# NeurAI-Lab/biHomE

Hardware: AMD Instinct MI355X
Metric: training image-pairs/s (128x128 patch, bs=64 per GPU, full step: fwd+bwd+Adam) (higher is better)
Workload: dtype f32

## Files before the change

### bihome_amd/_lib.py

```python
import ctypes
import os
from ctypes import POINTER, Structure, c_char_p, c_float, c_int, c_int64, c_void_p

_HERE = os.path.dirname(os.path.abspath(__file__))
TUNING = os.environ.get("BIHOME_TUNING") == "1"
_VARIANT = os.environ.get("BIHOME_LIB_VARIANT", "")
LIB_PATH = os.path.join(_HERE, "libbihome_hip_tuning.so" if TUNING else
                        ("libbihome_hip_%s.so" % _VARIANT if _VARIANT.isalnum() else "libbihome_hip.so"))


class BhConvDesc(Structure):
    _fields_ = [(n, c_int) for n in ("N", "Hi", "Wi", "Ci", "Ho", "Wo", "Co", "kh", "kw", "stride", "pad",
                                     "transposed", "in_nchw", "out_nchw", "precision", "w_layout", "route")] + \
               [("a_bound", c_void_p), ("b_bound", c_void_p)]


GEOMETRY_FIELDS = tuple(n for n, _ in BhConvDesc._fields_[:17])
AMAX_FLOATS = 512


class BhPack3x3Job(Structure):
    _fields_ = [("w", c_void_p), ("pf", c_void_p), ("pd", c_void_p), ("Co", c_int), ("Ci", c_int), ("split", c_int),
                ("reserved", c_int)]


ROUTE_GENERIC_CONV, ROUTE_HALO_SMALL, ROUTE_NO_STEM7, ROUTE_WGRAD_GENERIC, ROUTE_WGRAD_3TAP = 1, 2, 4, 8, 16


class BhBnReduce(Structure):
    _fields_ = [("z", c_void_p), ("y", c_void_p), ("stats", c_void_p), ("gamma", c_void_p), ("beta", c_void_p),
                ("eps", c_float), ("relu", c_int)]


class BhBnIn(Structure):
    _fields_ = [("table", c_void_p), ("groups", c_int), ("relu", c_int)]


P = c_void_p
SIGNATURES = {
    "bh_version": [],
    "bh_probe_mfma_bf16": [c_int, P, P, P],
    "bh_probe_mfma_f32": [c_int, P, P, P],
    "bh_device_arch": [c_char_p, c_int],
    "bh_h4pt_fwd": [P, c_int, c_float, c_float, P, P, P],
    "bh_h4pt_bwd": [P, P, P, c_int, c_float, c_float, P, P],
    "bh_dlt_fwd": [P, P, c_int, c_int, c_int, c_int, c_int, P, P, P, P],
    "bh_dlt_bwd": [P, P, P, P, P, c_int, c_int, c_int, c_int, c_int, P, c_int, P],
    "bh_dsac_scores_fwd": [P, c_int, c_int, P, P],
    "bh_scale_samples_fwd": [P, P, c_int, c_int64, c_int, P, P],
    "bh_scale_samples_bwd": [P, P, P, c_int, c_int64, c_int, P, P, c_int, P],
    "bh_dsac_score": [P, P, c_int, c_int, c_int, c_int, c_int, c_float, c_float, P, P, P],
    "bh_dsac_scores_bwd": [P, P, P, P, c_int, c_int, c_int, c_int, c_int, c_float, c_float, P, P, P, c_int, P],
    "bh_ransac_homography": [P, P, c_int, c_int, c_int, c_int, c_float, P, P, P, P, P, P, P, P, P],
    "bh_homography_refine_lm": [P, P, c_int, c_int, c_int, c_int, P, P, P, P],
    "bh_warp_fwd": [P, P, c_int, c_int, c_int, c_int, c_int, P, P, c_int, P],
    "bh_warp_bwd": [P, P, P, P, c_int, c_int, c_int, c_int, c_int, P, c_int, P],
    "bh_triplet_l1_fwd": [P] * 8 + [c_int, c_int, c_int, P, P, P, c_int, P],
    "bh_bihome_loss_fwd": [P, P, P, c_int, c_float, P, P],
    "bh_bihome_loss_bwd": [P] * 14 + [c_int, c_int, c_int, c_float] + [P] * 6 + [P],
    "bh_oneline_loss_fwd": [P, P, P, P, P, c_int, c_int, c_int, c_float, c_int, P, P, P, P, P, c_int, P],
    "bh_oneline_loss_bwd": [P, P, P, P, P, P, P, c_int, c_int, c_int, c_int, P, P, P, P],
    "bh_zhang_triplet_fwd": [P] * 8 + [c_int, c_int, c_float, c_int, P, P, P, P],
    "bh_zhang_triplet_bwd": [P] * 12 + [c_int, c_int, c_int] + [P] * 8 + [P],
    "bh_warp_bwd_img": [P, P, c_int, c_int, c_int, c_int, P, P, c_int, P],
    "bh_photo_warp_fwd": [P, P, P, c_int, c_int, c_int, c_int, c_int, P, c_int, P],
    "bh_photo_warp_bwd": [P, P, P, P, c_int, c_int, c_int, c_int, c_int, P, c_int, P],
    "bh_mask_fwd": [P, P, c_int, c_int, c_float, P, P, P, P, P],
    "bh_mask_bwd": [P] * 7 + [c_int, c_int, c_float, P, P, P],
    "bh_conv3x3_pack": [P, c_int, P],
    "bh_conv3x3_pack_f16": [P, c_int, P],
    "bh_absmax": [P, c_int64, P, P],
    "bh_bn_fwd_coeffs": [P, P, P, P, P, c_int, c_int, c_int, c_float, c_float, P, P, P],
    "bh_bn_fwd": [P] * 8 + [c_int, c_int, c_int, c_float, c_float, c_int, c_int, P, P],
    "bh_bn_bwd": [P] * 11 + [c_int, c_int, c_int, c_float, c_int, c_int, P, P, P, P],
    "bh_conv_variant": [POINTER(BhConvDesc), c_int, c_int, c_int, c_char_p, c_int],
    "bh_conv_fwd": [P, P, P, P, POINTER(BhConvDesc), P],
    "bh_conv_fwd_act": [P, P, P, P, P, POINTER(BhConvDesc), c_int, P],
    "bh_conv_fwd_amax": [P, P, P, P, POINTER(BhConvDesc), P, P],
    "bh_conv_fwd_bnstats": [P, P, P, P, POINTER(BhConvDesc), P, c_int, P],
    "bh_conv_fwd_bnin": [P, P, P, P, POINTER(BhConvDesc), P, c_int, POINTER(BhBnIn), P],
    "bh_conv_wgrad_bnin": [P, P, P, P, POINTER(BhConvDesc), P, c_int64, POINTER(BhBnIn), P],
    "bh_conv_dgrad": [P, P, P, POINTER(BhConvDesc), c_int, P],
    "bh_conv_dgrad_colsum": [P, P, P, POINTER(BhConvDesc), P, P],
    "bh_bias_grad_from_sums": [P, P, c_int, c_int, P],
    "bh_conv_dgrad_s2": [P, P, P, POINTER(BhConvDesc), c_int, P, P],
    "bh_conv_dgrad_bnreduce": [P, P, P, POINTER(BhConvDesc), c_int, POINTER(BhBnReduce), P, c_int, P],
    "bh_col2im_c1": [P, P, POINTER(BhConvDesc), c_int, P],
    "bh_stem7_dgrad_c1": [P, P, P, POINTER(BhConvDesc), P],
    "bh_stem7_dgrad_c1_warp": [P, P, P, POINTER(BhConvDesc), P, P, P, c_int, P, P],
    "bh_stem7_fwd_warp": [P, P, c_int, P, P, P, POINTER(BhConvDesc), P, P, P, c_int, P],
    "bh_stem7_wgrad": [P, P, P, POINTER(BhConvDesc), P, ctypes.c_size_t, P],
    "bh_conv_wgrad": [P, P, P, P, POINTER(BhConvDesc), P],
    "bh_conv_wgrad_det": [P, P, P, P, POINTER(BhConvDesc), P, c_int64, P],
    "bh_conv_bias_grad": [P, P, POINTER(BhConvDesc), P],
    "bh_bn_stats_doubles": [c_int, c_int],
    "bh_bn_scratch_doubles": [c_int, c_int],
    "bh_bn_stats": [P, P, c_int, c_int, c_int, c_int, P],
    "bh_bn_maxpool_fwd": [P] * 8 + [c_int] * 5 + [c_float, c_float, c_int, c_int, P, P],
    "bh_bn_maxpool_bwd": [P] * 10 + [c_int] * 5 + [c_float, c_int, c_int, P, P, P, P],
    "bh_bn_bwd_from_1x1": [P, P, c_int] + [P] * 8 + [c_int, c_int, c_int, c_float, c_int, P, P],
    "bh_bn_join_scratch_doubles": [c_int, c_int],
    "bh_bn_join_fwd": [P] * 13 + [c_int, c_int, c_int, c_float, c_float, c_float, c_float, c_int, P, P],
    "bh_bn_join_bwd": [P] * 15 + [c_int, c_int, c_int, c_float, c_float, c_int, P, P, P],
    "bh_bn_join_bwd_remask": [P] * 16 + [c_int, c_int, c_int, c_float, c_float, c_int, P, P, P],
    "bh_tail_ws_doubles": [c_int, c_int, c_int],
    "bh_tail_scratch_floats": [c_int, c_int, c_int],
    "bh_tail_fwd": [P] * 11 + [c_int] * 6 + [c_float, c_float, c_int, c_int, P],
    "bh_tail_bwd": [P] * 17 + [c_int] * 6 + [c_float, c_int, c_int, P],
    "bh_synth_pairs": [P] * 5 + [c_int] * 5 + [c_float, c_float, P, P, P],
    "bh_synth_image": [P, P, P, c_int, c_int, c_int, c_int, c_float, c_float, P, P],
    "bh_maxpool3s2_fwd": [P, P, P, c_int, c_int, c_int, c_int, P],
    "bh_maxpool3s2_bwd": [P, P, P, c_int, c_int, c_int, c_int, P],
    "bh_gap_fwd": [P, P, c_int, c_int, c_int, P],
    "bh_gap_bwd": [P, P, c_int, c_int, c_int, P],
    "bh_add": [P, P, P, c_int64, P],
}


class BihomeLibError(RuntimeError):
    pass


def _load():
    if not os.path.exists(LIB_PATH):
        raise BihomeLibError(
            "bihome_amd: %s not found - the HIP extension is not built. Run `python __graft_entry__.py build` "
            "(hipcc --offload-arch=gfx950). There is no CPU fallback." % LIB_PATH)
    lib = ctypes.CDLL(LIB_PATH)
    for name, argtypes in SIGNATURES.items():
        try:
            fn = getattr(lib, name)
        except AttributeError as e:
            raise BihomeLibError("bihome_amd: %s does not export %s (stale build?)" % (LIB_PATH, name)) from e
        fn.argtypes = argtypes
        fn.restype = c_int
    lib.bh_conv_wgrad_det_bytes.argtypes = [POINTER(BhConvDesc)]
    lib.bh_conv_wgrad_det_bytes.restype = c_int64
    lib.bh_stem7_wgrad_ws_bytes.argtypes = [POINTER(BhConvDesc)]
    lib.bh_stem7_wgrad_ws_bytes.restype = ctypes.c_size_t
    lib.bh_warp_bwd_img_scratch_doubles.argtypes = [c_int, c_int, c_int, c_int, c_int]
    lib.bh_warp_bwd_img_scratch_doubles.restype = ctypes.c_size_t
    if TUNING:
        lib.bh_debug_force_tile.argtypes = [c_int, c_int]
        lib.bh_debug_force_tile.restype = c_int
    return lib


lib = _load()
ROUTE_DETERMINISTIC, BN_DETERMINISTIC, F_DETERMINISTIC = 128, 32, 1
DSAC_METHODS = {"repr_error": 0, "inliers_ratio": 1, "soft_inliers_ratio": 2}
ROUTE_C3_PC = 512
ROUTE_WX3_PC = 1024
ROUTE_WX3_SHARED = 2048
ROUTE_GEMM_X3 = 4096
ROUTE_C3_TILE_WG = 256


def check(rc, what):
    if rc != 0:
        kind = {-1: "BH_E_BADARG", -2: "BH_E_UNSUPPORTED"}.get(rc, "hipError_t %d" % rc)
        raise BihomeLibError("%s failed: %s" % (what, kind))
```

### bihome_amd/csrc/bn.hip

```cpp
#include "common.h"

#define BN_MAX_CHUNKS 256

struct BnGeom {
    int groups, rows, C, C4, LPR, RPP, nchunks, rows_per_chunk;
    int det;
};

static bool bn_geom(int groups, int rows, int C, BnGeom& g, int det) {
    if (C % 4 || groups < 1 || rows < 1) return false;
    g.groups = groups; g.rows = rows; g.C = C; g.C4 = C / 4; g.det = det;
    if (g.C4 > 256 || (256 % g.C4)) return false;
    g.LPR = g.C4; g.RPP = 256 / g.LPR;
    int n = rows / (g.RPP * 4);
    if (n < 1) n = 1;
    if (n > BN_MAX_CHUNKS) n = BN_MAX_CHUNKS;
    g.rows_per_chunk = (rows + n - 1) / n;
    g.nchunks = (rows + g.rows_per_chunk - 1) / g.rows_per_chunk;
    return true;
}

template <int NV>
__device__ __forceinline__ void reduce_rows(double (&v)[NV], int LPR, int RPP, double* sm ) {
    for (int i = 0; i < NV; ++i) sm[threadIdx.x * NV + i] = v[i];
// ... 582 lines not shown
    for (int i = 0; i < 4; ++i) {
        const int c = cq * 4 + i;
        ra[i] = bn_raw(stats_a, gamma_a, remask ? beta_a : nullptr, nullptr, nullptr, 0, g.groups, grp, g.C, c, g.det);
        rb[i] = bn_raw(stats_b, gamma_b, remask ? beta_b : nullptr, nullptr, nullptr, 0, g.groups, grp, g.C, c, g.det);
        cf[i] = coef[(size_t)grp * g.C + c];
    }
    const size_t gbase = ((size_t)grp * g.rows) * g.C + cq * 4;
    const int stride = gridDim.x * g.RPP;
    int r = blockIdx.x * g.RPP + r0;
    float4 dv[4], yv[4], av[4], bv[4];
    auto issue = [&](int rbase) {
#pragma unroll
        for (int u = 0; u < 4; ++u) {
            const int rr = rbase + u * stride;
            const size_t off = gbase + (size_t)rr * g.C;
            const bool ok = rr < g.rows;
            dv[u] = make_float4(0.f, 0.f, 0.f, 0.f); av[u] = dv[u]; bv[u] = dv[u];
            yv[u] = make_float4(1.f, 1.f, 1.f, 1.f);
            if (ok) {
                dv[u] = *reinterpret_cast<const float4*>(gy + off);
                if (relu && !remask) yv[u] = *reinterpret_cast<const float4*>(y + off);
                av[u] = *reinterpret_cast<const float4*>(xa + off);
                bv[u] = *reinterpret_cast<const float4*>(xb + off);
            }
        }
    };
    issue(r);
    float ma[4], ia[4], sca[4], mb[4], ib[4], scb[4], shm[4];
    const double inv_rows = 1.0 / (double)g.rows;
#pragma unroll
    for (int i = 0; i < 4; ++i) {
        float sha, shb;
        bn_coeffs_from_raw(ra[i], 0, eps_a, inv_rows, ma[i], ia[i], sca[i], sha);
        bn_coeffs_from_raw(rb[i], 0, eps_b, inv_rows, mb[i], ib[i], scb[i], shb);
        shm[i] = sha + shb;
    }
    while (true) {
#pragma unroll
        for (int u = 0; u < 4; ++u) {
            const int rr = r + u * stride;
            if (rr >= g.rows) break;
            const size_t off = gbase + (size_t)rr * g.C;
            const float d0[4] = {dv[u].x, dv[u].y, dv[u].z, dv[u].w};
            const float y0[4] = {yv[u].x, yv[u].y, yv[u].z, yv[u].w};
            const float a[4] = {av[u].x, av[u].y, av[u].z, av[u].w}, b[4] = {bv[u].x, bv[u].y, bv[u].z, bv[u].w};
            float oa[4], ob[4];
#pragma unroll
            for (int i = 0; i < 4; ++i) {
                const float yi = remask ? __builtin_fmaf(a[i], sca[i], __builtin_fmaf(b[i], scb[i], shm[i])) : y0[i];
                const float di = (relu && !(yi > 0.f)) ? 0.f : d0[i];
                const float e = di - cf[i].x;
                oa[i] = sca[i] * (e - (a[i] - ma[i]) * ia[i] * cf[i].y);
                ob[i] = scb[i] * (e - (b[i] - mb[i]) * ib[i] * cf[i].z);
                vmax_a = fmaxf(vmax_a, fabsf(oa[i])); vmax_b = fmaxf(vmax_b, fabsf(ob[i]));
            }
            *reinterpret_cast<float4*>(gxa + off) = make_float4(oa[0], oa[1], oa[2], oa[3]);
            *reinterpret_cast<float4*>(gxb + off) = make_float4(ob[0], ob[1], ob[2], ob[3]);
        }
        r += 4 * stride;
        if (r >= g.rows) break;
        issue(r);
    }
    if (amax_a) bh_amax_commit(amax_a, vmax_a, blockIdx.x + blockIdx.y * 7u, sm_amax);
    if (amax_b) { __syncthreads(); bh_amax_commit(amax_b, vmax_b, blockIdx.x + blockIdx.y * 5u, sm_amax); }
}

BH_KNOB(g_bn_apply_cap, 512);
#ifdef BH_TUNING
void bh_bn_tune(int cap) { g_bn_apply_cap = cap; }
#endif
static int apply_blocks(const BnGeom& g) {
    int nb = (g.rows + g.RPP * 4 - 1) / (g.RPP * 4);
    int cap = g_bn_apply_cap / g.groups;
    if (cap < 1) cap = 1;
    if (nb > cap) nb = cap;
    if (nb < 1) nb = 1;
    return nb;
}

__global__ void __launch_bounds__(256) bn_fwd_coeffs_kernel(const double* __restrict__ stats, const float* __restrict__ gamma,
                                                            const float* __restrict__ beta, BnGeom g, float eps, float momentum,
                                                            float* __restrict__ upd_mean, float* __restrict__ upd_var,
                                                            float2* __restrict__ table, unsigned* __restrict__ amax) {
    __shared__ float sm_amax[4];
    if (upd_mean && blockIdx.x == gridDim.x - 1) { bn_update_running(stats, g, momentum, upd_mean, upd_var); return; }
    const int i = blockIdx.x * 256 + threadIdx.x;
    float bound = 0.f;
    if (i < g.groups * g.C) {
        const int grp = i / g.C, c = i - grp * g.C;
        float mean, invstd, sc, sh;
        bn_coeffs(stats, gamma, beta, nullptr, nullptr, 0, g.groups, grp, g.C, c, eps, (double)g.rows, mean, invstd, sc, sh, g.det);
        table[i] = make_float2(sc, sh);
        bound = 2.0f * (fabsf(gamma ? gamma[c] : 1.f) * sqrtf((float)g.rows) + fabsf(beta ? beta[c] : 0.f));
    }
    if (amax) bh_amax_commit(amax, bound, blockIdx.x, sm_amax);
}

int bn_launch_stats(const float* x, int groups, int rows, int C, double* sums, hipStream_t s, int det) {
    BnGeom g;
    if (!bn_geom(groups, rows, C, g, det ? 1 : 0)) return BH_E_UNSUPPORTED;
    hipLaunchKernelGGL(bn_stats_kernel, dim3(g.nchunks, groups), dim3(256), 0, s, x, g, sums);
    BH_LAUNCH_CHECK();
    return BH_OK;
}

int bn1_fwd(const float* x, const float* gamma, const float* beta, float* running_mean, float* running_var, const float* res, float* y,
            double* stats, int groups, int rows, float eps, float momentum, int flags, int use_running, hipStream_t s);
int bn1_bwd(const float* gy, const float* y, const float* x, const float* gamma, const float* beta, const double* stats, float* gx,
            float* gres, float* ggamma, float* gbeta, double* scratch, int groups, int rows, float eps, int flags, int use_running,
            const float* running_mean, const float* running_var, hipStream_t s);

extern "C" {

int bh_bn_stats_doubles(int groups, int C) { return (int)BH_BN_SUM_DOUBLES(groups, C); }

int bh_bn_fwd(const float* x, const float* gamma, const float* beta, float* running_mean, float* running_var,
              const float* res, float* y, double* stats, int groups, int rows, int C, float eps, float momentum,
              int flags, int use_running, float* amax_y, void* stream) {
    BnGeom g;
    if (!x || !y || !stats) return BH_E_BADARG;
    if (use_running && (!running_mean || !running_var)) return BH_E_BADARG;
    if (C == 1) return amax_y ? BH_E_UNSUPPORTED : bn1_fwd(x, gamma, beta, running_mean, running_var, res, y, stats, groups, rows, eps, momentum, flags, use_running, bh_stream(stream));
    if (!bn_geom(groups, rows, C, g, (flags & BH_BN_DETERMINISTIC) ? 1 : 0)) return BH_E_UNSUPPORTED;
    hipStream_t s = bh_stream(stream);
    if (!use_running && !(flags & 8)) {
        hipLaunchKernelGGL(bn_stats_kernel, dim3(g.nchunks, groups), dim3(256), 0, s, x, g, stats);
        BH_LAUNCH_CHECK();
    }
    const bool upd = !use_running && running_mean && running_var;
    hipLaunchKernelGGL(bn_apply_kernel, dim3(apply_blocks(g), groups), dim3(256), 0, s, x, gamma, beta, running_mean,
                       running_var, res, y, stats, g, eps, flags, use_running, momentum, upd ? running_mean : nullptr,
                       upd ? running_var : nullptr, reinterpret_cast<unsigned*>(amax_y));
    BH_LAUNCH_CHECK();
    return BH_OK;
}

int bh_bn_fwd_coeffs(const double* stats, const float* gamma, const float* beta, float* running_mean, float* running_var, int groups,
                     int rows, int C, float eps, float momentum, float* table, float* amax_y, void* stream) {
    BnGeom g;
    if (!stats || !table) return BH_E_BADARG;
    if (!bn_geom(groups, rows, C, g, -1)) return BH_E_UNSUPPORTED;
    const bool upd = running_mean && running_var;
    hipLaunchKernelGGL(bn_fwd_coeffs_kernel, dim3((groups * C + 255) / 256 + (upd ? 1 : 0)), dim3(256), 0, bh_stream(stream), stats, gamma, beta, g, eps,
                       momentum, upd ? running_mean : nullptr, upd ? running_var : nullptr, reinterpret_cast<float2*>(table),
                       reinterpret_cast<unsigned*>(amax_y));
    BH_LAUNCH_CHECK();
    return BH_OK;
}

int bh_bn_bwd(const float* gy, const float* y, const float* x, const float* gamma, const float* beta, const double* stats, float* gx,
              float* gres, float* ggamma, float* gbeta, double* scratch, int groups, int rows, int C, float eps, int flags,
              int use_running, const float* running_mean, const float* running_var, float* amax_gx, void* stream) {
    BnGeom g;
    if (!gy || !x || !gx || !stats || !scratch || ((flags & 1) && !(flags & 4) && !y)) return BH_E_BADARG;
    if ((flags & 4) && (flags & 2)) return BH_E_BADARG;
    if (C == 1) return amax_gx ? BH_E_UNSUPPORTED : bn1_bwd(gy, y, x, gamma, beta, stats, gx, gres, ggamma, gbeta, scratch, groups, rows, eps, flags, use_running,
                               running_mean, running_var, bh_stream(stream));
    if (!bn_geom(groups, rows, C, g, (flags & BH_BN_DETERMINISTIC) ? 1 : 0)) return BH_E_UNSUPPORTED;
    hipStream_t s = bh_stream(stream);
    if (flags & 16) {
        if (use_running) return BH_E_BADARG;
        hipLaunchKernelGGL(bn_bwd_apply_kernel, dim3(apply_blocks(g), groups), dim3(256), 0, s, gy, y, x, gamma, beta,
                           (const float4*)nullptr, gx, gres, g, flags, stats, (const double*)scratch, eps, ggamma, gbeta,
                           reinterpret_cast<unsigned*>(amax_gx));
        BH_LAUNCH_CHECK();
        return BH_OK;
    }
    float4* coef = reinterpret_cast<float4*>(scratch);
    double* part = scratch + (size_t)groups * C * 2;
    const bool need_sums = !use_running || ggamma || gbeta;
    if (need_sums) {
        hipLaunchKernelGGL(bn_bwd_reduce_kernel, dim3(g.nchunks, groups), dim3(256), 0, s, gy, y, x, gamma, beta, stats,
                           running_mean, running_var, g, eps, flags, use_running, part);
        BH_LAUNCH_CHECK();
    }
    BnGeom gf = g;
    if (!need_sums) gf.nchunks = 0;
    hipLaunchKernelGGL(bn_bwd_finalize_kernel, dim3(C), dim3(64), 0, s, part, gf, stats, running_mean, running_var, eps,
                       use_running, ggamma, gbeta, coef);
    BH_LAUNCH_CHECK();
    hipLaunchKernelGGL(bn_bwd_apply_kernel, dim3(apply_blocks(g), groups), dim3(256), 0, s, gy, y, x, gamma, beta, coef,
                       gx, gres, g, flags, (const double*)nullptr, (const double*)nullptr, eps, (float*)nullptr,
                       (float*)nullptr, reinterpret_cast<unsigned*>(amax_gx));
    BH_LAUNCH_CHECK();
    return BH_OK;
}

int bh_bn_scratch_doubles(int groups, int C) { return groups * C * 2 * (1 + (BN_MAX_CHUNKS > 256 ? BN_MAX_CHUNKS : 256)); }

int bh_bn_stats(const float* x, double* stats, int groups, int rows, int C, int flags, void* stream) {
    if (!x || !stats) return BH_E_BADARG;
    return bn_launch_stats(x, groups, rows, C, stats, bh_stream(stream), (flags & BH_BN_DETERMINISTIC) ? 1 : 0);
}

int bh_bn_maxpool_fwd(const float* x, const float* gamma, const float* beta, float* running_mean, float* running_var, float* y,
                      unsigned char* idx, double* stats, int groups, int N, int Hi, int Wi, int C, float eps, float momentum, int flags,
                      int use_running, float* amax_y, void* stream) {
    BnGeom g;
    if (!x || !y || !stats || N < 1 || groups < 1 || N % groups) return BH_E_BADARG;
    if (use_running && (!running_mean || !running_var)) return BH_E_BADARG;
    const int rows = (N / groups) * Hi * Wi;
    if (!bn_geom(groups, rows, C, g, (flags & BH_BN_DETERMINISTIC) ? 1 : 0) || groups * C * 8 > 32768) return BH_E_UNSUPPORTED;
    hipStream_t s = bh_stream(stream);
    if (!use_running && !(flags & 8)) {
        hipLaunchKernelGGL(bn_stats_kernel, dim3(g.nchunks, groups), dim3(256), 0, s, x, g, stats);
        BH_LAUNCH_CHECK();
    }
    const int Ho = (Hi - 1) / 2 + 1, Wo = (Wi - 1) / 2 + 1;
    const size_t total = (size_t)N * Ho * Wo * (C / 4);
    size_t nb = (total + 255) / 256;
    if (nb > 2048) nb = 2048;
    nb = (nb * 256 / (C / 4)) * (C / 4) / 256;
    if (nb < 1) nb = 1;
    const bool upd = !use_running && running_mean && running_var;
    hipLaunchKernelGGL(bn_maxpool_fwd_kernel, dim3((unsigned)nb), dim3(256), (size_t)groups * C * 8, s, x, gamma, beta, running_mean, running_var,
                       stats, y, idx, g, N, Hi, Wi, Ho, Wo, eps, flags & 1, use_running, momentum, upd ? running_mean : nullptr,
                       upd ? running_var : nullptr, reinterpret_cast<unsigned*>(amax_y));
    BH_LAUNCH_CHECK();
    return BH_OK;
}

struct PoolGeom { int Hi, Wi, Ho, Wo, ipg; };

struct PoolTaps {
    uchar4 w[4];
    float4 g[4];
    unsigned char t[4];
    bool ok[4];
};
__device__ __forceinline__ void pooled_taps_load(PoolTaps& q, const unsigned char* __restrict__ idx, const float* __restrict__ gy, const PoolGeom& pg,
                                                 int n, int iy, int ix, int C4, int c, bool live) {
    const int oyA = iy >> 1, oyB = (iy + 1) >> 1, oxA = ix >> 1, oxB = (ix + 1) >> 1;
    const bool vy = oyB != oyA && oyB < pg.Ho, vx = oxB != oxA && oxB < pg.Wo;
#pragma unroll
    for (int k = 0; k < 4; ++k) {
        const bool by = k >> 1, bx = k & 1;
        q.ok[k] = live && (!by || vy) && (!bx || vx);
        const int oy = (by && vy) ? oyB : oyA, ox = (bx && vx) ? oxB : oxA;
        q.t[k] = (unsigned char)((iy - (oy * 2 - 1)) * 3 + (ix - (ox * 2 - 1)));
        const size_t o = live ? (((size_t)n * pg.Ho + oy) * pg.Wo + ox) * C4 + c : 0;
        q.w[k] = *reinterpret_cast<const uchar4*>(idx + o * 4);
        q.g[k] = *reinterpret_cast<const float4*>(gy + o * 4);
    }
}
__device__ __forceinline__ float4 pooled_taps_sum(const PoolTaps& q) {
    float4 d = make_float4(0.f, 0.f, 0.f, 0.f);
#pragma unroll
    for (int k = 0; k < 4; ++k) {
        if (q.ok[k] && q.w[k].x == q.t[k]) d.x += q.g[k].x;
        if (q.ok[k] && q.w[k].y == q.t[k]) d.y += q.g[k].y;
        if (q.ok[k] && q.w[k].z == q.t[k]) d.z += q.g[k].z;
        if (q.ok[k] && q.w[k].w == q.t[k]) d.w += q.g[k].w;
    }
    return d;
}

__global__ void __launch_bounds__(256) bn_maxpool_bwd_reduce_kernel(const float* __restrict__ gy, const unsigned char* __restrict__ idx,
                                                                    const float* __restrict__ x, const float* __restrict__ gamma,
                                                                    const float* __restrict__ beta, const double* __restrict__ stats,
                                                                    const float* __restrict__ rmean, const float* __restrict__ rvar, BnGeom g,
                                                                    PoolGeom pg, float eps, int relu, int use_running, double* __restrict__ part) {
    __shared__ double sm[256 * 8];
    const int cq = threadIdx.x % g.LPR, r0 = threadIdx.x / g.LPR;
    const int grp = blockIdx.y, chunk = blockIdx.x;
    const int rbeg = chunk * g.rows_per_chunk, rend = min(g.rows, rbeg + g.rows_per_chunk);
    float mean[4], invstd[4], sc[4], sh[4];
#pragma unroll
    for (int i = 0; i < 4; ++i)
        bn_coeffs(stats, gamma, beta, rmean, rvar, use_running, g.groups, grp, g.C, cq * 4 + i, eps, (double)g.rows, mean[i], invstd[i], sc[i], sh[i], g.det);
    const size_t gbase = ((size_t)grp * g.rows) * g.C + cq * 4;
    const int hw = pg.Hi * pg.Wi;
    double v[8] = {0, 0, 0, 0, 0, 0, 0, 0};
    for (int r = rbeg + r0; r < rend; r += 4 * g.RPP) {
        float4 a[4];
        PoolTaps q[4];
#pragma unroll
        for (int u = 0; u < 4; ++u) {
            const int rr = r + u * g.RPP;
            const bool live = rr < rend;
            const int rc = live ? rr : rbeg;
            const int nl = rc / hw, p = rc - nl * hw, iy = p / pg.Wi, ix = p - iy * pg.Wi;
            a[u] = *reinterpret_cast<const float4*>(x + gbase + (size_t)rc * g.C);
            pooled_taps_load(q[u], idx, gy, pg, grp * pg.ipg + nl, iy, ix, g.C4, cq, live);
        }
#pragma unroll
        for (int u = 0; u < 4; ++u) {
            if (r + u * g.RPP >= rend) break;
            float4 d = pooled_taps_sum(q[u]);
            const float4 av = a[u];
            if (relu) {
                if (!(av.x * sc[0] + sh[0] > 0.f)) d.x = 0.f;
                if (!(av.y * sc[1] + sh[1] > 0.f)) d.y = 0.f;
                if (!(av.z * sc[2] + sh[2] > 0.f)) d.z = 0.f;
                if (!(av.w * sc[3] + sh[3] > 0.f)) d.w = 0.f;
            }
            v[0] += d.x; v[1] += d.y; v[2] += d.z; v[3] += d.w;
            v[4] += (double)(d.x * ((av.x - mean[0]) * invstd[0]));
            v[5] += (double)(d.y * ((av.y - mean[1]) * invstd[1]));
            v[6] += (double)(d.z * ((av.z - mean[2]) * invstd[2]));
            v[7] += (double)(d.w * ((av.w - mean[3]) * invstd[3]));
        }
    }
    reduce_rows<8>(v, g.LPR, g.RPP, sm);
    if ((int)threadIdx.x < g.LPR) {
        double* p = part + (((size_t)grp * g.nchunks + chunk) * g.C + cq * 4) * 2;
        for (int i = 0; i < 4; ++i) { p[i * 2] = v[i]; p[i * 2 + 1] = v[4 + i]; }
    }
}

__global__ void __launch_bounds__(256) bn_maxpool_bwd_apply_kernel(const float* __restrict__ gy, const unsigned char* __restrict__ idx,
                                                                   const float* __restrict__ x, const float* __restrict__ gamma,
                                                                   const float* __restrict__ beta, const float4* __restrict__ coef,
                                                                   float* __restrict__ gx, BnGeom g, PoolGeom pg, int relu,
                                                                   unsigned* __restrict__ amax) {
// ... 293 lines not shown
```

### bihome_amd/csrc/capi.hip

```cpp
#include "common.h"
#include <stdarg.h>
#include <stdio.h>
#include <string.h>


thread_local BhQuery* bh_query_ctx = nullptr;


bool bh_query(const char* fmt, ...) {
    BhQuery* q = bh_query_ctx;
    if (!q) return false;
    if (q->len && q->len < (int)sizeof(q->name) - 1) q->name[q->len++] = '+';
    va_list ap;
    va_start(ap, fmt);
    const int room = (int)sizeof(q->name) - q->len;
    const int w = vsnprintf(q->name + q->len, (size_t)room, fmt, ap);
    va_end(ap);
    if (w > 0) q->len += w < room ? w : room - 1;
    return true;
}

extern "C" {

int bh_version(void) { return 2; }


int bh_device_arch(char* buf, int buflen) {
    hipDeviceProp_t prop;
    hipError_t e = hipGetDeviceProperties(&prop, 0);
    if (e != hipSuccess) return (int)e;
    if (buf && buflen > 0) {
        strncpy(buf, prop.gcnArchName, (size_t)buflen - 1);
        buf[buflen - 1] = 0;
    }
    return BH_OK;
}

int bh_conv_variant(const bh_conv_desc* d, int which, int accumulate, int with_bnstats , char* buf, int n) {
    if (!d || !buf || n < 2 || which < 0 || which > 6) return BH_E_BADARG;
    BhQuery q;
    q.name[0] = 0; q.len = 0;
    float* p = reinterpret_cast<float*>(static_cast<uintptr_t>(256));
    double* pd = reinterpret_cast<double*>(static_cast<uintptr_t>(256));
    bh_query_ctx = &q;
    int rc;
    if (which == 0) rc = with_bnstats ? bh_conv_fwd_bnstats(p, p, nullptr, p, d, pd, with_bnstats, nullptr) : bh_conv_fwd(p, p, nullptr, p, d, nullptr);
    else if (which == 1) rc = bh_conv_dgrad(p, p, p, d, accumulate, nullptr);
    else if (which == 2) rc = bh_conv_wgrad(p, p, p, nullptr, d, nullptr);
    else if (which == 3) rc = bh_conv_wgrad_det(p, p, p, nullptr, d, p, 1ll << 40, nullptr);
    else if (which == 6) rc = bh_conv_dgrad_colsum(p, p, p, d, pd, nullptr);
    else {
        bh_bn_reduce bnr = {};
        bnr.z = p; bnr.y = which == 5 ? p : nullptr; bnr.stats = pd; bnr.gamma = p; bnr.beta = p; bnr.eps = 1e-5f; bnr.relu = 1;
        rc = bh_conv_dgrad_bnreduce(p, p, p, d, accumulate, &bnr, pd, with_bnstats > 0 ? with_bnstats : 1, nullptr);
    }
    bh_query_ctx = nullptr;
    if (rc) return rc;
    strncpy(buf, q.name, (size_t)n - 1);
    buf[n - 1] = 0;
    return BH_OK;
}

}
```

### bihome_amd/csrc/conv3x3.hip

```cpp
#include "common.h"
#include "conv3x3_args.h"
#include <type_traits>

#ifndef C3_X3_PIPE
#define C3_X3_PIPE 0
#endif

#ifndef C3_BN32_WAVES
#define C3_BN32_WAVES 2
#endif

#ifdef BH_TUNING
__device__ unsigned long long g_c3_ts[8 * 16384];
#define C3_STAMP(tile, k) do { if (a.dbg_ts && threadIdx.x == 0 && (tile) < 16384) { g_c3_ts[(tile) * 8 + (k)] = wall_clock64();          \
        if ((k) == 1 || (k) == 2) g_c3_ts[(tile) * 8 + 4 + (k)] = __builtin_readcyclecounter(); } } while (0)
#else
#define C3_STAMP(tile, k) do { } while (0)
#endif

constexpr int C3_HALO_BYTES = 8 * 200 * 16;
constexpr int C3_B_BYTES = 8192;
constexpr int C3_LDS_BYTES = 2 * C3_HALO_BYTES + 2 * C3_B_BYTES;

template <int BN, int SUBT, int TM, bool MAP4 = false>
__device__ __forceinline__ void c3_epilogue(const C3Args& a, f32x16 (&acc)[TM], int bx, int n0, int wm, int wn, int wh, int l31, int kh2,
                                            double& s1, double& s2, int& img, int& g) {
    g = bx * SUBT + wm;
    const int n = n0 + wn * 32 + l31;
    const bool valid = g < a.subtiles && n < a.Nn;
    const int gg = g < a.subtiles ? g : 0;
    int ty, tx;
    if constexpr (MAP4) { img = gg * 4; ty = 0; tx = 0; }
    else if (a.tpi_shift >= 0) { img = gg >> a.tpi_shift; const int t = gg & (a.tiles_per_img - 1); ty = t >> a.tx_shift; tx = t & (a.tiles_x - 1); }
    else { img = gg / a.tiles_per_img; const int t = gg - img * a.tiles_per_img; ty = t / a.tiles_x; tx = t - ty * a.tiles_x; }
    const float bv = (a.bias && n < a.Nn) ? a.bias[n] : 0.0f;
    s1 = 0.0; s2 = 0.0;
    float r_mean = 0.f, r_invstd = 0.f, r_sc = 0.f, r_sh = 0.f;
    if (a.bnr_z && valid) {
        const int grp = img / a.imgs_per_group;
        const double rows = (double)a.bnr_rows;
        const double mu = bn_sum_total(a.bnr_stats, a.groups, grp, a.Nn, n, 0, a.det) / rows;
        double var = bn_sum_total(a.bnr_stats, a.groups, grp, a.Nn, n, 1, a.det) / rows - mu * mu;
        if (var < 0) var = 0;
        r_mean = (float)mu;
        r_invstd = 1.0f / sqrtf((float)var + a.bnr_eps);
        r_sc = (a.bnr_gamma ? a.bnr_gamma[n] : 1.f) * r_invstd;
        r_sh = (a.bnr_beta ? a.bnr_beta[n] : 0.f) - r_mean * r_sc;
    }
    if (valid) {
        unsigned rowoff[4];
#pragma unroll
        for (int rq = 0; rq < 4; ++rq) {
            const int sr = c3_strip_row(2 * rq + kh2);
            if constexpr (MAP4)
                rowoff[rq] = ((unsigned)((img + 2 * wh + (sr >> 2)) * 16 + (sr & 3) * 4) * (unsigned)a.Nn + (unsigned)n) * 4u;
            else
                rowoff[rq] = ((unsigned)((img * a.H + ty * 8 + sr) * a.W + tx * 8) * (unsigned)a.Nn + (unsigned)n) * 4u;
        }
        const unsigned colstep = (unsigned)a.Nn * 4u;
        const unsigned col0 = MAP4 ? 0u : (unsigned)(wh * 4) * colstep;
        const __amdgpu_buffer_rsrc_t rsO = __builtin_amdgcn_make_buffer_rsrc(a.Out, 0, a.out_bytes, 0x00020000);
#define C3_SOFF(i, r) (col0 + (unsigned)((i) * 4 + ((r) & 3)) * colstep)
        if (!a.accumulate && !a.res && !a.bnr_z) {
#pragma unroll
            for (int i = 0; i < TM; ++i)
#pragma unroll
                for (int rq = 0; rq < 4; ++rq) {
                    float q1 = 0.f, q2 = 0.f;
#pragma unroll
                    for (int c = 0; c < 4; ++c) {
                        float v = acc[i][rq * 4 + c] + bv;
                        if (a.relu) v = fmaxf(v, 0.0f);
                        __builtin_amdgcn_raw_buffer_store_b32(__builtin_bit_cast(unsigned, v), rsO, rowoff[rq], C3_SOFF(i, c), 0);
                        q1 += v; q2 = __builtin_fmaf(v, v, q2);
                    }
                    s1 += (double)q1; s2 += (double)q2;
                }
        } else {
            const bool rd_old = a.accumulate, rd_res = a.res != nullptr, rd_z = a.bnr_z != nullptr;
            const bool rd_y = rd_z && a.bnr_relu && a.bnr_y != nullptr;
            const float c_x0 = -r_mean * r_invstd;
            auto body = [&](auto EXTRA, auto ZMODE) {
                constexpr bool HAS_EXTRA = decltype(EXTRA)::value;
                constexpr int ZM = decltype(ZMODE)::value;
                float ext[HAS_EXTRA ? TM : 1][16], zin[ZM > 0 ? TM : 1][16], yin[ZM == 2 ? TM : 1][16];
                if constexpr (HAS_EXTRA) {
                    const __amdgpu_buffer_rsrc_t rsR = __builtin_amdgcn_make_buffer_rsrc(const_cast<float*>(rd_res ? a.res : a.Out), 0, a.out_bytes, 0x00020000);
#pragma unroll
                    for (int i = 0; i < TM; ++i)
#pragma unroll
                        for (int r = 0; r < 16; ++r) {
                            float o = 0.f;
                            if (rd_old) o = __builtin_bit_cast(float, __builtin_amdgcn_raw_buffer_load_b32(rsO, rowoff[r >> 2], C3_SOFF(i, r), 0));
                            if (rd_res) o += __builtin_bit_cast(float, __builtin_amdgcn_raw_buffer_load_b32(rsR, rowoff[r >> 2], C3_SOFF(i, r), 0));
                            ext[i][r] = o;
                        }
                }
                if constexpr (ZM > 0) {
                    const __amdgpu_buffer_rsrc_t rsZ = __builtin_amdgcn_make_buffer_rsrc(const_cast<float*>(a.bnr_z), 0, a.out_bytes, 0x00020000);
#pragma unroll
                    for (int i = 0; i < TM; ++i)
#pragma unroll
                        for (int r = 0; r < 16; ++r)
                            zin[i][r] = __builtin_bit_cast(float, __builtin_amdgcn_raw_buffer_load_b32(rsZ, rowoff[r >> 2], C3_SOFF(i, r), 0));
                }
                if constexpr (ZM == 2) {
                    const __amdgpu_buffer_rsrc_t rsY = __builtin_amdgcn_make_buffer_rsrc(const_cast<float*>(a.bnr_y), 0, a.out_bytes, 0x00020000);
#pragma unroll
                    for (int i = 0; i < TM; ++i)
#pragma unroll
                        for (int r = 0; r < 16; ++r)
                            yin[i][r] = __builtin_bit_cast(float, __builtin_amdgcn_raw_buffer_load_b32(rsY, rowoff[r >> 2], C3_SOFF(i, r), 0));
                }
#pragma unroll
                for (int i = 0; i < TM; ++i)
#pragma unroll
                    for (int rq = 0; rq < 4; ++rq) {
                        float q1 = 0.f, q2 = 0.f;
#pragma unroll
                        for (int c = 0; c < 4; ++c) {
                            const int r = rq * 4 + c;
                            float v = acc[i][r] + bv;
                            if constexpr (HAS_EXTRA) v += ext[i][r];
                            if (a.relu) v = fmaxf(v, 0.0f);
                            __builtin_amdgcn_raw_buffer_store_b32(__builtin_bit_cast(unsigned, v), rsO, rowoff[rq], C3_SOFF(i, r), 0);
                            if constexpr (ZM > 0) {
                                const float zv = zin[i][r];
                                if (a.bnr_relu) {
                                    const float yv = ZM == 2 ? yin[i][r] : __builtin_fmaf(zv, r_sc, r_sh);
                                    if (!(yv > 0.f)) v = 0.f;
                                }
                                q1 += v; q2 = __builtin_fmaf(v, __builtin_fmaf(zv, r_invstd, c_x0), q2);
                            } else {
                                q1 += v; q2 = __builtin_fmaf(v, v, q2);
                            }
                        }
                        s1 += (double)q1; s2 += (double)q2;
                    }
            };
            using T_ = std::true_type; using F_ = std::false_type;
            using Z0 = std::integral_constant<int, 0>; using Z1 = std::integral_constant<int, 1>; using Z2 = std::integral_constant<int, 2>;
            if (rd_old || rd_res) {
                if (!rd_z) body(T_{}, Z0{}); else if (!rd_y) body(T_{}, Z1{}); else body(T_{}, Z2{});
            } else {
                if (!rd_z) body(F_{}, Z0{}); else if (!rd_y) body(F_{}, Z1{}); else body(F_{}, Z2{});
            }
        }
#undef C3_SOFF
    }
}

template <int BN, int PHASE>
__device__ __forceinline__ void c3_stats_merge(const C3Args& a, char* redb, double s1, double s2, int img, int g, int bx, int n0, int wave,
                                               int lane, int tid) {
    const int l31 = lane & 31, kh2 = lane >> 5;
    double* red = reinterpret_cast<double*>(redb);
    int* grp_of = reinterpret_cast<int*>(redb + 4 * 32 * 2 * 8);
    if constexpr (PHASE != 2) {
        s1 += __shfl_xor(s1, 32, 64);
        s2 += __shfl_xor(s2, 32, 64);
        const int grp = img / a.imgs_per_group;
        if (kh2 == 0) { red[(wave * 32 + l31) * 2] = s1; red[(wave * 32 + l31) * 2 + 1] = s2; }
        if (lane == 0) grp_of[wave] = g < a.subtiles ? grp : -1;
    }
    if constexpr (PHASE == 0) __syncthreads();
    if constexpr (PHASE != 1) {
        constexpr int SHARE = BN == 64 ? 2 : 4;
        if (tid < (4 / SHARE) * 64) {
            const int cr = tid >> 6, col = (tid >> 1) & 31, mom = tid & 1;
            const int nn = n0 + cr * 32 + col;
            if (nn < a.Nn) {
                int done = 0;
#pragma unroll
                for (int w0 = 0; w0 < SHARE; ++w0) {
                    const int wv0 = BN == 64 ? (w0 + 2 * cr) : w0;
                    const int g0 = grp_of[wv0];
                    if (g0 < 0 || (done >> w0) & 1) continue;
                    double tot = red[(wv0 * 32 + col) * 2 + mom];
#pragma unroll
                    for (int w1 = w0 + 1; w1 < SHARE; ++w1) {
                        const int wv1 = BN == 64 ? (w1 + 2 * cr) : w1;
                        if (grp_of[wv1] == g0) { tot += red[(wv1 * 32 + col) * 2 + mom]; done |= 1 << w1; }
                    }
                    bh_acc_add(&a.bn_sums[bn_sum_index(bx % BH_BN_SUM_SLOTS, a.groups, g0, a.Nn, nn, mom)], tot, a.det);
                }
            }
        }
    }
}

template <bool FLIP, int BN, bool BF16 = false, int SUBT = 2, bool PACKED = false, bool X3 = false, bool BNI = false, int NP = 3, bool MAP4 = false, bool F16 = false>
__global__ void __launch_bounds__(256, X3 ? ((BN == 32 && NP == 2 && !BNI) ? C3_BN32_WAVES : 2) : 1) conv3x3_halo_kernel(C3Args a) {
    static_assert(NP == 3 || (NP == 2 && X3), "two pieces: split form only");
    static_assert(!F16 || (X3 && NP == 2), "fp16 pieces: the two-piece split form");
    static_assert(!MAP4 || (X3 && SUBT == 1 && BN == 64 && !BNI), "the 4 x 4 map form: split operands, one sub-tile, 64-channel tile");
    constexpr int SLOTS = MAP4 ? 144 : 100;
    constexpr int ROWP = MAP4 ? 6 : 10;
    static_assert(SUBT == 2 || BN == 64, "one sub-tile per workgroup is built for the 64-channel tile only");
    static_assert(!X3 || (PACKED && !BF16), "the split form exists for packed weights only");
    static_assert(!BNI || (X3 && !FLIP), "the BatchNorm-on-load form is a forward f32x3 kernel");
    constexpr int TM = (BN == 64 && SUBT == 2) ? 2 : 1;
    constexpr int HPL = SLOTS * SUBT;
    constexpr int HALO_B = (X3 ? 4 * NP : 8) * HPL * 16;
    constexpr int XJ = (4 * HPL + 255) / 256;
    constexpr int HINS = (8 * HPL + 63) / 64;
    constexpr int HJ = (HINS + 3) / 4;
    constexpr int BINS = BN == 64 ? 2 : 1;
    extern __shared__ __attribute__((aligned(16))) char smem[];
    const int tid = threadIdx.x, lane = tid & 63, wave = __builtin_amdgcn_readfirstlane(tid >> 6);
    const int l31 = lane & 31, kh2 = lane >> 5;
    const int wm = SUBT == 1 ? 0 : (BN == 64 ? (wave & 1) : (wave >> 1));
    const int wn = BN == 64 ? (wave >> 1) : 0;
    const int wh = (BN == 64 && SUBT == 2) ? 0 : (wave & 1);
    const int n0 = blockIdx.y * BN;
    constexpr unsigned OOB = 0xFFFFFFF0u;
    __amdgpu_buffer_rsrc_t rsA = __builtin_amdgcn_make_buffer_rsrc(const_cast<float*>(a.Src), 0, a.src_bytes, 0x00020000);
    __amdgpu_buffer_rsrc_t rsB = __builtin_amdgcn_make_buffer_rsrc(const_cast<float*>(a.Wt), 0, a.w_bytes, 0x00020000);
    float f16_s = 1.0f;
    int f16_kout = 0;
    if constexpr (F16) {
        const unsigned* const wrec = reinterpret_cast<const unsigned*>(a.Wt) + (a.w_bytes >> 2);
        unsigned wv = lane < 16 ? wrec[lane] : 0u;
#pragma unroll
        for (int off = 8; off > 0; off >>= 1) { const unsigned o = (unsigned)__shfl_xor((int)wv, off, 64); wv = o > wv ? o : wv; }
        const int kw = bh_f16_scale_exp((unsigned)__builtin_amdgcn_readfirstlane((int)wv));
        const int ka = bh_f16_scale_exp(bh_amax_read(a.amax_src, lane));
        f16_s = __builtin_bit_cast(float, (unsigned)(127 + ka) << 23);
        f16_kout = -(ka + kw);
    }

    unsigned boff[2] = {0u, 0u};
#pragma unroll
    for (int i = 0; i < BINS; ++i) {
        const int idx = i * 4 + wave;
        if (!FLIP) {
            const int plane = BN == 64 ? idx : idx * 2 + (lane >> 5), n = n0 + (BN == 64 ? lane : (lane & 31));
            boff[i] = n < a.Nn ? ((unsigned)(n * 9) * (unsigned)a.Cw + (unsigned)(plane * 4)) * 4u : OOB;
        } else {
            constexpr int LPR = BN / 4;
            const int k = idx * (64 / LPR) + lane / LPR, n = n0 + (lane % LPR) * 4;
            boff[i] = n < a.Nn ? ((unsigned)(k * 9) * (unsigned)a.Cw + (unsigned)n) * 4u : OOB;
        }
    }
#ifdef BH_TUNING
    const int nch = a.dbg_nch >= 0 ? a.dbg_nch : a.Kc / 32;
    const int dbg_noload = a.dbg_noload;
#else
    const int nch = a.Kc / 32;
    constexpr int dbg_noload = 0;
#endif
    const int wnG = blockIdx.y * (BN / 32) + (BN == 64 ? (wave >> 1) : 0);
    const unsigned pb_voff = (unsigned)lane * 16u;
#define C3_LOAD_B(dst, c, tap)                                                                                          \
    do {                                                                                                                \
        const unsigned so_ = (unsigned)(((c) * 9 + (tap)) * a.NW + wnG) * 4096u;                                        \
        _Pragma("unroll") for (int q_ = 0; q_ < 4; ++q_) {                                                              \
            const auto v_ = __builtin_amdgcn_raw_buffer_load_b128(rsB, pb_voff + (unsigned)q_ * 1024u, so_, 0);         \
            dst[q_] = __builtin_bit_cast(float4, v_);                                                                   \
        }                                                                                                               \
    } while (0)
#define C3_LOAD_BX(dst, c, tap)                                                                                         \
    do {                                                                                                                \
        const unsigned so_ = (unsigned)(((c) * 9 + (tap)) * a.NW + wnG) * (unsigned)(NP * 2048);                        \
        _Pragma("unroll") for (int q_ = 0; q_ < 2 * NP; ++q_) {                                                              \
            const auto v_ = __builtin_amdgcn_raw_buffer_load_b128(rsB, pb_voff + (unsigned)q_ * 1024u, so_, 0);         \
            dst[q_] = __builtin_bit_cast(uint4, v_);                                                                    \
        }                                                                                                               \
    } while (0)
    const int slab0 = (a.Kc / 32 > 1 ? 2 : 1) * HALO_B;
#define issue_B(c, tap, bs)                                                                                             \
    do {                                                                                                                \
        const unsigned soff_ = FLIP ? (unsigned)(((c) * 32 * 9 + (8 - (tap))) * a.Cw) * 4u                             \
                                    : (unsigned)((tap) * a.Cw + (c) * 32) * 4u;                                        \
        char* base_ = smem + slab0 + (bs) * C3_B_BYTES + wave * 1024;                                              \
        __builtin_amdgcn_raw_ptr_buffer_load_lds(rsB, (lds_void_ptr)(base_), 16, boff[0], soff_, 0, 0);                 \
        if (BINS == 2)                                                                                                  \
            __builtin_amdgcn_raw_ptr_buffer_load_lds(rsB, (lds_void_ptr)(base_ + 4096), 16, boff[1], soff_, 0, 0); \
    } while (0)
#define C3_ISSUE_HALO(j, c, hs)                                                                                         \
    do {                                                                                                                \
        if ((j) < HJ && (j) * 4 + wave < HINS && (((j) * 4 + wave) * 64 + lane) < 8 * HPL)                              \
            __builtin_amdgcn_raw_ptr_buffer_load_lds(rsA, (lds_void_ptr)(smem + (hs) * HALO_B + ((j) * 4 + wave) * 1024), \
                                                     16, hoff[(j) < HJ ? (j) : 0], (unsigned)((c) * 32) * 4u, 0, 0);    \
    } while (0)

    if constexpr (BNI) {
        const int n4 = a.bni_groups * a.Kc / 2;
        for (int i = tid; i < n4; i += 256)
            reinterpret_cast<float4*>(smem + a.bni_lds)[i] = reinterpret_cast<const float4*>(a.bni)[i];
        __syncthreads();
    }
    double S1 = 0.0, S2 = 0.0;
    int Simg = 0, Sg = 0x7fffffff, Sbx = 0;
    if (a.desync > 0 && (((blockIdx.x + gridDim.x * blockIdx.y) >> 8) & 1)) {
        for (int i = 0; i < a.desync; ++i) __builtin_amdgcn_s_sleep(127);
    }
    for (int it = 0; it < a.tpb; ++it) {
    const int bx = blockIdx.x * a.tpb + it;
// ... 278 lines not shown
                        for (int i = 0; i < TM; ++i) acc[i] = __builtin_amdgcn_mfma_f32_32x32x2f32(af[i][q].z, bcur[q].z, acc[i], 0, 0, 0);
#pragma unroll
                        for (int i = 0; i < TM; ++i) acc[i] = __builtin_amdgcn_mfma_f32_32x32x2f32(af[i][q].w, bcur[q].w, acc[i], 0, 0, 0);
                    }
                }
                if (tap == 8) {
                    __builtin_amdgcn_sched_barrier(0);
                    asm volatile("s_waitcnt vmcnt(0)" ::: "memory");
                    __syncthreads();
                }
#pragma unroll
                for (int q = 0; q < 4; ++q) bcur[q] = bnext[q];
            }
        }
    } else {
    for (int c = 0; c < nch; ++c) {
        const int hs = c & 1;
        const char* hbase = smem + hs * HALO_B + a_lane;
        const bool more = c + 1 < nch;
#pragma unroll
        for (int tap = 0; tap < 9; ++tap) {
            const int dy = tap / 3, dx = tap - dy * 3;
            const char* ap = hbase + (dy * 10 + dx) * 16;
            const char* bp = smem + slab0 + bs * C3_B_BYTES + b_lane;
            float4 af[TM][4], b[4];
#pragma unroll
            for (int q = 0; q < 4; ++q) {
#pragma unroll
                for (int i = 0; i < TM; ++i) af[i][q] = *reinterpret_cast<const float4*>(ap + q * (2 * HPL * 16) + i * 64);
                if (!FLIP) b[q] = *reinterpret_cast<const float4*>(bp + q * (2 * BN * 16));
                else {
                    b[q].x = *reinterpret_cast<const float*>(bp + (q * 8 + 0) * (BN * 4));
                    b[q].y = *reinterpret_cast<const float*>(bp + (q * 8 + 1) * (BN * 4));
                    b[q].z = *reinterpret_cast<const float*>(bp + (q * 8 + 2) * (BN * 4));
                    b[q].w = *reinterpret_cast<const float*>(bp + (q * 8 + 3) * (BN * 4));
                }
            }
            if (!(dbg_noload & 1)) {
                if (tap < 8) issue_B(c, tap + 1, bs ^ 1);
                else if (more) issue_B(c + 1, 0, bs ^ 1);
            }
            if (tap < HJ && more && !(dbg_noload & 2)) C3_ISSUE_HALO(tap, c + 1, hs ^ 1);
            if constexpr (BF16) {
#pragma unroll
                for (int s2 = 0; s2 < 2; ++s2) {
                    const bf16x8 bb = c3_pack_bf16(b[2 * s2], b[2 * s2 + 1]);
#pragma unroll
                    for (int i = 0; i < TM; ++i)
                        acc[i] = __builtin_amdgcn_mfma_f32_32x32x16_bf16(c3_pack_bf16(af[i][2 * s2], af[i][2 * s2 + 1]), bb, acc[i], 0, 0, 0);
                }
            } else {
#pragma unroll
            for (int q = 0; q < 4; ++q) {
#pragma unroll
                for (int i = 0; i < TM; ++i) acc[i] = __builtin_amdgcn_mfma_f32_32x32x2f32(af[i][q].x, b[q].x, acc[i], 0, 0, 0);
#pragma unroll
                for (int i = 0; i < TM; ++i) acc[i] = __builtin_amdgcn_mfma_f32_32x32x2f32(af[i][q].y, b[q].y, acc[i], 0, 0, 0);
#pragma unroll
                for (int i = 0; i < TM; ++i) acc[i] = __builtin_amdgcn_mfma_f32_32x32x2f32(af[i][q].z, b[q].z, acc[i], 0, 0, 0);
#pragma unroll
                for (int i = 0; i < TM; ++i) acc[i] = __builtin_amdgcn_mfma_f32_32x32x2f32(af[i][q].w, b[q].w, acc[i], 0, 0, 0);
            }
            }
            __builtin_amdgcn_sched_barrier(0);
            asm volatile("s_waitcnt vmcnt(0)" ::: "memory");
            __syncthreads();
            bs ^= 1;
        }
    }
    }
    }
#undef C3_ISSUE_HALO
#undef issue_B
#undef C3_LOAD_B
#undef C3_LOAD_BX

    C3_STAMP(bx * gridDim.y + blockIdx.y, 2);
    if constexpr (F16) {
#pragma unroll
        for (int i = 0; i < TM; ++i)
#pragma unroll
            for (int r = 0; r < 16; ++r) acc[i][r] = __builtin_ldexpf(acc[i][r], f16_kout);
    }
    double s1, s2;
    int img, g;
    c3_epilogue<BN, SUBT, TM, MAP4>(a, acc, bx, n0, wm, wn, wh, l31, kh2, s1, s2, img, g);
    if (a.bn_sums) {
        if (a.stat_acc) { S1 += s1; S2 += s2; Sbx = bx; if (g < Sg) { Sg = g; Simg = img; } }
        else c3_stats_merge<BN, 0>(a, smem, s1, s2, img, g, bx, n0, wave, lane, tid);
    }
#ifdef BH_TUNING
    if (a.dbg_ts) asm volatile("s_waitcnt vmcnt(0)" ::: "memory");
#endif
    __syncthreads();
    C3_STAMP(bx * gridDim.y + blockIdx.y, 3);
    }
    if (a.bn_sums && a.stat_acc) c3_stats_merge<BN, 0>(a, smem, S1, S2, Simg, Sg, Sbx, n0, wave, lane, tid);
}

constexpr int C3_MIN_BLOCKS = 256;
BH_KNOB(g_c3_noload, 0); BH_KNOB(g_c3_dbg_nch, -1); BH_KNOB(g_c3_subt, 2); BH_KNOB(g_c3_tpb, 2); BH_KNOB(g_c3_stamp, 0); BH_KNOB(g_c3_desync, 0); BH_KNOB(g_c3_walk32, 1); BH_KNOB(g_c3_pc, 1); BH_KNOB(g_c3_wt64, 512); BH_KNOB(g_c3_wt32, 512);
#ifdef BH_TUNING
extern "C" int bh_debug_read_c3_stamps(unsigned long long* out, int n) {
    if (n > 16384) n = 16384;
    return (int)hipMemcpyFromSymbol(out, HIP_SYMBOL(g_c3_ts), (size_t)n * 8 * sizeof(unsigned long long), 0, hipMemcpyDeviceToHost);
}
void bh_conv3x3_tune(int disable, int min_blocks) {
    (void)min_blocks;
    if (disable >= 500 && disable < 1000) { g_c3_stamp = disable - 500; return; }
    if (disable >= 200 && disable < 264) { g_c3_desync = disable - 200; return; }
    if (disable == 300 || disable == 301) { g_c3_walk32 = disable - 300; return; }
    if (disable >= 2000 && disable < 6000) { g_c3_wt64 = disable - 2000; return; }
    if (disable >= 6000 && disable < 10000) { g_c3_wt32 = disable - 6000; return; }
    if (disable == 310 || disable == 311) { g_c3_pc = disable - 310; return; }
    if (disable <= -100) { g_c3_dbg_nch = -100 - disable - 1; return; }
    if (disable >= 400 && disable < 464) { g_c3_noload = disable - 400; return; }
    if (disable >= 20 && disable < 24) { g_c3_tpb = disable - 20; return; }
    if (disable >= 11 && disable <= 13) { g_c3_subt = disable - 10; return; }
}
#endif

int bh_conv3x3_try(const float* src, const float* w, const float* bias, float* out, const bh_conv_desc* d, int dgrad,
                   int accumulate, hipStream_t stream, int* taken, double* bn_sums, int groups, const float* res, int relu,
                   const bh_bn_reduce* bnr, const bh_bn_in* bni) {
    *taken = 0;
    if ((d->route & BH_ROUTE_GENERIC_CONV) || d->transposed || d->kh != 3 || d->kw != 3 || d->stride != 1 || d->pad != 1 || d->in_nchw ||
        d->out_nchw || d->precision < 0 || d->precision > 4)
        return d->w_layout ? BH_E_UNSUPPORTED : 0;
    if (d->w_layout != 0 && ((d->w_layout == 2) != (d->precision == 2) || (d->w_layout == 3) != (d->precision == 3) ||
                             (d->w_layout == 4) != (d->precision == 4))) return BH_E_BADARG;
    if (d->w_layout == 4 && !d->a_bound) return BH_E_BADARG;
    const bool map4 = d->Hi == 4 && d->Wi == 4 && d->Ho == 4 && d->Wo == 4 && d->N % 4 == 0 && (d->w_layout >= 2 && d->w_layout <= 4) &&
                      d->Co % 64 == 0 && d->Ci % 64 == 0 && !bni && (!bn_sums || (groups >= 1 && d->N % groups == 0 && (d->N / groups) % 4 == 0));
    if (!map4 && (d->Hi % 8 || d->Wi % 8 || d->Ho != d->Hi || d->Wo != d->Wi)) return d->w_layout ? BH_E_UNSUPPORTED : 0;
    const int Kc = dgrad ? d->Co : d->Ci, Nn = dgrad ? d->Ci : d->Co;
    if (Kc % 32 || Nn % 32) return d->w_layout ? BH_E_UNSUPPORTED : 0;
    const int bn_tile = (Nn % 64) ? 32 : 64;
    const bool packed = d->w_layout != 0;
    const bool x3 = d->w_layout >= 2 && d->w_layout <= 4;
    const int np = d->w_layout >= 3 ? 2 : 3;
    const bool f16 = d->w_layout == 4;
    const bool bf16 = d->precision == 1;
    const long long src_bytes = (long long)d->N * d->Hi * d->Wi * Kc * 4, w_bytes = (long long)d->Co * 9 * d->Ci * (x3 ? 2 * np : 4);
    const long long out_bytes = (long long)d->N * d->Hi * d->Wi * Nn * 4;
    if (src_bytes >= (1ll << 31) || w_bytes >= (1ll << 31) || out_bytes >= (1ll << 31)) return 0;
    C3Args a = {};
    a.Src = src; a.Wt = w; a.bias = bias; a.Out = out;
    a.N = d->N; a.H = d->Hi; a.W = d->Wi; a.Kc = Kc; a.Nn = Nn; a.Cw = d->Ci; a.accumulate = accumulate;
    a.amax_src = reinterpret_cast<const unsigned*>(d->a_bound);
    a.src_bytes = (unsigned)src_bytes; a.w_bytes = (unsigned)w_bytes; a.out_bytes = (unsigned)out_bytes;
    if (bn_sums && (groups < 1 || d->N % groups || (!dgrad && bnr) || (dgrad && !bnr && accumulate))) return BH_E_BADARG;
    if (bnr) {
        if (!bnr->z || !bnr->stats) return BH_E_BADARG;
        a.bnr_z = bnr->z; a.bnr_y = bnr->y; a.bnr_stats = bnr->stats; a.bnr_gamma = bnr->gamma; a.bnr_beta = bnr->beta;
        a.bnr_eps = bnr->eps; a.bnr_relu = bnr->relu; a.bnr_rows = (d->N / groups) * d->Hi * d->Wi;
    }
    a.res = res; a.relu = relu; a.dbg_nch = g_c3_dbg_nch;
    a.bn_sums = bn_sums; a.imgs_per_group = bn_sums ? d->N / groups : 1; a.groups = groups;
    a.tiles_x = d->Wi / 8; a.tiles_per_img = (d->Hi / 8) * a.tiles_x; a.subtiles = d->N * a.tiles_per_img;
    if (map4) { a.tiles_x = 1; a.tiles_per_img = 1; a.subtiles = d->N / 4; }
    a.tx_shift = a.tpi_shift = -1;
    for (int b = 0; b < 24; ++b) {
        if (a.tiles_x == (1 << b)) a.tx_shift = b;
        if (a.tiles_per_img == (1 << b)) a.tpi_shift = b;
    }
    if (a.tx_shift < 0 || a.tpi_shift < 0) a.tx_shift = a.tpi_shift = -1;
    const bool few = (long long)((a.subtiles + 1) / 2) * (Nn / bn_tile) <= 256;
    const int subt = map4 ? 1 : (bn_tile == 64 && (g_c3_subt == 1 || (d->route & BH_ROUTE_C3_ONE_SUBTILE) || (g_c3_subt == 2 && few))) ? 1 : 2;
    dim3 grid((a.subtiles + subt - 1) / subt, Nn / bn_tile);
    a.gx_total = (int)grid.x; a.tpb = 1;
    {
        const long long wgs = (long long)grid.x * grid.y;
        if (g_c3_tpb >= 2 && !(d->route & BH_ROUTE_C3_ONE_POSITION) && subt == 2 && Kc / 32 > 1 && wgs > 512 && wgs <= 1024) {
            a.tpb = 2; grid.x = (grid.x + 1) / 2;
        }
    }
    if (bn_sums && !map4 && !(d->route & BH_ROUTE_C3_ONE_POSITION) && groups >= 1 && a.subtiles % (subt * groups) == 0) {
        const int ppg = a.subtiles / (subt * groups);
        int t = a.tpb;
        const long long wtarget = (x3 && bn_tile == 64) ? g_c3_wt64 : (x3 ? g_c3_wt32 : 2048);
        while (ppg % (t * 2) == 0 && (ppg / t > 1024 || (long long)(ppg / t) * groups * grid.y > wtarget) && t < 64) t *= 2;
        if (ppg % t == 0 && (t > 1 || a.tpb == 1)) {
            if (t != a.tpb) { a.tpb = t; grid.x = (a.gx_total + t - 1) / t; }
            a.stat_acc = 1;
        }
    }
    if (x3 && !map4 && a.tpb == 1 && !bn_sums && g_c3_walk32 && !(d->route & BH_ROUTE_C3_ONE_POSITION)) {
        const long long target = bn_tile == 32 ? 1024 : 512;
        int t = 1;
        while (a.gx_total % (t * 2) == 0 && (long long)(a.gx_total / (t * 2)) * grid.y >= target && t < 64) t *= 2;
        if (t > 1) { a.tpb = t; grid.x = a.gx_total / t; }
    }
    if (!(d->route & BH_ROUTE_HALO_SMALL) && (int)((map4 ? a.subtiles : (a.subtiles + 1) / 2) * grid.y) < (map4 ? C3_MIN_BLOCKS / 2 : C3_MIN_BLOCKS))
        return d->w_layout ? BH_E_UNSUPPORTED : 0;
    a.NW = Nn / 32;
    if (bni) {
        if (!x3 || dgrad || !bni->table || bni->groups < 1 || d->N % bni->groups || (long long)bni->groups * Kc * 8 > 4096) return BH_E_UNSUPPORTED;
        a.bni = bni->table; a.bni_relu = bni->relu; a.bni_groups = bni->groups; a.bni_ipg = d->N / bni->groups;
    }
    if (f16 && !map4 && bn_tile == 64 && !(d->route & (BH_ROUTE_C3_TILE_WG | BH_ROUTE_C3_ONE_SUBTILE | BH_ROUTE_C3_ONE_POSITION)) && g_c3_pc) {
        C3Args b = a;
        b.det = (d->route & BH_ROUTE_DETERMINISTIC) ? 1 : 0; b.dbg_noload = g_c3_noload; b.dbg_ts = g_c3_stamp;
        const int st = bh_conv3x3_pc_launch(b, dgrad, bni ? bni->table : nullptr, bni ? bni->groups : 0, bni ? bni->relu : 0, (d->route & BH_ROUTE_C3_PC) != 0, stream);
        if (st != BH_E_UNSUPPORTED) { if (st == BH_OK) *taken = 1; return st; }
    }
    if (bh_query("conv3x3_halo_kernel<%s,%d,%s,%d,%s,%s,%s,%d,%s,%s>", dgrad ? "true" : "false", bn_tile, bf16 ? "true" : "false", subt,
                 packed ? "true" : "false", x3 ? "true" : "false", bni ? "true" : "false", np, map4 ? "true" : "false", f16 ? "true" : "false")) {
        *taken = 1;
        return BH_OK;
    }
    static unsigned long long attr_devs = 0;
    typedef void (*kern_t)(C3Args);
#define C3_ROW(P) conv3x3_halo_kernel<false, 64, false, 2, P>, conv3x3_halo_kernel<true, 64, false, 2, P>,   \
                  conv3x3_halo_kernel<false, 32, false, 2, P>, conv3x3_halo_kernel<true, 32, false, 2, P>,   \
                  conv3x3_halo_kernel<false, 64, true, 2, P>,  conv3x3_halo_kernel<true, 64, true, 2, P>,    \
                  conv3x3_halo_kernel<false, 32, true, 2, P>,  conv3x3_halo_kernel<true, 32, true, 2, P>,    \
                  conv3x3_halo_kernel<false, 64, false, 1, P>, conv3x3_halo_kernel<true, 64, false, 1, P>,   \
                  conv3x3_halo_kernel<false, 64, true, 1, P>,  conv3x3_halo_kernel<true, 64, true, 1, P>
#define C3_XROW(NP_, F_) conv3x3_halo_kernel<false, 64, false, 2, true, true, false, NP_, false, F_>, conv3x3_halo_kernel<true, 64, false, 2, true, true, false, NP_, false, F_>,  \
                     conv3x3_halo_kernel<false, 32, false, 2, true, true, false, NP_, false, F_>, conv3x3_halo_kernel<true, 32, false, 2, true, true, false, NP_, false, F_>,  \
                     conv3x3_halo_kernel<false, 64, false, 1, true, true, false, NP_, false, F_>, conv3x3_halo_kernel<true, 64, false, 1, true, true, false, NP_, false, F_>,  \
                     conv3x3_halo_kernel<false, 64, false, 2, true, true, true, NP_, false, F_>, conv3x3_halo_kernel<false, 32, false, 2, true, true, true, NP_, false, F_>,   \
                     conv3x3_halo_kernel<false, 64, false, 1, true, true, true, NP_, false, F_>
    static const kern_t fns[57] = {C3_ROW(false), C3_ROW(true), C3_XROW(3, false), C3_XROW(2, false),
                                   conv3x3_halo_kernel<false, 64, false, 1, true, true, false, 3, true>, conv3x3_halo_kernel<true, 64, false, 1, true, true, false, 3, true>,
                                   conv3x3_halo_kernel<false, 64, false, 1, true, true, false, 2, true>, conv3x3_halo_kernel<true, 64, false, 1, true, true, false, 2, true>,
                                   C3_XROW(2, true),
                                   conv3x3_halo_kernel<false, 64, false, 1, true, true, false, 2, true, true>, conv3x3_halo_kernel<true, 64, false, 1, true, true, false, 2, true, true>};
#undef C3_XROW
#undef C3_ROW
    constexpr int HALO2 = 8 * 200 * 16, HALO1 = 8 * 100 * 16;
    constexpr int LDS1 = 2 * HALO1 + 2 * C3_B_BYTES;
    const int XHALO2 = 4 * np * 200 * 16, XHALO1 = 4 * np * 100 * 16;
    if (bh_device_once(attr_devs)) {
        for (int i = 42; i < 57; ++i) {
            if (i >= 46 && i < 55) continue;
            hipError_t e = hipFuncSetAttribute(reinterpret_cast<const void*>(fns[i]), hipFuncAttributeMaxDynamicSharedMemorySize, 2 * (i < 44 ? 12 : 8) * 144 * 16);
            if (e != hipSuccess) return (int)e;
        }
        for (int i0 = 0; i0 < 51; ++i0) {
            const int i = i0 < 42 ? i0 : 33 + (i0 - 42);
            const int fi = i0 < 42 ? i0 : 46 + (i0 - 42);
            const int j = i % 12;
            const int xi = i >= 24 ? (i - 24) % 9 : 0, xh2 = (i >= 33 ? 8 : 12) * 200 * 16, xh1 = xh2 / 2;
            const int full = i >= 24 ? 2 * ((xi == 4 || xi == 5 || xi == 8) ? xh1 : xh2) + (xi >= 6 ? 4096 : 0)
                                     : i < 12 ? (j < 8 ? C3_LDS_BYTES : LDS1) : 2 * (j < 8 ? HALO2 : HALO1);
            hipError_t e = hipFuncSetAttribute(reinterpret_cast<const void*>(fns[fi]), hipFuncAttributeMaxDynamicSharedMemorySize, full);
            if (e != hipSuccess) return (int)e;
        }
    }
    const int xrow = f16 ? 46 : 24 + (np == 2 ? 9 : 0);
    const kern_t fn = map4 ? fns[(f16 ? 55 : 42 + (np == 2 ? 2 : 0)) + (dgrad ? 1 : 0)] : bni ? fns[xrow + 6 + (subt == 1 ? 2 : bn_tile == 64 ? 0 : 1)] : x3 ? fns[xrow + (subt == 1 ? 4 : bn_tile == 64 ? 0 : 2) + (dgrad ? 1 : 0)]
                         : fns[(packed ? 12 : 0) + (subt == 1 ? 8 + (bf16 ? 2 : 0) + (dgrad ? 1 : 0)
                                                              : (bf16 ? 4 : 0) + (bn_tile == 64 ? 0 : 2) + (dgrad ? 1 : 0))];
    a.dbg_noload = g_c3_noload; a.dbg_ts = g_c3_stamp; a.desync = g_c3_desync; a.det = (d->route & BH_ROUTE_DETERMINISTIC) ? 1 : 0;
    const int stage = map4 ? 4 * np * 144 * 16 : x3 ? (subt == 1 ? XHALO1 : XHALO2) : subt == 1 ? HALO1 : HALO2;
    const int lds = packed ? (Kc / 32 > 1 ? 2 : 1) * stage
                           : (subt == 1 ? LDS1 : C3_LDS_BYTES) - (Kc / 32 > 1 ? 0 : stage);
    if (bni) a.bni_lds = lds;
    hipLaunchKernelGGL(fn, grid, dim3(256), lds + (bni ? bni->groups * Kc * 8 : 0), stream, a);
    BH_LAUNCH_CHECK();
    *taken = 1;
    return BH_OK;
}

__global__ void __launch_bounds__(256) pack_conv3x3_weights_kernel(const bh_pack3x3_job* __restrict__ jobs) {
    const bh_pack3x3_job j = jobs[blockIdx.y];
    const int Co = j.Co, Ci = j.Ci;
    const long long n4 = (long long)Co * 9 * Ci / 4;
    const float4* __restrict__ w4 = reinterpret_cast<const float4*>(j.w);
    if (j.split) {
        const int np = j.split == 1 ? 3 : 2;
        float wscale = 1.0f;
        if (j.split == 3) {
            const unsigned* rec = reinterpret_cast<const unsigned*>(j.pf ? j.pf : j.pd) + (long long)Co * 9 * Ci;
            unsigned m = 0;
            for (int i = 0; i < 16; ++i) m = rec[i] > m ? rec[i] : m;
            wscale = __builtin_bit_cast(float, (unsigned)(127 + bh_f16_scale_exp(m)) << 23);
        }
        const long long n8 = (long long)Co * 9 * Ci / 8;
        for (long long i = (long long)blockIdx.x * 256 + threadIdx.x; i < n8; i += (long long)gridDim.x * 256) {
            const int lane = (int)(i & 63), s2 = (int)((i >> 6) & 1);
            const int l31 = lane & 31, kh2 = lane >> 5;
            const long long r = i >> 7;
            for (int dir = 0; dir < 2; ++dir) {
                float* const dst = dir ? j.pd : j.pf;
                if (!dst) continue;
                const int NW = (dir ? Ci : Co) / 32;
                const int nt = (int)(r % NW); const long long r2 = r / NW;
                const int tap = (int)(r2 % 9), c = (int)(r2 / 9);
                const int n = nt * 32 + l31, k0 = c * 32 + (2 * s2 + kh2) * 8;
                float4 u, v;
                if (!dir) {
                    const float4* src = reinterpret_cast<const float4*>(j.w + ((long long)(n * 9 + tap) * Ci + k0));
                    u = src[0]; v = src[1];
                } else {
                    const float* src = j.w + ((long long)k0 * 9 + (8 - tap)) * Ci + n;
                    const long long ks = 9ll * Ci;
                    u = make_float4(src[0], src[ks], src[2 * ks], src[3 * ks]);
                    v = make_float4(src[4 * ks], src[5 * ks], src[6 * ks], src[7 * ks]);
                }
                uint4 p0, p1, p2;
                uint4* const o = reinterpret_cast<uint4*>(dst) + (r * 2 * np + s2) * 64 + lane;
                if (np == 3) { bh_split8(u, v, p0, p1, p2); o[4 * 64] = p2; }
                else if (j.split == 3) bh_split8_f16(u, v, wscale, p0, p1);
                else bh_split8_2(u, v, p0, p1);
// ... 65 lines not shown
```

### bihome_amd/csrc/conv3x3_pc.hip

```cpp
#include "conv3x3_args.h"
#include <type_traits>

namespace {
constexpr int PC_HPL = 200;
constexpr int PC_PS = PC_HPL * 16 + 32;
constexpr int PC_PIECE = 4 * PC_PS;
constexpr int PC_STAGE = 2 * PC_PIECE;
constexpr int PC_BTAP = 8192;
constexpr int PC_BROW = 3 * PC_BTAP;
constexpr int PC_OFF_B = 2 * PC_STAGE;
constexpr int PC_OFF_EPI = PC_OFF_B + 3 * PC_BROW;
constexpr int PC_EPI_BYTES = 128 * 64 * 4;
constexpr int PC_OFF_RED = PC_OFF_EPI + PC_EPI_BYTES;
constexpr int PC_RED_BYTES = 4 * 128 * 8;
constexpr int PC_LDS = PC_OFF_RED + PC_RED_BYTES;
constexpr unsigned PC_XOOB = 0x80000000u;

#ifdef BH_TUNING
__device__ unsigned long long g_pc_ts[12 * 160 * 2];
#define PC_BARRIER()                                                                                                    \
    do {                                                                                                                \
        const bool st_ = a.dbg_ts && blockIdx.x == (unsigned)(a.dbg_ts - 1) && (tid & 63) == 0;                        \
        if (st_ && pc_nb < 160) g_pc_ts[(wave * 160 + pc_nb) * 2] = __builtin_readcyclecounter();                       \
        asm volatile("s_waitcnt lgkmcnt(0)\n\ts_barrier" ::: "memory");                                                \
// ... 206 lines not shown
            pc_decode(a, bx * 2 < a.subtiles ? bx * 2 : 0, img, ty, tx);
            const unsigned vo = k < K ? (unsigned)((img / a.bni_ipg) * a.Kc + plane * 8) * 8u : PC_XOOB, so = (unsigned)(c_ * 256);
#pragma unroll
            for (int q = 0; q < 4; ++q)
                tb[q] = __builtin_bit_cast(pc_f4, __builtin_amdgcn_raw_buffer_load_b128(rsT, vo + (unsigned)q * 16u, so, 0));
            nis += 4; seq_tb = nis;
        };
        auto h_issue = [&](auto J, pc_f4 (&h)[NR][2], unsigned& okm, int (&seq)[NR], bool en) {
            constexpr int j = decltype(J)::value;
            if (j == 0 && en && li_c == 0) h_tile(wt0 + li_t);
            const unsigned vo = en ? xoff[j] : PC_XOOB, so = en ? (unsigned)(li_c * 128) : 0u;
            h[j][0] = __builtin_bit_cast(pc_f4, __builtin_amdgcn_raw_buffer_load_b128(rsA, vo, so, 0));
            h[j][1] = __builtin_bit_cast(pc_f4, __builtin_amdgcn_raw_buffer_load_b128(rsA, vo + 16u, so, 0));
            nis += 2; seq[j] = nis;
            okm = (okm & ~(1u << j)) | ((vo != PC_XOOB ? 1u : 0u) << j);
            if (j == NR - 1 && en) { if (++li_c == nch) { li_c = 0; ++li_t; } }
        };
        float f16_s = 1.0f;
        const float bni_lo = a.bni_relu ? 0.0f : -__builtin_inff();
        auto h_cut = [&](auto J, int stage, pc_f4 (&h)[NR][2], unsigned okm, const int (&seq)[NR], bool en) {
            constexpr int j = decltype(J)::value;
            if constexpr (BNI) {
                if (j == 0 && PC_H_ASM) {
                    wait_vm(nis - seq_tb);
                    asm volatile("" : "+v"(tb[0]), "+v"(tb[1]), "+v"(tb[2]), "+v"(tb[3]));
                }
            }
            if (PC_H_ASM) {
                wait_vm(nis - seq[j]);
                asm volatile("" : "+v"(h[j][0]), "+v"(h[j][1]));
            }
            if (en && j * 48 + (ht >> 2) < PC_HPL) {
                char* const st = smem + stage * PC_STAGE;
                float4 u = make_float4(h[j][0][0], h[j][0][1], h[j][0][2], h[j][0][3]), v = make_float4(h[j][1][0], h[j][1][1], h[j][1][2], h[j][1][3]);
                if constexpr (BNI) {
                    const bool ok = (okm >> j) & 1u;
                    u.x = ok ? __builtin_elementwise_maximum(__builtin_fmaf(u.x, tb[0][0], tb[0][1]), bni_lo) : 0.f;
                    u.y = ok ? __builtin_elementwise_maximum(__builtin_fmaf(u.y, tb[0][2], tb[0][3]), bni_lo) : 0.f;
                    u.z = ok ? __builtin_elementwise_maximum(__builtin_fmaf(u.z, tb[1][0], tb[1][1]), bni_lo) : 0.f;
                    u.w = ok ? __builtin_elementwise_maximum(__builtin_fmaf(u.w, tb[1][2], tb[1][3]), bni_lo) : 0.f;
                    v.x = ok ? __builtin_elementwise_maximum(__builtin_fmaf(v.x, tb[2][0], tb[2][1]), bni_lo) : 0.f;
                    v.y = ok ? __builtin_elementwise_maximum(__builtin_fmaf(v.y, tb[2][2], tb[2][3]), bni_lo) : 0.f;
                    v.z = ok ? __builtin_elementwise_maximum(__builtin_fmaf(v.z, tb[3][0], tb[3][1]), bni_lo) : 0.f;
                    v.w = ok ? __builtin_elementwise_maximum(__builtin_fmaf(v.w, tb[3][2], tb[3][3]), bni_lo) : 0.f;
                }
                uint4 p0, p1;
                bh_split8_f16(u, v, f16_s, p0, p1);
                *reinterpret_cast<uint4*>(st + lo0 + j * 768) = p0;
                *reinterpret_cast<uint4*>(st + PC_PIECE + lo0 + j * 768) = p1;
            }
        };
#ifdef BH_TUNING
        const bool hon = !(a.dbg_noload & 4);
#else
        constexpr bool hon = true;
#endif
        using J0 = std::integral_constant<int, 0>; using J1 = std::integral_constant<int, 1>; using J2 = std::integral_constant<int, 2>;
        using J3 = std::integral_constant<int, 3>; using J4 = std::integral_constant<int, 4>;
#define PC_H_CHUNK(kap_, h, okm, seq, SET, AHEAD)                                                                       \
    do {                                                                                                                \
        const bool cut_ = (kap_) + 1 < K && hon, iss_ = (kap_) + (AHEAD) < K && hon;                                    \
        h_cut(J0{}, SET, h, okm, seq, cut_); h_issue(J0{}, h, okm, seq, iss_);                                          \
        h_cut(J1{}, SET, h, okm, seq, cut_); h_issue(J1{}, h, okm, seq, iss_);                                          \
        PC_BARRIER();                                                                                        \
        h_cut(J2{}, SET, h, okm, seq, cut_); h_issue(J2{}, h, okm, seq, iss_);                                          \
        h_cut(J3{}, SET, h, okm, seq, cut_); h_issue(J3{}, h, okm, seq, iss_);                                          \
        PC_BARRIER();                                                                                        \
        h_cut(J4{}, SET, h, okm, seq, cut_); h_issue(J4{}, h, okm, seq, iss_);                                          \
        if constexpr (BNI) tb_issue(hon ? (kap_) + 2 : K);                                                              \
        PC_BARRIER();                                                                                        \
    } while (0)
#define PC_H_ISSUE_ALL(h, okm, seq, en)                                                                                 \
    do { h_issue(J0{}, h, okm, seq, en); h_issue(J1{}, h, okm, seq, en); h_issue(J2{}, h, okm, seq, en);                \
         h_issue(J3{}, h, okm, seq, en); h_issue(J4{}, h, okm, seq, en); } while (0)
        if constexpr (!BNI) {
            const unsigned rec_ = lane < BH_AMAX_SLOTS ? a.amax_src[lane * BH_AMAX_STRIDE] : 0u;
            PC_H_ISSUE_ALL(hA, okA, seqA, hon);
            PC_H_ISSUE_ALL(hB, okB, seqB, 1 < K && hon);
            f16_s = __builtin_bit_cast(float, (unsigned)(127 + bh_f16_scale_exp(pc_amax_reduce(rec_))) << 23);
            h_cut(J0{}, 0, hA, okA, seqA, hon); h_cut(J1{}, 0, hA, okA, seqA, hon); h_cut(J2{}, 0, hA, okA, seqA, hon);
            h_cut(J3{}, 0, hA, okA, seqA, hon); h_cut(J4{}, 0, hA, okA, seqA, hon);
            PC_H_ISSUE_ALL(hA, okA, seqA, 2 < K && hon);
            PC_BARRIER();
            for (int kap = 0; kap < K; kap += 2) {
                PC_H_CHUNK(kap, hB, okB, seqB, 1, 3);
                if (kap + 1 < K) PC_H_CHUNK(kap + 1, hA, okA, seqA, 0, 3);
            }
        } else {
            (void)hB; (void)okB; (void)seqB;
            const unsigned rec_ = lane < BH_AMAX_SLOTS ? a.amax_src[lane * BH_AMAX_STRIDE] : 0u;
            tb_issue(hon ? 0 : K);
            PC_H_ISSUE_ALL(hA, okA, seqA, hon);
            f16_s = __builtin_bit_cast(float, (unsigned)(127 + bh_f16_scale_exp(pc_amax_reduce(rec_))) << 23);
            h_cut(J0{}, 0, hA, okA, seqA, hon); h_cut(J1{}, 0, hA, okA, seqA, hon); h_cut(J2{}, 0, hA, okA, seqA, hon);
            h_cut(J3{}, 0, hA, okA, seqA, hon); h_cut(J4{}, 0, hA, okA, seqA, hon);
            tb_issue(hon ? 1 : K);
            PC_H_ISSUE_ALL(hA, okA, seqA, 1 < K && hon);
            PC_BARRIER();
            for (int kap = 0; kap < K; ++kap) PC_H_CHUNK(kap, hA, okA, seqA, (kap + 1) & 1, 2);
        }
        PC_BARRIER();
        PC_BARRIER();
        PC_BARRIER();
        PC_BARRIER();
#undef PC_H_ISSUE_ALL
#undef PC_H_CHUNK
        return;
    }

    if (wave < 8) {
        const __amdgpu_buffer_rsrc_t rsB = __builtin_amdgcn_make_buffer_rsrc(const_cast<float*>(a.Wt), 0, a.w_bytes, 0x00020000);
#ifdef BH_TUNING
        const bool doff = a.dbg_noload & 8;
#else
        constexpr bool doff = false;
#endif
        auto dma_num = [&](int r) {
            const int kp = r / 3, row = r - kp * 3, ti_ = kp / nch, c_ = kp - ti_ * nch;
            const int ny = (wt0 + ti_) / a.gx_total;
#pragma unroll
            for (int t = 0; t < 3; ++t)
#pragma unroll
                for (int piece = 0; piece < 8; ++piece) {
                    const unsigned so = (unsigned)(((c_ * 9 + row * 3 + t) * a.NW + ny * 2) * 4096 + piece * 1024);
                    __builtin_amdgcn_raw_ptr_buffer_load_lds(rsB, (lds_void_ptr)(smem + PC_OFF_B + row * PC_BROW + t * PC_BTAP + piece * 1024), 16,
                                                             (unsigned)lane * 16u, so, 0, 0);
                }
        };
        int pro = 0;
        if (!doff) { dma_num(0); if (R > 1) { dma_num(1); ++pro; } if (R > 2) { dma_num(2); ++pro; } }
        wait_vm(24 * pro);
        PC_BARRIER();
        for (int rho = 0; rho < R; ++rho) {
            int nd = 0;
            if (rho >= 1 && rho + 2 < R && !doff) { dma_num(rho + 2); nd = 24; }
            wait_vm(rho == 0 ? ((R > 2 && !doff) ? 24 : 0) : nd);
            PC_BARRIER();
        }
        PC_BARRIER();
        PC_BARRIER();
        PC_BARRIER();
        PC_BARRIER();
        return;
    }

    {
        __builtin_amdgcn_s_setprio(1);
        const int ew = wave - 8;
        const int cq = lane & 15, pl = lane >> 4;
        const __amdgpu_buffer_rsrc_t rsO = __builtin_amdgcn_make_buffer_rsrc(a.Out, 0, a.out_bytes, 0x00020000);
        const __amdgpu_buffer_rsrc_t rsR = __builtin_amdgcn_make_buffer_rsrc(const_cast<float*>(a.res ? a.res : a.Out), 0, a.out_bytes, 0x00020000);
        const __amdgpu_buffer_rsrc_t rsZ = __builtin_amdgcn_make_buffer_rsrc(const_cast<float*>(a.bnr_z ? a.bnr_z : a.Out), 0, a.out_bytes, 0x00020000);
        const __amdgpu_buffer_rsrc_t rsY = __builtin_amdgcn_make_buffer_rsrc(const_cast<float*>(a.bnr_y ? a.bnr_y : a.Out), 0, a.out_bytes, 0x00020000);
        constexpr bool stats = EM & 1, use_ext = EM & 2, rd_z = EM & 4, rd_y = EM & 8;
        const bool rd_res = a.res != nullptr;
        const unsigned nn4 = (unsigned)a.Nn * 4u;
#ifdef BH_TUNING
        const bool eoff_ = a.dbg_noload & 16;
#else
        constexpr bool eoff_ = false;
#endif

        unsigned tbase[2] = {0u, 0u}, fbase[2] = {0u, 0u};
        bool tvalid[2] = {false, false}, fvalid[2] = {false, false};
        float4 bv = make_float4(0.f, 0.f, 0.f, 0.f);
        float4 r_invstd = bv, r_cx0 = bv, r_sc = bv, r_sh = bv;
        int cur_grp = -1, cur_n0 = 0;
        double S1[4] = {0.0, 0.0, 0.0, 0.0}, S2[4] = {0.0, 0.0, 0.0, 0.0};
        bool have = false;
        int pend_grp = 0, pend_n0 = 0;
        bool pending = false;
        auto stash = [&]() {
            double* const red = reinterpret_cast<double*>(smem + PC_OFF_RED);
#pragma unroll
            for (int e = 0; e < 4; ++e) {
                double s1 = S1[e], s2 = S2[e];
                s1 += __shfl_xor(s1, 16, 64); s1 += __shfl_xor(s1, 32, 64);
                s2 += __shfl_xor(s2, 16, 64); s2 += __shfl_xor(s2, 32, 64);
                if (pl == 0) { red[(ew * 64 + cq * 4 + e) * 2] = s1; red[(ew * 64 + cq * 4 + e) * 2 + 1] = s2; }
                S1[e] = 0.0; S2[e] = 0.0;
            }
            pend_grp = cur_grp; pend_n0 = cur_n0; pending = true; have = false;
        };
        auto commit = [&]() {
            if (!pending) return;
            if (ew == 0) {
                const double* const red = reinterpret_cast<const double*>(smem + PC_OFF_RED);
#pragma unroll
                for (int q = 0; q < 2; ++q) {
                    const int idx = q * 64 + lane;
                    const double tot = ((red[idx] + red[128 + idx]) + red[256 + idx]) + red[384 + idx];
                    bh_acc_add(&a.bn_sums[bn_sum_index(0, a.groups, pend_grp, a.Nn, pend_n0 + (idx >> 1), idx & 1)], tot, a.det);
                }
            }
            pending = false;
        };
        auto tile_geom = [&](int wt, unsigned (&base)[2], bool (&valid)[2], int& grp, int& n0) {
            const int ny_ = wt / a.gx_total, bx = wt - ny_ * a.gx_total;
            n0 = ny_ * 64; grp = 0;
#pragma unroll
            for (int s_ = 0; s_ < 2; ++s_) {
                const int g = bx * 2 + s_;
                int img, ty, tx;
                pc_decode(a, g < a.subtiles ? g : 0, img, ty, tx);
                valid[s_] = g < a.subtiles;
                base[s_] = ((unsigned)((img * a.H + ty * 8) * a.W + tx * 8) * (unsigned)a.Nn + (unsigned)n0) * 4u;
                if (s_ == 0) grp = img / a.imgs_per_group;
            }
        };
        auto f_tile = [&](int wt) { int g_, n_; tile_geom(wt, fbase, fvalid, g_, n_); };
        auto e_tile = [&](int wt) {
            int grp, n0;
            tile_geom(wt, tbase, tvalid, grp, n0);
            if (stats && have && (grp != cur_grp || n0 != cur_n0)) stash();
            if (grp != cur_grp || n0 != cur_n0) {
                cur_grp = grp; cur_n0 = n0;
                const int n = n0 + cq * 4;
                bv = a.bias ? *reinterpret_cast<const float4*>(a.bias + n) : make_float4(0.f, 0.f, 0.f, 0.f);
                if (rd_z) {
                    float isd[4], cx[4], sc[4], sh[4];
                    const double rows = (double)a.bnr_rows;
#pragma unroll
                    for (int e = 0; e < 4; ++e) {
                        const double mu = bn_sum_total(a.bnr_stats, a.groups, grp, a.Nn, n + e, 0, a.det) / rows;
                        double var = bn_sum_total(a.bnr_stats, a.groups, grp, a.Nn, n + e, 1, a.det) / rows - mu * mu;
                        if (var < 0) var = 0;
                        const float mean = (float)mu;
                        isd[e] = 1.0f / sqrtf((float)var + a.bnr_eps);
                        sc[e] = (a.bnr_gamma ? a.bnr_gamma[n + e] : 1.f) * isd[e];
                        sh[e] = (a.bnr_beta ? a.bnr_beta[n + e] : 0.f) - mean * sc[e];
                        cx[e] = -mean * isd[e];
                    }
                    r_invstd = make_float4(isd[0], isd[1], isd[2], isd[3]); r_cx0 = make_float4(cx[0], cx[1], cx[2], cx[3]);
                    r_sc = make_float4(sc[0], sc[1], sc[2], sc[3]); r_sh = make_float4(sh[0], sh[1], sh[2], sh[3]);
                }
            }
        };
        float4 pf_a[4], pf_z[4], pf_y[4];
        constexpr int nld = (use_ext ? 1 : 0) + (rd_z ? 1 : 0) + (rd_y ? 1 : 0);
        const unsigned voff = (unsigned)((ew >> 1) * a.W + ((ew & 1) << 2) + pl) * nn4 + (unsigned)cq * 16u;
        const unsigned rowstep2 = 2u * (unsigned)a.W * nn4;
        const char* const epi_l = smem + PC_OFF_EPI + ew * 1024 + lane * 16;
        const __amdgpu_buffer_rsrc_t rsA_ = rd_res ? rsR : rsO;
        auto epi_fetch = [&](auto Q, int idx) {
            constexpr int q = decltype(Q)::value;
            if (nld == 0 || !((idx >> 2) ? fvalid[1] : fvalid[0])) return;
            const unsigned so = ((idx >> 2) ? fbase[1] : fbase[0]) + (unsigned)(idx & 3) * rowstep2;
            if constexpr (use_ext) pf_a[q] = __builtin_bit_cast(float4, __builtin_amdgcn_raw_buffer_load_b128(rsA_, voff, so, 0));
            if constexpr (rd_z) pf_z[q] = __builtin_bit_cast(float4, __builtin_amdgcn_raw_buffer_load_b128(rsZ, voff, so, 0));
            if constexpr (rd_y) pf_y[q] = __builtin_bit_cast(float4, __builtin_amdgcn_raw_buffer_load_b128(rsY, voff, so, 0));
        };
        int kout = 0;
        auto epi_run = [&](auto Q, int idx) {
            constexpr int q = decltype(Q)::value;
            if (!((idx >> 2) ? tvalid[1] : tvalid[0])) return;
            const unsigned so = ((idx >> 2) ? tbase[1] : tbase[0]) + (unsigned)(idx & 3) * rowstep2;
            const float4 av = *reinterpret_cast<const float4*>(epi_l + idx * 4096);
            const float4 z0 = make_float4(0.f, 0.f, 0.f, 0.f);
            const float4 o = use_ext ? pf_a[q] : z0, zz = rd_z ? pf_z[q] : z0, yy = rd_y ? pf_y[q] : z0;
            const float accv[4] = {av.x, av.y, av.z, av.w}, bb[4] = {bv.x, bv.y, bv.z, bv.w};
            const float oo[4] = {o.x, o.y, o.z, o.w};
            const float z4[4] = {zz.x, zz.y, zz.z, zz.w}, y4[4] = {yy.x, yy.y, yy.z, yy.w};
            const float isd[4] = {r_invstd.x, r_invstd.y, r_invstd.z, r_invstd.w}, cx[4] = {r_cx0.x, r_cx0.y, r_cx0.z, r_cx0.w};
            const float sc[4] = {r_sc.x, r_sc.y, r_sc.z, r_sc.w}, sh[4] = {r_sh.x, r_sh.y, r_sh.z, r_sh.w};
            float out[4];
            const bool do_relu = a.relu != 0, mask_on = rd_z && a.bnr_relu;
#pragma unroll
            for (int e = 0; e < 4; ++e) {
                float v = __builtin_ldexpf(accv[e], kout) + bb[e];
                if constexpr (use_ext) v += oo[e];
                v = do_relu ? fmaxf(v, 0.0f) : v;
                out[e] = v;
                if constexpr (stats) {
                    float vm = v, t = v;
                    if constexpr (rd_z) {
                        const float yv = rd_y ? y4[e] : __builtin_fmaf(z4[e], sc[e], sh[e]);
                        vm = (mask_on && !(yv > 0.f)) ? 0.f : v;
                        t = __builtin_fmaf(z4[e], isd[e], cx[e]);
                    }
                    S1[e] += (double)vm;
                    S2[e] = __builtin_fma((double)vm, (double)t, S2[e]);
                }
            }
            const __attribute__((ext_vector_type(4))) unsigned ov =
                __builtin_bit_cast(__attribute__((ext_vector_type(4))) unsigned, make_float4(out[0], out[1], out[2], out[3]));
            __builtin_amdgcn_raw_buffer_store_b128(ov, rsO, voff, so, 0);
            asm volatile("s_nop 3" :: "v"(ov));
            have = true;
        };
        using Q0 = std::integral_constant<int, 0>; using Q1 = std::integral_constant<int, 1>; using Q2 = std::integral_constant<int, 2>;
        using Q3 = std::integral_constant<int, 3>;
        const int nph = 3 * nch;
        const int grp = ew >> 1;
        const int nA = grp ? (nph - 1) / 2 : nph / 2;
        constexpr int UB = 4, NB = 2;
        const int BPP = (NB + nA - 1) / nA;
        auto run_batch = [&](int b) {
            const int i0 = b * UB;
            epi_run(Q0{}, i0 + 0); epi_run(Q1{}, i0 + 1); epi_run(Q2{}, i0 + 2); epi_run(Q3{}, i0 + 3);
        };
        auto fetch_batch = [&](int b) {
            const int i0 = b * UB;
            epi_fetch(Q0{}, i0 + 0); epi_fetch(Q1{}, i0 + 1); epi_fetch(Q2{}, i0 + 2); epi_fetch(Q3{}, i0 + 3);
        };
        auto step_batch = [&](int b, int nxt) {
            run_batch(b);
            if (nld == 0) return;
            if (b + 1 < NB) fetch_batch(b + 1);
            else if (nxt >= 0) { f_tile(nxt); fetch_batch(0); }
        };

        if (!eoff_) {
            const unsigned* const wrec = reinterpret_cast<const unsigned*>(a.Wt) + (a.w_bytes >> 2);
            const unsigned wv = lane < 16 ? wrec[lane] : 0u;
            const unsigned rec_ = lane < BH_AMAX_SLOTS ? a.amax_src[lane * BH_AMAX_STRIDE] : 0u;
            kout = -(bh_f16_scale_exp(pc_amax_reduce(wv)) + bh_f16_scale_exp(pc_amax_reduce(rec_)));
            asm volatile("" :: "s"(kout) : "memory");
            f_tile(wt0);
            fetch_batch(0);
        }
        PC_BARRIER();
        for (int ti = 0; ti < Tw; ++ti) {
            for (int k = 0; k < nph; ++k) {
                if (ti > 0 && !eoff_) {
                    if (k == 0) e_tile(wt0 + ti - 1);
                    else {
                        if (k == 1) commit();
                        if ((k & 1) != grp) {
                            const int a_ = grp ? (k >> 1) - 1 : (k >> 1);
                            for (int bb = 0; bb < BPP; ++bb) { const int b = a_ * BPP + bb; if (b < NB) step_batch(b, wt0 + ti); }
                        }
                    }
                }
                PC_BARRIER();
            }
        }
        PC_BARRIER();
        if (!eoff_) e_tile(wt0 + Tw - 1);
        PC_BARRIER();
        commit();
        PC_BARRIER();
        if (!eoff_) {
            for (int b = 0; b < NB; ++b) step_batch(b, -1);
            if (stats) stash();
        }
        PC_BARRIER();
        commit();
    }
}
}

#ifdef BH_TUNING
extern "C" int bh_debug_read_pc_stamps(unsigned long long* out) {
    return (int)hipMemcpyFromSymbol(out, HIP_SYMBOL(g_pc_ts), sizeof(unsigned long long) * 12 * 160 * 2, 0, hipMemcpyDeviceToHost);
}
#endif

int bh_conv3x3_pc_launch(C3Args& a, int dgrad, const float* bni_table, int bni_groups, int bni_relu, bool force, hipStream_t stream) {
    if (a.Kc % 32 || a.Nn % 64 || a.subtiles < 1) return BH_E_UNSUPPORTED;
    const long long sub_per_group = (long long)a.imgs_per_group * a.tiles_per_img;
    if ((a.bn_sums || a.bnr_z) && (sub_per_group % 2)) return BH_E_UNSUPPORTED;
    if (a.accumulate && a.res) return BH_E_UNSUPPORTED;
    if (a.bnr_z && !a.bn_sums) return BH_E_UNSUPPORTED;
    if (bni_table) {
        if (dgrad || bni_groups < 1 || a.N % bni_groups || ((long long)(a.N / bni_groups) * a.tiles_per_img) % 2) return BH_E_UNSUPPORTED;
        a.bni = bni_table; a.bni_groups = bni_groups; a.bni_relu = bni_relu; a.bni_ipg = a.N / bni_groups;
    }
    const int em = (a.bn_sums ? 1 : 0) | ((a.accumulate || a.res) ? 2 : 0) | (a.bnr_z ? 4 : 0) | ((a.bnr_z && a.bnr_relu && a.bnr_y) ? 8 : 0);
    typedef void (*kern_t)(C3Args);
    struct Row { int dgrad, bni, em; kern_t fn; };
#define PC_ROW(D, B, E) {D, B, E, conv3x3_pc_kernel<(D) != 0, (B) != 0, E>}
    static const Row rows[] = {PC_ROW(0, 0, 0), PC_ROW(0, 0, 1), PC_ROW(0, 0, 2), PC_ROW(0, 1, 0), PC_ROW(0, 1, 1),
                               PC_ROW(1, 0, 0), PC_ROW(1, 0, 1), PC_ROW(1, 0, 2), PC_ROW(1, 0, 5), PC_ROW(1, 0, 7), PC_ROW(1, 0, 13), PC_ROW(1, 0, 15)};
#undef PC_ROW
    constexpr int NROWS = sizeof(rows) / sizeof(rows[0]);
    kern_t fn = nullptr;
    for (int i = 0; i < NROWS; ++i)
        if (rows[i].dgrad == (dgrad ? 1 : 0) && rows[i].bni == (bni_table ? 1 : 0) && rows[i].em == em) fn = rows[i].fn;
    if (!fn) return BH_E_UNSUPPORTED;
    a.gx_total = (a.subtiles + 1) / 2;
    const long long total = (long long)a.gx_total * (a.Nn / 64);
    const int cus = 256;
    const int T = (int)((total + cus - 1) / cus);
    if (!force && (em & 14) && dgrad && T > 1) return BH_E_UNSUPPORTED;
    const int grid = (int)((total + T - 1) / T);
    a.tpb = T;
    a.NW = a.Nn / 32;
    if (bh_query("conv3x3_pc_kernel<%s,%s,%d>", dgrad ? "true" : "false", bni_table ? "true" : "false", em)) return BH_OK;
    static unsigned long long attr_devs = 0;
    if (bh_device_once(attr_devs)) {
        for (int i = 0; i < NROWS; ++i) {
            hipError_t e = hipFuncSetAttribute(reinterpret_cast<const void*>(rows[i].fn), hipFuncAttributeMaxDynamicSharedMemorySize, PC_LDS);
            if (e != hipSuccess) return (int)e;
        }
    }
    hipLaunchKernelGGL(fn, dim3(grid), dim3(768), PC_LDS, stream, a);
    BH_LAUNCH_CHECK();
    return BH_OK;
}
```

### bihome_amd/kernels.py

```python
import ctypes
import os

import torch

from ._lib import (AMAX_FLOATS, BN_DETERMINISTIC, DSAC_METHODS, F_DETERMINISTIC, GEOMETRY_FIELDS, ROUTE_DETERMINISTIC, ROUTE_WX3_PC, ROUTE_WX3_SHARED, BhBnIn, BhBnReduce, BhConvDesc,
                   BhPack3x3Job, check, lib)


def _p(t):
    return None if t is None else ctypes.c_void_p(t.data_ptr())


_DET_DEFAULT = os.environ.get("BIHOME_DETERMINISTIC", "0") == "1"
_DET_SCOPE = []


def set_deterministic(on=True):
    global _DET_DEFAULT
    prev, _DET_DEFAULT = _DET_DEFAULT, bool(on)
    return prev


def deterministic():
    return _DET_SCOPE[-1] if _DET_SCOPE else _DET_DEFAULT


class det_scope:

    def __init__(self, on):
        self.on = bool(on)

    def __enter__(self):
        _DET_SCOPE.append(self.on)
        return self

    def __exit__(self, *exc):
        _DET_SCOPE.pop()


def scoped_function(cls):
    fwd, bwd = cls.forward, cls.backward

    def forward(ctx, *a, **k):
        ctx.det = deterministic()
        return fwd(ctx, *a, **k)

    def backward(ctx, *g):
        with det_scope(ctx.det):
            return bwd(ctx, *g)
    cls.forward, cls.backward = staticmethod(forward), staticmethod(backward)
    return cls


def scoped_module(cls):
    init = cls.__init__

    def __init__(self, *a, **k):
        init(self, *a, **k)
        if not hasattr(self, "det"):
            self.det = deterministic()
    cls.__init__ = __init__
    for name in ("forward", "predict_homography"):
        fn = cls.__dict__.get(name)
        if fn is None:
            continue

        def wrap(fn):
            def method(self, *a, **k):
                with det_scope(self.det):
                    return fn(self, *a, **k)
            method.__name__, method.__doc__ = fn.__name__, fn.__doc__
            return method
        setattr(cls, name, wrap(fn))
    return cls


def _mark(d):
    _route_det(d)
    dp = getattr(d, "bh_packed", None)
    if dp is not None:
        _route_det(dp)
    return d


def _fdet():
    return F_DETERMINISTIC if deterministic() else 0


def _route_det(d):
    d.route = (d.route | ROUTE_DETERMINISTIC) if deterministic() else (d.route & ~ROUTE_DETERMINISTIC)
    return d


_raw_stream, _cur_device = torch._C._cuda_getCurrentRawStream, torch._C._cuda_getDevice


def _stream():
    return ctypes.c_void_p(_raw_stream(_cur_device()))


TIMING_DETAIL = False
TIMING = None


class _Timed:
    __slots__ = ("name", "flops", "bytes", "ev")

    def __init__(self, name, flops=0.0, nbytes=0.0):
        self.name, self.flops, self.bytes = name, flops, nbytes

    def __enter__(self):
        if TIMING is not None:
            self.ev = (torch.cuda.Event(enable_timing=True), torch.cuda.Event(enable_timing=True))
            self.ev[0].record()
        return self

    def __exit__(self, *exc):
        if TIMING is not None:
            self.ev[1].record()
            r = TIMING.setdefault(self.name, {"events": [], "flops": 0.0, "bytes": 0.0, "n": 0})
            r["events"].append(self.ev)
            r["flops"] += self.flops
            r["bytes"] += self.bytes
            r["n"] += 1


_VARIANT_CACHE = {}


def conv_variant(d, which, accumulate=False, bn_groups=0):
    key = (tuple(getattr(d, f) for f in GEOMETRY_FIELDS), which, bool(accumulate), int(bn_groups))
    v = _VARIANT_CACHE.get(key)
    if v is None:
        buf = ctypes.create_string_buffer(256)
        if d.precision == 4 and not d.a_bound:
            d = _with_layout(d, d.w_layout)
            d.a_bound = d.b_bound = 256
        check(lib.bh_conv_variant(ctypes.byref(d), {"fwd": 0, "dgrad": 1, "wgrad": 2, "wgrad_det": 3, "dgrad_bnr_z": 4, "dgrad_bnr_y": 5, "dgrad_colsum": 6}[which], int(bool(accumulate)), int(bn_groups),
                                  buf, 256), "bh_conv_variant")
        v = _VARIANT_CACHE[key] = buf.value.decode()
    return v


def _conv_variant(d, which, accumulate=False, bn_groups=0):
    if TIMING is None:
        return ""
    v = conv_variant(d, which, accumulate, bn_groups)
    if TIMING_DETAIL:
        v += " %s N%d %dx%d C%d->%d k%d s%d%s" % (which.split("_")[0], d.N, d.Hi, d.Wi, d.Ci, d.Co, d.kh, d.stride, " T" if d.transposed else "")
    return v


def _bni_name(v):
    import re
    if v.startswith("conv3x3_pc_kernel<"):
        return re.sub(r"<(false|true),false,", r"<\1,true,", v, count=1)
    return re.sub(r",false,(\d)((?:,(?:false|true))*)>", r",true,\1\2>", v, count=1)


def conv_flops(d):
    if d.transposed:
        return 2.0 * d.N * d.Hi * d.Wi * d.Ci * d.Co * d.kh * d.kw
    return 2.0 * d.N * d.Ho * d.Wo * d.Co * d.Ci * d.kh * d.kw


def _chk(t, dtype=torch.float32):
    if t is None:
        return
    if not t.is_cuda:
        raise RuntimeError("bihome_amd kernels need device tensors (got %s); there is no CPU path" % t.device)
    if t.dtype != dtype:
        raise TypeError("expected %s, got %s" % (dtype, t.dtype))
    if not t.is_contiguous():
        raise ValueError("tensor must be contiguous")


def h4pt_fwd(delta, size):
    _chk(delta)
    B = delta.shape[0]
    H64 = torch.empty(B, 9, dtype=torch.float64, device=delta.device)
    H32 = torch.empty(B, 3, 3, dtype=torch.float32, device=delta.device)
    check(lib.bh_h4pt_fwd(_p(delta), B, float(size), float(size), _p(H64), _p(H32), _stream()), "bh_h4pt_fwd")
    return H64, H32


def h4pt_bwd(delta, H64, gH, size):
    _chk(delta); _chk(H64, torch.float64); _chk(gH, torch.float64)
    B = delta.shape[0]
    gd = torch.empty(B, 4, 2, dtype=torch.float32, device=delta.device)
    check(lib.bh_h4pt_bwd(_p(delta), _p(H64), _p(gH), B, float(size), float(size), _p(gd), _stream()), "bh_h4pt_bwd")
    return gd


def dlt_fwd(pf, choice, n, P):
    _chk(pf); _chk(choice, torch.int64)
    B, _, h, w = pf.shape
    assert choice.shape == (B, n * P), (choice.shape, B, n, P)
    Hd = torch.empty(B * n, 3, 3, dtype=torch.float32, device=pf.device)
    dh = torch.empty(B * n, 4, 2, dtype=torch.float32, device=pf.device)
    eig = torch.empty(B * n, 96, dtype=torch.float64, device=pf.device)
    check(lib.bh_dlt_fwd(_p(pf), _p(choice), B, n, P, h, w, _p(Hd), _p(dh), _p(eig), _stream()), "bh_dlt_fwd")
    return Hd, dh, eig


def dlt_bwd(pf, choice, eig, g_delta, n, P, g_H=None):
    _chk(pf); _chk(choice, torch.int64); _chk(eig, torch.float64); _chk(g_delta); _chk(g_H, torch.float64)
    B, _, h, w = pf.shape
    g_pf = torch.zeros_like(pf)
    check(lib.bh_dlt_bwd(_p(pf), _p(choice), _p(eig), _p(g_delta), _p(g_H), B, n, P, h, w, _p(g_pf), _fdet(), _stream()), "bh_dlt_bwd")
    return g_pf


def _dsac_method(method, thr, beta):
    if method not in DSAC_METHODS:
        raise ValueError("unknown DSAC scoring method %r (built: %s)" % (method, ", ".join(DSAC_METHODS)))
    return DSAC_METHODS[method], float(thr), float(beta)


def dsac_scores_fwd(pf, Hd, n, method="repr_error", thr=0.0, beta=0.0):
    _chk(pf); _chk(Hd)
    B, _, h, w = pf.shape
    err = torch.empty(B, n, dtype=torch.float32, device=pf.device)
    scores = torch.empty_like(err)
    m, thr, beta = _dsac_method(method, thr, beta)
    check(lib.bh_dsac_score(_p(pf), _p(Hd), B, n, h, w, m, thr, beta, _p(err), None, _stream()), "bh_dsac_score")
    check(lib.bh_dsac_scores_fwd(_p(err), B, n, _p(scores), _stream()), "bh_dsac_scores_fwd")
    return scores, err


def dsac_scores_bwd(pf, Hd, scores, g_scores, n, method="repr_error", thr=0.0, beta=0.0):
    _chk(pf); _chk(Hd); _chk(scores); _chk(g_scores)
    B, _, h, w = pf.shape
    g_err = torch.empty_like(scores)
    g_Hd = torch.empty(B * n, 9, dtype=torch.float64, device=pf.device)
    g_pf = torch.zeros_like(pf)
    m, thr, beta = _dsac_method(method, thr, beta)
    check(lib.bh_dsac_scores_bwd(_p(pf), _p(Hd), _p(scores), _p(g_scores), B, n, h, w, m, thr, beta, _p(g_err), _p(g_Hd), _p(g_pf),
                                 _fdet(), _stream()), "bh_dsac_scores_bwd")
    return g_pf, g_Hd


def scale_samples_fwd(x, s, rep):
    _chk(x); _chk(s)
    Bn = s.numel()
    L = x.numel() // x.shape[0]
    y = torch.empty((Bn,) + tuple(x.shape[1:]), dtype=torch.float32, device=x.device)
    check(lib.bh_scale_samples_fwd(_p(x), _p(s), Bn, L, rep, _p(y), _stream()), "bh_scale_samples_fwd")
    return y


def scale_samples_bwd(g_y, x, s, rep, want_gx):
    _chk(g_y); _chk(x); _chk(s)
    Bn = s.numel()
    L = x.numel() // x.shape[0]
    g_x = torch.empty_like(g_y) if want_gx else None
    g_s = torch.empty(Bn, dtype=torch.float32, device=x.device)
    check(lib.bh_scale_samples_bwd(_p(g_y), _p(x), _p(s), Bn, L, rep, _p(g_x), _p(g_s), _fdet(), _stream()), "bh_scale_samples_bwd")
    return g_x, g_s


def dsac_score(pf, Hd, n, method="repr_error", thr=0.0, beta=0.0):
    _chk(pf); _chk(Hd)
    B, _, h, w = pf.shape
    err = torch.empty(B, n, dtype=torch.float32, device=pf.device)
    best = torch.empty(B, dtype=torch.int64, device=pf.device)
    m, thr, beta = _dsac_method(method, thr, beta)
    check(lib.bh_dsac_score(_p(pf), _p(Hd), B, n, h, w, m, thr, beta, _p(err), _p(best), _stream()), "bh_dsac_score")
    return err, best


def ransac_homography(pf, choice, thr=10.0, want_mask=False, check_range=True):
    _chk(pf); _chk(choice, torch.int64)
    if pf.requires_grad:
        raise RuntimeError("ransac_homography is an evaluation path without a gradient: call it under torch.no_grad() on a detached field")
    if pf.dim() != 4 or pf.shape[1] != 2:
        raise ValueError("pf must be [B,2,h,w], got %s" % (tuple(pf.shape),))
    B, _, h, w = pf.shape
    if choice.dim() != 3 or choice.shape[0] != B or choice.shape[2] != 4 or choice.shape[1] < 1:
        raise ValueError("choice must be [B,K,4] with K >= 1, got %s for B = %d" % (tuple(choice.shape), B))
    K = choice.shape[1]
    if check_range and choice.numel() and not torch.cuda.is_current_stream_capturing() and not bool(((choice >= 0) & (choice < h * w)).all()):
        raise ValueError("bihome_amd: ransac_homography choice holds indices outside [0, %d)" % (h * w))
    dev = pf.device
    hyp = torch.empty(B, K, 9, dtype=torch.float32, device=dev)
    count = torch.empty(B, K, dtype=torch.int32, device=dev)
    best = torch.empty(B, dtype=torch.int64, device=dev)
    n_inl = torch.empty(B, dtype=torch.int32, device=dev)
    mask = torch.empty(B, h, w, dtype=torch.uint8, device=dev) if want_mask else None
    work = torch.empty(B, 32, dtype=torch.float64, device=dev)
    Hd = torch.empty(B, 3, 3, dtype=torch.float32, device=dev)
    dh = torch.empty(B, 4, 2, dtype=torch.float32, device=dev)
# ... 349 lines not shown
    @property
    def shape(self):
        return self.z.shape

    def struct(self):
        b = BhBnIn()
        b.table, b.groups, b.relu = self.table.data_ptr(), int(self.groups), int(bool(self.relu))
        return b


def bn_fwd_coeffs(stats, gamma, beta, rmean, rvar, groups, rows, C, eps, momentum, amax=None):
    table = torch.empty((groups, C, 2), dtype=torch.float32, device=stats.device)
    check(lib.bh_bn_fwd_coeffs(_p(stats), _p(gamma), _p(beta), _p(rmean), _p(rvar), groups, rows, C, float(eps), float(momentum),
                               _p(table), _p(amax), _stream()), "bh_bn_fwd_coeffs")
    return table


def conv_fwd(x, w, bias, d, bn_sums=None, groups=1, res=None, relu=False, wpacked=None, amax=None, warp_src=None):
    _mark(d)
    if warp_src is not None:
        ws_ = warp_src
        _chk(ws_["src"]); _chk(ws_["H64"], torch.float64); _chk(ws_["cov"]); _chk(x); _chk(w); _chk(bias); _chk(bn_sums, torch.float64)
        B_, h_, w_ = ws_["src"].shape[0], ws_["src"].shape[-2], ws_["src"].shape[-1]
        if (res is None and not relu and wpacked is None and amax is None and d.Ci == 1 and d.precision == F16X2 and ws_["pool"] == 4
                and not d.transposed and d.kh == 7 and d.kw == 7 and d.stride == 2 and d.pad == 3 and d.Co == 64 and not d.out_nchw
                and d.Ho % 8 == 0 and d.Wo % 8 == 0 and d.Ho * 2 == d.Hi and d.Wo * 2 == d.Wi and d.N * (d.Ho // 8) * (d.Wo // 8) >= 256
                and w.is_contiguous() and os.environ.get("BIHOME_WARP_IN_STEM_FWD", "1") != "0"):
            y = torch.empty(conv_out_shape(d), dtype=torch.float32, device=x.device)
            with _Timed("stem7_fwd_f16_kernel<1,true>", conv_flops(d), 4.0 * (2 * x.numel() + y.numel() + w.numel())):
                rc = lib.bh_stem7_fwd_warp(_p(ws_["src"]), _p(ws_["H64"]), 4, _p(w), _p(bias), _p(y), ctypes.byref(d),
                                           _p(x) if ws_.get("want_image", True) else None, _p(ws_["cov"]), _p(bn_sums), groups, _stream())
            if rc != -2:
                check(rc, "bh_stem7_fwd_warp")
                ws_["done"] = ws_["filled"] = True
                return y
        with _Timed("warp_fwd_kernel", 0.0, 4.0 * (2 * x.numel() + (ws_["cov"].numel() if ws_["cov"] is not None else 0))):
            check(lib.bh_warp_fwd(_p(ws_["src"]), _p(ws_["H64"]), B_, 1, h_, w_, int(ws_["pool"]), _p(x), _p(ws_["cov"]), _fdet(), _stream()),
                  "bh_warp_fwd")
        ws_["filled"] = True
    if isinstance(x, BnOnLoad):
        bol, x = x, x.z
        _chk(x); _chk(bias); _chk(bn_sums, torch.float64)
        if d.kh == 1 and wpacked is None and res is None and not relu:
            _chk(w)
            y = torch.empty(conv_out_shape(d), dtype=torch.float32, device=x.device)
            bs = bol.struct()
            with _Timed((conv_variant(d, "fwd") + " bnin" + (" fwd N%d %dx%d C%d->%d k1" % (d.N, d.Hi, d.Wi, d.Ci, d.Co) if TIMING_DETAIL else "")) if TIMING is not None else "",
                        conv_flops(d), 4.0 * (x.numel() + y.numel() + w.numel())):
                check(lib.bh_conv_fwd_bnin(_p(x), _p(w), _p(bias), _p(y), ctypes.byref(d), _p(bn_sums), groups, ctypes.byref(bs), _stream()),
                      "bh_conv_fwd_bnin(1x1)")
            return y
        if wpacked is None or res is not None or relu:
            raise RuntimeError("BatchNorm-on-load needs the packed f32x3 3x3 forward")
        y = torch.empty(conv_out_shape(d), dtype=torch.float32, device=x.device)
        dp = getattr(d, "bh_packed", None) or _with_layout(d, packed_layout(d.precision))
        _route_det(dp)
        if dp.precision == F16X2:
            dp.a_bound = amax_of(bol).data_ptr()
        bs = bol.struct()
        with _Timed(_bni_name(_conv_variant(dp, "fwd", bn_groups=groups if bn_sums is not None else 0)) if TIMING is not None else "",
                    conv_flops(d), 4.0 * (x.numel() + y.numel() + w.numel())):
            check(lib.bh_conv_fwd_bnin(_p(x), _p(wpacked), _p(bias), _p(y), ctypes.byref(dp), _p(bn_sums), groups, ctypes.byref(bs),
                                       _stream()), "bh_conv_fwd_bnin")
        return y
    _chk(x); _chk(w); _chk(bias); _chk(res)
    y = torch.empty(conv_out_shape(d), dtype=torch.float32, device=x.device)
    if wpacked is not None:
        d, w = _route_det(getattr(d, "bh_packed", None) or _with_layout(d, packed_layout(d.precision))), wpacked
        if d.precision == F16X2:
            d.a_bound = amax_of(x).data_ptr()
    with _Timed(_conv_variant(d, "fwd", bn_groups=groups if bn_sums is not None else 0), conv_flops(d),
                4.0 * (x.numel() + y.numel() + w.numel())):
        if res is not None or relu:
            check(lib.bh_conv_fwd_act(_p(x), _p(w), _p(bias), _p(res), _p(y), ctypes.byref(d), int(bool(relu)), _stream()),
                  "bh_conv_fwd_act")
        elif amax is not None and bn_sums is None and wpacked is None:
            check(lib.bh_conv_fwd_amax(_p(x), _p(w), _p(bias), _p(y), ctypes.byref(d), _p(amax), _stream()), "bh_conv_fwd_amax")
            y._bh_amax = amax
        elif bn_sums is None:
            check(lib.bh_conv_fwd(_p(x), _p(w), _p(bias), _p(y), ctypes.byref(d), _stream()), "bh_conv_fwd")
        else:
            _chk(bn_sums, torch.float64)
            check(lib.bh_conv_fwd_bnstats(_p(x), _p(w), _p(bias), _p(y), ctypes.byref(d), _p(bn_sums), groups, _stream()),
                  "bh_conv_fwd_bnstats")
    return y


_STEM_WT = {}
_STEM_WT_DIRTY = set()


def invalidate_stem_tables():
    _STEM_WT_DIRTY.update(_STEM_WT.keys())


def _stem_dgrad_two_step(gy, w, d, wkey=None):
    cols = 49 * d.Ci
    ld = (cols + 3) // 4 * 4
    import weakref
    key = None if wkey is None else (id(wkey[0]), str(w.device), d.Ci)
    ent = _STEM_WT.get(key) if key is not None else None
    if ent is not None and (ent[2]() is not wkey[0] or ent[1].shape != (ld, 1, 1, d.Co)):
        ent = None
    if ent is None:
        wt = torch.zeros(ld, 1, 1, d.Co, dtype=torch.float32, device=w.device)
        wt[:cols, 0, 0, :] = w.reshape(d.Co, cols).t()
        if key is not None:
            _STEM_WT[key] = [wkey[1], wt, weakref.ref(wkey[0])]
            _STEM_WT_DIRTY.discard(key)
    else:
        wt = ent[1]
        if ent[0] != wkey[1] or key in _STEM_WT_DIRTY:
            wt[:cols, 0, 0, :] = w.reshape(d.Co, cols).t()
            ent[0] = wkey[1]
            _STEM_WT_DIRTY.discard(key)
    d1 = conv_desc(d.N, d.Ho, d.Wo, d.Co, ld, 1, 1, 0, precision=d.precision)
    tm = conv_fwd(gy, wt, None, d1)
    shape = (d.N, d.Hi, d.Wi, 1) if d.Ci == 1 else (d.N, d.Ci, d.Hi, d.Wi)
    gx = torch.empty(shape, dtype=torch.float32, device=gy.device)
    with _Timed("col2im_c1_kernel", 0.0, 4.0 * (tm.numel() + gx.numel())):
        check(lib.bh_col2im_c1(_p(tm), _p(gx), ctypes.byref(d), ld, _stream()), "bh_col2im_c1")
    return gx


def dgrad_bn_reduce_ok(d):
    return conv_variant(d, "dgrad").startswith(_C3_KERNELS)


def bias_grad_from_sums(sums, gbias, groups, C):
    _chk(sums, torch.float64); _chk(gbias)
    check(lib.bh_bias_grad_from_sums(_p(sums), _p(gbias), groups, C, _stream()), "bh_bias_grad_from_sums")


def conv_dgrad(gy, w, d, out=None, bn_reduce=None, wkey=None, wpacked=None, colsum=None, warp_sink=None):
    _chk(gy); _chk(w)
    _mark(d)
    if wpacked is not None:
        d, w = _route_det(getattr(d, "bh_packed", None) or _with_layout(d, packed_layout(d.precision))), wpacked
        if d.precision == F16X2:
            d.a_bound = amax_of(gy).data_ptr()
    if colsum is not None:
        assert out is None and bn_reduce is None
        _chk(colsum, torch.float64)
        out = torch.empty((d.N, d.Hi, d.Wi, d.Ci), dtype=torch.float32, device=gy.device)
        with _Timed(_conv_variant(d, "dgrad_colsum"), conv_flops(d), 4.0 * (gy.numel() + out.numel() + w.numel())):
            check(lib.bh_conv_dgrad_colsum(_p(gy), _p(w), _p(out), ctypes.byref(d), _p(colsum), _stream()), "bh_conv_dgrad_colsum")
        return out
    if bn_reduce is not None:
        acc = out is not None
        if out is None:
            out = torch.empty((d.N, d.Hi, d.Wi, d.Ci), dtype=torch.float32, device=gy.device)
        b = bn_reduce
        _chk(b["z"]); _chk(b["y"]); _chk(b["stats"], torch.float64); _chk(b["sums"], torch.float64)
        st = BhBnReduce(_p(b["z"]), _p(b["y"]), _p(b["stats"]), _p(b["gamma"]), _p(b["beta"]), float(b["eps"]), int(bool(b["relu"])))
        with _Timed(_conv_variant(d, "dgrad_bnr_y" if b["y"] is not None else "dgrad_bnr_z", acc, int(b["groups"])), conv_flops(d),
                    4.0 * (gy.numel() + out.numel() * ((3 if acc else 2) + (1 if b["y"] is not None else 0)) + w.numel())):
            check(lib.bh_conv_dgrad_bnreduce(_p(gy), _p(w), _p(out), ctypes.byref(d), int(acc), ctypes.byref(st), _p(b["sums"]),
                                             int(b["groups"]), _stream()), "bh_conv_dgrad_bnreduce")
        if acc:
            out._bh_amax = None
        return out
    if (out is None and not d.transposed and d.kh == 7 and d.stride == 2 and not d.out_nchw
            and (d.Ci == 1 or (d.Ci == 3 and d.in_nchw)) and d.Co % 4 == 0 and d.N * d.Ho * d.Wo >= 4096):
        if (d.Ci == 1 and d.Co == 64 and d.pad == 3 and d.Ho % 8 == 0 and d.Wo % 8 == 0 and d.Ho * 2 == d.Hi and d.Wo * 2 == d.Wi
                and w.is_contiguous() and os.environ.get("BIHOME_STEM_DGRAD_FUSED", "1") != "0"):
            if warp_sink is not None and not deterministic() and os.environ.get("BIHOME_WARP_IN_STEM_DGRAD", "1") != "0":
                ws_ = warp_sink
                _chk(ws_["src"]); _chk(ws_["H64"], torch.float64); _chk(ws_["gH"], torch.float64); _chk(ws_["g_cov"])
                with _Timed("stem7_dgrad_c1_kernel<true>", conv_flops(d), 4.0 * (gy.numel() + ws_["src"].numel())):
                    check(lib.bh_stem7_dgrad_c1_warp(_p(gy), _p(w), None, ctypes.byref(d), _p(ws_["src"]), _p(ws_["H64"]), _p(ws_["g_cov"]),
                                                     int(ws_["pool"]), _p(ws_["gH"]), _stream()), "bh_stem7_dgrad_c1_warp")
                ws_["done"] = True
                return None
            gx = torch.empty((d.N, d.Hi, d.Wi, 1), dtype=torch.float32, device=gy.device)
            with _Timed("stem7_dgrad_c1_kernel", conv_flops(d), 4.0 * (gy.numel() + gx.numel())):
                check(lib.bh_stem7_dgrad_c1(_p(gy), _p(w), _p(gx), ctypes.byref(d), _stream()), "bh_stem7_dgrad_c1")
            return gx
        return _stem_dgrad_two_step(gy, w, d, wkey)
    acc = out is not None
    if (not d.transposed and d.stride == 2 and not d.in_nchw and not d.out_nchw and d.Co % 4 == 0 and d.Ci % 4 == 0
            and d.Hi % 2 == 0 and d.Wi % 2 == 0 and d.Ho * 2 == d.Hi and d.Wo * 2 == d.Wi
            and ((d.kh == 3 and d.kw == 3 and d.pad == 1) or (d.kh == 1 and d.kw == 1 and d.pad == 0))):
        if out is None:
            out = torch.empty((d.N, d.Hi, d.Wi, d.Ci), dtype=torch.float32, device=gy.device)
        wpack = torch.empty(w.numel(), dtype=torch.float32, device=gy.device)
        nlaunch = 2 if d.kh == 3 else (2 + (0 if acc else 1))
        with _Timed("conv_dgrad_s2(%d kernels)" % nlaunch + (" N%d %dx%d C%d->%d k%d" % (d.N, d.Hi, d.Wi, d.Ci, d.Co, d.kh) if TIMING_DETAIL else ""),
                    conv_flops(d) / 4.0 * (1.0 if d.kh == 1 else 1.0), 4.0 * (gy.numel() + out.numel() * (2 if acc else 1) + 2 * w.numel())):
            check(lib.bh_conv_dgrad_s2(_p(gy), _p(w), _p(out), ctypes.byref(d), int(acc), _p(wpack), _stream()), "bh_conv_dgrad_s2")
        if acc:
            out._bh_amax = None
        return out
    if out is None:
        shape = (d.N, d.Ci, d.Hi, d.Wi) if d.in_nchw else (d.N, d.Hi, d.Wi, d.Ci)
        out = torch.empty(shape, dtype=torch.float32, device=gy.device)
    with _Timed(_conv_variant(d, "dgrad", acc), conv_flops(d), 4.0 * (gy.numel() + out.numel() * (2 if acc else 1) + w.numel())):
        check(lib.bh_conv_dgrad(_p(gy), _p(w), _p(out), ctypes.byref(d), int(acc), _stream()), "bh_conv_dgrad")
    if acc:
        out._bh_amax = None
    return out


def wgrad_det_bytes(d):
    _route_det(d)
    if d.precision == 4 and not d.a_bound:
        d = _with_layout(d, d.w_layout)
        d.a_bound = d.b_bound = 256
    return int(lib.bh_conv_wgrad_det_bytes(ctypes.byref(d)))


_STEM_WGRAD_WS = {}


def conv_wgrad(x, gy, gw, gbias, d, det_ws=None):
    _route_det(d)
    if d.precision == F16X2 and getattr(d, "bh_wx3", True):
        d.a_bound, d.b_bound = amax_of(x).data_ptr(), amax_of(gy).data_ptr()
    if isinstance(x, BnOnLoad):
        bol, x = x, x.z
        _chk(x); _chk(gy); _chk(gw); _chk(gbias)
        if d.kh == 1:
            bs = bol.struct()
            ws_ = det_ws if deterministic() else None
            with _Timed((conv_variant(d, "wgrad") + " bnin") if TIMING is not None else "", conv_flops(d), 4.0 * (x.numel() + gy.numel() + gw.numel())):
                check(lib.bh_conv_wgrad_bnin(_p(x), _p(gy), _p(gw), _p(gbias), ctypes.byref(d), _p(ws_), ws_.numel() * 4 if ws_ is not None else 0,
                                             ctypes.byref(bs), _stream()), "bh_conv_wgrad_bnin(1x1)")
            return
        need = wgrad_det_bytes(d)
        if det_ws is None or not (0 < need <= det_ws.numel() * 4):
            raise RuntimeError("BatchNorm-on-load needs the f32x3 weight gradient and its workspace")
        bs = bol.struct()
        with _Timed((_bni_name(conv_variant(d, "wgrad_det")) if TIMING is not None else ""), conv_flops(d),
                    4.0 * (x.numel() + gy.numel() + gw.numel())):
            check(lib.bh_conv_wgrad_bnin(_p(x), _p(gy), _p(gw), _p(gbias), ctypes.byref(d), _p(det_ws), det_ws.numel() * 4,
                                         ctypes.byref(bs), _stream()), "bh_conv_wgrad_bnin")
        return
    _chk(x); _chk(gy); _chk(gw); _chk(gbias)
    if d.kh == 7 and d.stride == 2 and d.Ci == 2 and d.in_nchw and gbias is None and gw.is_contiguous():
        need = lib.bh_stem7_wgrad_ws_bytes(ctypes.byref(d))
        if need:
            if torch.cuda.is_current_stream_capturing():
                ws = torch.empty(need // 4, dtype=torch.float32, device=x.device)
            else:
                key = (str(x.device), int(need), int(torch.cuda.current_stream(x.device).cuda_stream))
                ws = _STEM_WGRAD_WS.get(key)
                if ws is None:
                    if len(_STEM_WGRAD_WS) >= 8:
                        _STEM_WGRAD_WS.clear()
                    ws = _STEM_WGRAD_WS[key] = torch.empty(need // 4, dtype=torch.float32, device=x.device)
            with _Timed("stem7_wgrad_kernel<2>+stem7_wgrad_reduce_kernel<2>", conv_flops(d), 4.0 * (x.numel() + gy.numel() + gw.numel())):
                check(lib.bh_stem7_wgrad(_p(x), _p(gy), _p(gw), ctypes.byref(d), _p(ws), need, _stream()), "bh_stem7_wgrad")
            return
    det = deterministic()
    if det and det_ws is None:
        raise RuntimeError("deterministic mode: conv_wgrad needs a workspace (det_ws) - bh_conv_wgrad has only the atomic form")
    if det_ws is not None:
        need = wgrad_det_bytes(d)
        if det and not (0 < need <= det_ws.numel() * 4):
            raise RuntimeError("deterministic mode: workspace of %d bytes, %d needed" % (det_ws.numel() * 4, need))
        if 0 < need <= det_ws.numel() * 4:
            with _Timed((conv_variant(d, "wgrad_det") if TIMING is not None else ""), conv_flops(d), 4.0 * (x.numel() + gy.numel() + gw.numel())):
                check(lib.bh_conv_wgrad_det(_p(x), _p(gy), _p(gw), _p(gbias) if det else None, ctypes.byref(d), _p(det_ws),
                                            det_ws.numel() * 4, _stream()), "bh_conv_wgrad_det")
            if gbias is not None and not det:
                check(lib.bh_conv_bias_grad(_p(gy), _p(gbias), ctypes.byref(d), _stream()), "bh_conv_bias_grad")
            return
    with _Timed((conv_variant(d, "wgrad") if TIMING is not None else "") + (" N%d %dx%d C%d->%d k%d s%d%s" % (d.N, d.Hi, d.Wi, d.Ci, d.Co, d.kh, d.stride, " T" if d.transposed else "") if TIMING_DETAIL else ""), conv_flops(d), 4.0 * (x.numel() + gy.numel() + gw.numel())):
        check(lib.bh_conv_wgrad(_p(x), _p(gy), _p(gw), None, ctypes.byref(d), _stream()), "bh_conv_wgrad")
    if gbias is not None:
        with _Timed("bias_grad(colsum)", 0.0, 4.0 * gy.numel()):
            check(lib.bh_conv_bias_grad(_p(gy), _p(gbias), ctypes.byref(d), _stream()), "bh_conv_bias_grad")


BN_SUM_STRIDE = 16
BN_SUM_SLOTS = 1


def bn_stats_doubles(groups, C):
    return BN_SUM_SLOTS * groups * C * 2 * BN_SUM_STRIDE


def bn_stats_buffer(groups, C, device):
    return torch.zeros(lib.bh_bn_stats_doubles(groups, C), dtype=torch.float64, device=device)


def bn_fwd(x, gamma, beta, rmean, rvar, res, groups, eps, momentum, relu, training, stats=None, stats_ready=False, amax=None):
    _chk(x); _chk(res)
    C = gamma.numel() if gamma is not None else x.shape[-1]
    rows = x.numel() // C // groups
    y = torch.empty_like(x)
    if stats is None:
        stats = bn_stats_buffer(groups, C, x.device)
        stats_ready = False
    flags = (1 if relu else 0) | (2 if res is not None else 0) | (8 if stats_ready else 0) | (BN_DETERMINISTIC if deterministic() else 0)
    nb = 4.0 * x.numel() * ((2 if (training and not stats_ready) else 1) + 1 + (1 if res is not None else 0))
    with _Timed("bn_fwd(%d kernels)" % (2 if (training and not stats_ready) else 1) + (" g%d rows%d C%d" % (groups, rows, C) if TIMING_DETAIL else ""), 0.0, nb):
        check(lib.bh_bn_fwd(_p(x), _p(gamma), _p(beta), _p(rmean), _p(rvar), _p(res), _p(y), _p(stats), groups, rows, C,
                            float(eps), float(momentum), flags, 0 if training else 1, _p(amax), _stream()), "bh_bn_fwd")
    if amax is not None:
        y._bh_amax = amax
    return y, stats


def bn_bwd(gy, y, x, gamma, stats, rmean, rvar, groups, eps, relu, training, want_gres, ggamma=None, gbeta=None, beta=None,
           had_res=None, scratch=None, sums_ready=None, amax=None):
    _chk(gy); _chk(x)
    C = gamma.numel() if gamma is not None else x.shape[-1]
    rows = x.numel() // C // groups
    gx = torch.empty_like(x)
    gres = torch.empty_like(x) if want_gres else None
    if sums_ready is not None:
        scratch = sums_ready
    elif scratch is None:
        scratch = torch.empty(lib.bh_bn_scratch_doubles(groups, C), dtype=torch.float64, device=x.device)
    had_res = want_gres if had_res is None else had_res
    mask_from_x = relu and not had_res
    flags = ((1 if relu else 0) | (2 if want_gres else 0) | (4 if mask_from_x else 0) | (16 if sums_ready is not None else 0)
             | (BN_DETERMINISTIC if deterministic() else 0))
    passes = 1 if sums_ready is not None else 2
    nb = 4.0 * x.numel() * (passes * (2 + (1 if (relu and not mask_from_x) else 0)) + 1 + (1 if want_gres else 0))
    with _Timed("bn_bwd(%d kernels)" % (1 if sums_ready is not None else 3) + (" g%d rows%d C%d" % (groups, rows, C) if TIMING_DETAIL else ""), 0.0, nb):
        check(lib.bh_bn_bwd(_p(gy), _p(y), _p(x), _p(gamma), _p(beta), _p(stats), _p(gx), _p(gres), _p(ggamma), _p(gbeta),
                            _p(scratch), groups, rows, C, float(eps), flags, 0 if training else 1, _p(rmean), _p(rvar),
                            _p(amax), _stream()), "bh_bn_bwd")
    if amax is not None:
        gx._bh_amax = amax
    return gx, gres


def bn_stats(x, stats, groups, C):
    _chk(x); _chk(stats, torch.float64)
    rows = x.numel() // C // groups
    with _Timed("bn_stats_kernel", 0.0, 4.0 * x.numel()):
        check(lib.bh_bn_stats(_p(x), _p(stats), groups, rows, C, BN_DETERMINISTIC if deterministic() else 0, _stream()), "bh_bn_stats")
    return stats


class BnPooled:
    __slots__ = ("pooled", "idx", "shape")

    def __init__(self, pooled, idx, shape):
        self.pooled, self.idx, self.shape = pooled, idx, tuple(shape)


def bn_maxpool_fwd(x, gamma, beta, rmean, rvar, groups, eps, momentum, relu, training, stats, stats_ready, want_index=True, amax=None):
    _chk(x)
    N, Hi, Wi, C = x.shape
    y = torch.empty((N, (Hi - 1) // 2 + 1, (Wi - 1) // 2 + 1, C), dtype=torch.float32, device=x.device)
    idx = torch.empty(y.shape, dtype=torch.uint8, device=x.device) if want_index else None
    flags = (1 if relu else 0) | (8 if stats_ready else 0) | (BN_DETERMINISTIC if deterministic() else 0)
    with _Timed("bn_maxpool_fwd" + (" N%d %dx%d C%d" % (N, Hi, Wi, C) if TIMING_DETAIL else ""), 0.0, 4.0 * (x.numel() + y.numel()) + y.numel()):
        check(lib.bh_bn_maxpool_fwd(_p(x), _p(gamma), _p(beta), _p(rmean), _p(rvar), _p(y), _p(idx), _p(stats), groups, N, Hi, Wi, C,
                                    float(eps), float(momentum), flags, 0 if training else 1, _p(amax), _stream()), "bh_bn_maxpool_fwd")
    if amax is not None:
        y._bh_amax = amax
    return BnPooled(y, idx, x.shape)


class BnJoinPending:
    __slots__ = ("x", "stats", "mod")

    def __init__(self, x, stats, mod):
        self.x, self.stats, self.mod = x, stats, mod

    @property
    def shape(self):
        return self.x.shape


def bn_join_fwd(xa, xb, ma, mb, stats_a, stats_b, groups, relu, mom_a, mom_b, amax=None):
    _chk(xa); _chk(xb); _chk(stats_a, torch.float64); _chk(stats_b, torch.float64)
    C = ma.num_features
    rows = xa.numel() // C // groups
    y = torch.empty_like(xa)
    flags = (1 if relu else 0) | (BN_DETERMINISTIC if deterministic() else 0)
    with _Timed("bn_join_fwd" + (" g%d rows%d C%d" % (groups, rows, C) if TIMING_DETAIL else ""), 0.0, 12.0 * xa.numel()):
        check(lib.bh_bn_join_fwd(_p(xa), _p(xb), _p(ma.weight), _p(ma.bias), _p(ma.running_mean), _p(ma.running_var), _p(mb.weight), _p(mb.bias),
                                 _p(mb.running_mean), _p(mb.running_var), _p(stats_a), _p(stats_b), _p(y), groups, rows, C, float(ma.eps),
                                 float(mb.eps), float(mom_a), float(mom_b), flags, _p(amax), _stream()), "bh_bn_join_fwd")
    if amax is not None:
        y._bh_amax = amax
    return y


def bn_join_bwd(gy, y, xa, xb, ma, mb, stats_a, stats_b, groups, relu, train_a, train_b, amax_a=None, amax_b=None):
    _chk(gy); _chk(xa); _chk(xb)
    C = ma.num_features
    rows = xa.numel() // C // groups
    gxa, gxb = torch.empty_like(xa), torch.empty_like(xb)
    scratch = torch.empty(lib.bh_bn_join_scratch_doubles(groups, C), dtype=torch.float64, device=xa.device)
    flags = (1 if relu else 0) | (BN_DETERMINISTIC if deterministic() else 0)
    if os.environ.get("BIHOME_JOIN_REMASK", "1") != "0":
        with _Timed("bn_join_bwd(3 kernels)" + (" g%d rows%d C%d" % (groups, rows, C) if TIMING_DETAIL else ""), 0.0, 32.0 * xa.numel()):
            check(lib.bh_bn_join_bwd_remask(_p(gy), _p(xa), _p(xb), _p(ma.weight), _p(ma.bias), _p(mb.weight), _p(mb.bias), _p(stats_a),
                                            _p(stats_b), _p(gxa), _p(gxb),
                                            _p(ma.weight.grad) if train_a else None, _p(ma.bias.grad) if train_a else None,
                                            _p(mb.weight.grad) if train_b else None, _p(mb.bias.grad) if train_b else None, _p(scratch), groups,
                                            rows, C, float(ma.eps), float(mb.eps), flags, _p(amax_a), _p(amax_b), _stream()),
                  "bh_bn_join_bwd_remask")
    else:
      with _Timed("bn_join_bwd(3 kernels)" + (" g%d rows%d C%d" % (groups, rows, C) if TIMING_DETAIL else ""), 0.0, 40.0 * xa.numel()):
        check(lib.bh_bn_join_bwd(_p(gy), _p(y), _p(xa), _p(xb), _p(ma.weight), _p(mb.weight), _p(stats_a), _p(stats_b), _p(gxa), _p(gxb),
                                 _p(ma.weight.grad) if train_a else None, _p(ma.bias.grad) if train_a else None,
                                 _p(mb.weight.grad) if train_b else None, _p(mb.bias.grad) if train_b else None, _p(scratch), groups, rows, C,
                                 float(ma.eps), float(mb.eps), flags, _p(amax_a), _p(amax_b), _stream()), "bh_bn_join_bwd")
    if amax_a is not None:
        gxa._bh_amax = amax_a
    if amax_b is not None:
        gxb._bh_amax = amax_b
    return gxa, gxb


TAIL_ROUTE_VALU_FWD = 1
TAIL_ROUTE_LDS_MOMENTS = 2


def tail_fwd(x, w1, b1, gamma, beta, rmean, rvar, w2, b2, groups, hw, eps, momentum, training, route=0):
    _chk(x)
    N, h, w, Ci = x.shape
    Cm, Co = w1.shape[0], w2.shape[0]
    rows = N * h * w // groups
    out = torch.empty((N, Co, h, w), dtype=torch.float32, device=x.device)
    ws = torch.empty(lib.bh_tail_ws_doubles(groups, Ci, Cm), dtype=torch.float64, device=x.device)
    fl = 2.0 * N * h * w * Cm * (Ci + Co)
    with _Timed("tail_fwd(4 kernels)", fl, 4.0 * (x.numel() * (2 if training else 1) + out.numel())):
        check(lib.bh_tail_fwd(_p(x), _p(w1), _p(b1), _p(gamma), _p(beta), _p(rmean), _p(rvar), _p(w2), _p(b2), _p(out),
                              _p(ws), groups, rows, hw, Ci, Cm, Co, float(eps), float(momentum), 0 if training else 1,
                              int(route), _stream()), "bh_tail_fwd")
    return out, ws


def tail_bwd(gout, x, w1, b1, gamma, beta, w2, ws, rmean, rvar, groups, hw, eps, training, want_gx, gw1, ggamma, gbeta,
             gw2, gb2):
    _chk(gout); _chk(x)
    N, h, w, Ci = x.shape
    Cm, Co = w1.shape[0], w2.shape[0]
    rows = N * h * w // groups
    gx = torch.empty_like(x) if want_gx else None
    scratch = torch.empty(lib.bh_tail_scratch_floats(groups, Ci, Cm), dtype=torch.float32, device=x.device)
    fl = 2.0 * N * h * w * Cm * (3 * Ci + 2 * Co + Ci)
    with _Timed("tail_bwd(5 kernels)", fl, 4.0 * (x.numel() * 3 + gout.numel() * 3)):
        check(lib.bh_tail_bwd(_p(gout), _p(x), _p(w1), _p(b1), _p(gamma), _p(beta), _p(w2), _p(ws), _p(rmean), _p(rvar),
                              _p(gx), _p(gw1), _p(ggamma), _p(gbeta), _p(gw2), _p(gb2), _p(scratch), groups, rows, hw, Ci,
                              Cm, Co, float(eps), 0 if training else 1, _fdet(), _stream()), "bh_tail_bwd")
    return gx


def maxpool_fwd(x, want_index=True):
    _chk(x)
    N, Hi, Wi, C = x.shape
    y = torch.empty((N, (Hi - 1) // 2 + 1, (Wi - 1) // 2 + 1, C), dtype=torch.float32, device=x.device)
    idx = torch.empty(y.shape, dtype=torch.uint8, device=x.device) if want_index else None
    check(lib.bh_maxpool3s2_fwd(_p(x), _p(y), _p(idx), N, Hi, Wi, C, _stream()), "bh_maxpool3s2_fwd")
    rec = getattr(x, "_bh_amax", None)
    if rec is not None:
        y._bh_amax = rec
    return y, idx


class GradFrom1x1:
    __slots__ = ("gs", "w")
# ... 78 lines not shown
```

### bihome_amd/net.py

```python
import os
import weakref

import torch
import torch.nn as nn

from . import kernels as K
from . import plan as P


def to_kernel_layout_(module):
    for m in module.modules():
        if isinstance(m, (nn.Conv2d, nn.ConvTranspose2d)):
            if not m.weight.data.is_contiguous(memory_format=torch.channels_last):
                m.weight.data = m.weight.data.contiguous(memory_format=torch.channels_last)
    return module


def kview(w):
    if w.dim() == 2:
        return w
    v = w.permute(0, 2, 3, 1)
    if not v.is_contiguous():
        raise RuntimeError("conv weight is not in kernel (channels_last) layout; call net.to_kernel_layout_(module)")
    return v
# ... 275 lines not shown
            pf = ent[3]
    return K.conv_fwd(csrc, kview(wf), bf, d, res=slots[op.res] if op.res is not None else None, relu=op.relu, wpacked=pf,
                      warp_src=s.input_source if cop.src == 0 else None)


def _fw_conv(s, i, op, src):
    e, packer, groups, amax_next = op.extra, s.packer, s.groups, s.amax_next
    d = _conv_geometry(op.mod, src.shape, e["in_nchw"], e["out_nchw"], s.precision)
    w = e["weight_fn"](op.mod.weight) if e["weight_fn"] else op.mod.weight
    wk = kview(w)
    pk = None
    if packer is not None and e["weight_fn"] is None and d.bh_packs and id(op.mod.weight) in packer.entries:
        pk = packer.entries[id(op.mod.weight)]
    wsrc = s.input_source if op.src == 0 else None
    fused_stats = s.plan.fused_stats
    if i in fused_stats and d.N % groups == 0:
        b = fused_stats[i]
        out = K.conv_fwd(src, wk, op.mod.bias, d, bn_sums=_bn_stats_slice(s, b, d.Co), groups=groups,
                         wpacked=pk[1] if pk else None, warp_src=wsrc)
        s.ready.add(b)
    elif amax_next and pk is None and isinstance(op.mod, nn.ConvTranspose2d) and not e["out_nchw"]:
        out = K.conv_fwd(src, wk, op.mod.bias, d, amax=amax_next(), warp_src=wsrc)
    else:
        out = K.conv_fwd(src, wk, op.mod.bias, d, wpacked=pk[1] if pk else None, warp_src=wsrc)
    if s.save:
        ctx = s.ctx
        ctx.descs[i], ctx.weights[i] = d, wk
        ctx.wpacked[i] = pk[2] if pk else None
        ctx.wkeys[i] = (op.mod.weight, op.mod.weight._version)
    return out


def _bn_on_load_ok(s, i, op, src):
    m, groups, plan = op.mod, s.groups, s.plan
    if i in plan.bn_on_load_1x1 and i in s.ready and src.shape[0] % groups == 0 and (src.numel() // (m.num_features * groups)) % 128 == 0:
        return True
    if i in plan.bn_on_load and i in s.ready and src.shape[0] % groups == 0:
        cop = s.prog.ops[plan.consumer[op.dst]]
        cd = _conv_geometry(cop.mod, src.shape, False, cop.extra["out_nchw"], s.precision)
        return bool(cd.bh_packs and cd.bh_wx3 and 0 < cd.bh_wx3_bytes <= (DET_WS_BYTES if K.deterministic() else X3_WS_BYTES))
    return False


def _fw_bn(s, i, op, src):
    m, plan, groups, training, amax_next = op.mod, s.plan, s.groups, s.training, s.amax_next
    res = s.slots[op.res] if op.res is not None else None
    if i in plan.join_lower and src.shape[0] % groups == 0:
        st = _bn_stats_slice(s, i, m.num_features)
        if i not in s.ready:
            K.bn_stats(src, st, groups, m.num_features)
        out = K.BnJoinPending(src, st, m)
    elif i in plan.joins and isinstance(res, K.BnJoinPending) and src.shape[0] % groups == 0:
        st = _bn_stats_slice(s, i, m.num_features)
        if i not in s.ready:
            K.bn_stats(src, st, groups, m.num_features)
        out = K.bn_join_fwd(src, res.x, m, res.mod, st, res.stats, groups, op.relu, _momentum(m), _momentum(res.mod),
                            amax=amax_next() if amax_next else None)
        if s.save:
            s.ctx.joined[i] = plan.joins[i]
    else:
        if isinstance(res, K.BnJoinPending):
            lo, _ = K.bn_fwd(res.x, res.mod.weight, res.mod.bias, res.mod.running_mean, res.mod.running_var, None, groups, res.mod.eps,
                             _momentum(res.mod), False, training, stats=res.stats, stats_ready=True)
            res = s.slots[op.res] = lo
        st = _bn_stats_slice(s, i, m.num_features)
        if i in plan.bn_pool and src.dim() == 4 and src.shape[0] % groups == 0:
            out = K.bn_maxpool_fwd(src, m.weight, m.bias, m.running_mean, m.running_var, groups, m.eps, _momentum(m), op.relu,
                                   training, st, i in s.ready, want_index=s.save, amax=amax_next() if amax_next else None)
        elif _bn_on_load_ok(s, i, op, src):
            rec = amax_next() if amax_next else None
            table = K.bn_fwd_coeffs(st, m.weight, m.bias, m.running_mean, m.running_var, groups,
                                    src.numel() // (m.num_features * groups), m.num_features, m.eps, _momentum(m), amax=rec)
            out = K.BnOnLoad(src, table, groups, op.relu, amax=rec)
        else:
            out, st = K.bn_fwd(src, m.weight, m.bias, m.running_mean, m.running_var, res, groups, m.eps, _momentum(m), op.relu, training,
                               stats=st, stats_ready=i in s.ready, amax=amax_next() if (amax_next and m.num_features > 1) else None)
    if training:
        _count_batch(m, groups)
    if s.save:
        s.ctx.stats[i] = st
    return out


def _fw_tail(s, i, op, src):
    c1, bn, c2 = op.mod
    N, h, w, _ = src.shape
    out, ws = K.tail_fwd(src, kview(c1.weight), c1.bias, bn.weight, bn.bias, bn.running_mean, bn.running_var,
                         kview(c2.weight), c2.bias, s.groups, h * w, bn.eps, _momentum(bn), s.training)
    if s.training:
        _count_batch(bn, s.groups)
    if s.save:
        s.ctx.stats[i] = ws
    return out


def _fw_maxpool(s, i, op, src):
    if isinstance(src, K.BnPooled):
        out, idx = src.pooled, src.idx
    else:
        out, idx = K.maxpool_fwd(src, want_index=s.save)
    if s.save:
        s.ctx.stats[i] = idx
    return out


def _fw_gap(s, i, op, src):
    return K.gap_fwd(src)


_FW_ARMS = {"conv": _fw_conv, "bn": _fw_bn, "tail": _fw_tail, "maxpool": _fw_maxpool, "gap": _fw_gap}


def run_forward(prog, x, groups, training, save, precision=0, fold_cache=None, packer=None, input_source=None):
    precision = int(precision)
    if precision == K.F16X2 and (packer is None or not packer.f16):
        precision = 2
    if packer is not None:
        packer.refresh(training or save)
    plan = P.forward_plan(prog, training, groups, precision, packer, fold_cache is not None and not training and not save)
    s = _FwPass()
    s.prog, s.plan, s.groups, s.training, s.save, s.precision = prog, plan, groups, training, save, precision
    s.packer, s.fold_cache, s.input_source = packer, fold_cache, input_source
    s.slots = slots = {0: x}
    s.ready = set()
    s.ctx = ctx = Ctx() if save else None
    if save:
        ctx.groups, ctx.training, ctx.precision = groups, training, precision
    s.arena, amax_arena = _zero_arenas(plan.total, plan.nrec * K.AMAX_FLOATS, x.device)
    s.amax_next = iter(amax_arena.split(K.AMAX_FLOATS)).__next__ if plan.nrec else None
    folded, deferred, arms = plan.folded, plan.deferred, _FW_ARMS
    for i, op in enumerate(prog.ops):
        if i in deferred:
            continue
        if i in folded:
            slots[op.dst] = _fw_folded_conv(s, i, op)
        else:
            slots[op.dst] = arms[op.kind](s, i, op, slots.get(op.src))
    if save:
        ctx.slots = slots
    return slots[prog.ops[-1].dst], ctx


_SIDE_STREAMS = {}


def side_stream(device):
    key = torch.device(device).index if torch.device(device).index is not None else torch.cuda.current_device()
    if key not in _SIDE_STREAMS:
        _SIDE_STREAMS[key] = torch.cuda.Stream(device=key)
    return _SIDE_STREAMS[key]


class _BwPass:
    __slots__ = ("prog", "plan", "ctx", "slots", "grads", "bn_reduced", "red_arena", "amax_next", "want_wgrad", "want_input_grad",
                 "on_param_grad", "wgrad_stream", "main", "det_ws", "x3_ws", "input_sink")


def _contribute(grads, slot, g):
    if slot in grads:
        K.add_(grads[slot], g)
    else:
        grads[slot] = g


def _params_ready(s, *params):
    if s.on_param_grad is not None:
        for p in params:
            if p is not None:
                s.on_param_grad(p)


def _enqueue_wgrad(s, i, op, g, x, d):
    m, wgrad_stream, red_arena, bias_off = op.mod, s.wgrad_stream, s.red_arena, s.plan.bias_off
    gw = m.weight.grad if m.weight.dim() == 2 else kview(m.weight.grad)
    gb = m.bias.grad if (m.bias is not None and m.bias.requires_grad) else None
    has_gb = gb is not None
    if i in bias_off and has_gb:
        K.bias_grad_from_sums(red_arena[bias_off[i]:bias_off[i] + K.bn_stats_doubles(1, d.Co)], gb, 1, d.Co)
        gb = None
    ws = s.det_ws if s.det_ws is not None else (s.x3_ws if d.bh_wx3 else None)
    if wgrad_stream is None:
        d.route = (d.route | K.ROUTE_WX3_PC) & ~K.ROUTE_WX3_SHARED
    else:
        d.route = (d.route & ~K.ROUTE_WX3_PC) | K.ROUTE_WX3_SHARED
    if wgrad_stream is None:
        K.conv_wgrad(x, g, gw, gb, d, det_ws=ws)
    else:
        if s.ctx.precision == K.F16X2 and d.bh_wx3:
            K.amax_of(g)
            K.amax_of(x)
        ev = torch.cuda.Event()
        ev.record(s.main)
        g.record_stream(wgrad_stream)
        with torch.cuda.stream(wgrad_stream):
            wgrad_stream.wait_event(ev)
            K.conv_wgrad(x, g, gw, gb, d, det_ws=ws if d.bh_wx3 else None)
    _params_ready(s, m.weight, m.bias if has_gb else None)


def _bw_conv(s, i, op, g, x, need_src_grad):
    ctx, plan, grads = s.ctx, s.plan, s.grads
    d, wk = ctx.descs[i], ctx.weights[i]
    if s.want_wgrad and op.mod.weight.requires_grad and op.extra["weight_fn"] is None:
        _enqueue_wgrad(s, i, op, g, x, d)
    if not need_src_grad:
        return
    if i in plan.from_1x1 and op.src not in grads:
        grads[op.src] = K.GradFrom1x1(g, wk)
        return
    red = None
    if i in plan.fuse_bn:
        b = plan.fuse_bn[i]
        bop, bm = s.prog.ops[b], s.prog.ops[b].mod
        sums = s.red_arena[plan.red_off[b]:plan.red_off[b] + K.bn_stats_doubles(ctx.groups, bm.num_features)]
        red = dict(z=s.slots[bop.src], y=s.slots[bop.dst] if (bop.relu and bop.res is not None) else None,
                   stats=ctx.stats[b], gamma=bm.weight, beta=bm.bias, eps=bm.eps, relu=bop.relu, sums=sums,
                   groups=ctx.groups)
        s.bn_reduced[b] = sums
    if i in plan.fuse_bias and op.src not in grads and red is None:
        p = plan.fuse_bias[i]
        grads[op.src] = K.conv_dgrad(g, wk, d, wpacked=ctx.wpacked.get(i),
                                     colsum=s.red_arena[plan.bias_off[p]:plan.bias_off[p] + K.bn_stats_doubles(1, d.Ci)])
    elif op.src in grads:
        K.conv_dgrad(g, wk, d, out=grads[op.src], bn_reduce=red, wkey=ctx.wkeys[i], wpacked=ctx.wpacked.get(i))
    else:
        gsrc = K.conv_dgrad(g, wk, d, bn_reduce=red, wkey=ctx.wkeys[i], wpacked=ctx.wpacked.get(i),
                            warp_sink=s.input_sink if (op.src == 0 and red is None) else None)
        if gsrc is not None:
            grads[op.src] = gsrc


def _bw_bn_join(s, i, op, g, x, need_src_grad):
    ctx, slots, amax_next = s.ctx, s.slots, s.amax_next
    j = ctx.joined[i]
    lop, m, lm = s.prog.ops[j], op.mod, s.prog.ops[j].mod
    train_a = s.want_wgrad and m.weight.requires_grad
    train_b = s.want_wgrad and lm.weight.requires_grad
    xb = slots[lop.src]
    gxa, gxb = K.bn_join_bwd(g, slots[op.dst], x, xb, m, lm, ctx.stats[i], ctx.stats[j], ctx.groups, op.relu, train_a, train_b,
                             amax_a=amax_next() if amax_next else None, amax_b=amax_next() if amax_next else None)
    if train_a:
        _params_ready(s, m.weight, m.bias)
    if train_b:
        _params_ready(s, lm.weight, lm.bias)
    if need_src_grad:
        _contribute(s.grads, op.src, gxa)
    if (lop.src != 0) or s.want_input_grad:
        _contribute(s.grads, lop.src, gxb)


def _bw_bn(s, i, op, g, x, need_src_grad):
    m, ctx, amax_next = op.mod, s.ctx, s.amax_next
    train_w = s.want_wgrad and m.weight is not None and m.weight.requires_grad
    ggamma, gbeta = (m.weight.grad, m.bias.grad) if train_w else (None, None)
    amax = amax_next() if (amax_next and m.num_features > 1) else None
    gres = None
    if isinstance(g, K.GradFrom1x1):
        gx = K.bn_bwd_from_1x1(g, x, m.weight, m.bias, ctx.stats[i], ctx.groups, m.eps, op.relu, ggamma, gbeta, amax=amax)
    elif isinstance(g, K.PooledGrad):
        gx = K.bn_maxpool_bwd(g, x, m.weight, m.bias, ctx.stats[i], m.running_mean, m.running_var, ctx.groups, m.eps, op.relu,
                              ctx.training, ggamma, gbeta, amax=amax)
    else:
        yb = s.slots[op.dst]
        if isinstance(yb, (K.BnOnLoad, K.BnPooled)):
            yb = None
        gx, gres = K.bn_bwd(g, yb, x, m.weight, ctx.stats[i], m.running_mean, m.running_var, ctx.groups,
                            m.eps, op.relu, ctx.training, op.res is not None and ((op.res != 0) or s.want_input_grad),
                            ggamma, gbeta, beta=m.bias, had_res=op.res is not None, sums_ready=s.bn_reduced.get(i), amax=amax)
    if train_w and s.on_param_grad is not None:
        s.on_param_grad(m.weight)
        s.on_param_grad(m.bias)
    if need_src_grad:
        _contribute(s.grads, op.src, gx)
    if gres is not None:
        _contribute(s.grads, op.res, gres)


def _bw_tail(s, i, op, g, x, need_src_grad):
    ctx = s.ctx
    c1, bn, c2 = op.mod
    tr = s.want_wgrad and c1.weight.requires_grad
    N, h, w, _ = x.shape
    eval_b1 = tr and not ctx.training and c1.bias is not None and c1.bias.requires_grad
    gbeta0 = bn.bias.grad.clone() if eval_b1 else None
    gx = K.tail_bwd(g, x, kview(c1.weight), c1.bias, bn.weight, bn.bias, kview(c2.weight), ctx.stats[i],
                    bn.running_mean, bn.running_var, ctx.groups, h * w, bn.eps, ctx.training, need_src_grad,
                    kview(c1.weight.grad) if tr else None, bn.weight.grad if tr else None,
                    bn.bias.grad if tr else None, kview(c2.weight.grad) if tr else None,
                    c2.bias.grad if (tr and c2.bias is not None) else None)
    if eval_b1:
        with torch.no_grad():
            c1.bias.grad.add_((bn.bias.grad - gbeta0) * bn.weight * torch.rsqrt(bn.running_var + bn.eps))
    if tr:
        _params_ready(s, c2.weight, c2.bias, bn.weight, bn.bias, c1.weight, c1.bias)
    if need_src_grad:
        _contribute(s.grads, op.src, gx)


def _bw_maxpool(s, i, op, g, x, need_src_grad):
    if need_src_grad:
        if isinstance(x, K.BnPooled) and op.src not in s.grads:
            s.grads[op.src] = K.PooledGrad(g, s.ctx.stats[i])
        else:
            _contribute(s.grads, op.src, K.maxpool_bwd(s.ctx.stats[i], g, tuple(x.shape)))


def _bw_gap(s, i, op, g, x, need_src_grad):
    if need_src_grad:
        _contribute(s.grads, op.src, K.gap_bwd(g, tuple(x.shape)))


_BW_ARMS = {"conv": _bw_conv, "bn": _bw_bn, "tail": _bw_tail, "maxpool": _bw_maxpool, "gap": _bw_gap}


def run_backward(prog, ctx, gout, want_wgrad, want_input_grad, on_param_grad=None, wgrad_stream=None, det_ws=None, x3_ws=None, input_sink=None):
    main = torch.cuda.current_stream() if wgrad_stream is not None else None
    if wgrad_stream is not None:
        wgrad_stream.wait_stream(main)
    plan = P.backward_plan(prog, ctx, gout.shape, want_wgrad)
    s = _BwPass()
    s.prog, s.plan, s.ctx, s.slots, s.main, s.wgrad_stream = prog, plan, ctx, ctx.slots, main, wgrad_stream
    s.want_wgrad, s.want_input_grad, s.on_param_grad = want_wgrad, want_input_grad, on_param_grad
    s.det_ws, s.x3_ws, s.input_sink = det_ws, x3_ws, input_sink
    s.grads = grads = {prog.ops[-1].dst: gout}
    s.bn_reduced = {}
    s.red_arena, amax_arena = _zero_arenas(plan.total, plan.nrec * K.AMAX_FLOATS, gout.device)
    s.amax_next = iter(amax_arena.split(K.AMAX_FLOATS)).__next__ if plan.nrec else None
    ops, slots, joined, arms = prog.ops, ctx.slots, ctx.joined, _BW_ARMS
    for i in range(len(ops) - 1, -1, -1):
        op = ops[i]
        g = grads.pop(op.dst, None)
        if g is None:
            continue
        arm = _bw_bn_join if (op.kind == "bn" and i in joined) else arms[op.kind]
        arm(s, i, op, g, slots[op.src], (op.src != 0) or want_input_grad)
    if wgrad_stream is not None:
        main.wait_stream(wgrad_stream)
    return grads.get(0)


def _drop_pending_counters(module, *unused):
    for m in module.modules():
        if getattr(m, "_bh_pending_batches", 0):
            m._bh_pending_batches = 0


def install_counter_hooks(module):
    module.register_load_state_dict_pre_hook(lambda *a, **k: _drop_pending_counters(module))
    return module


def flush_counters(module):
    for m in module.modules():
        n = getattr(m, "_bh_pending_batches", 0)
        if n and getattr(m, "num_batches_tracked", None) is not None:
            m.num_batches_tracked += n
            m._bh_pending_batches = 0


class NetFunction(torch.autograd.Function):

    @staticmethod
    def forward(ctx, x, anchor, runner, groups, grad_mode=True):
        with K.det_scope(runner.det):
            return NetFunction._forward(ctx, x, anchor, runner, groups, grad_mode)

    @staticmethod
    def backward(ctx, g):
        with K.det_scope(ctx.runner.det):
            return NetFunction._backward(ctx, g)

    @staticmethod
    def _forward(ctx, x, anchor, runner, groups, grad_mode=True):
        need = grad_mode and (ctx.needs_input_grad[0] or ctx.needs_input_grad[1])
        training = runner.module.training
        if training or need:
            runner._fold.clear()
        fold = runner._fold if (runner.fold_bn and not training and not need) else None
        source = getattr(runner, "input_source", None)
        out, saved = run_forward(runner.prog, x, groups, training, save=need, precision=runner.precision, fold_cache=fold,
                                 packer=runner.packer_for(x.device) if fold is None else None, input_source=source)
        if source is not None and not source.get("filled"):
            raise RuntimeError("input_source: no conv reads the network's input directly - nobody made the warped image")
        ctx.runner, ctx.saved, ctx.want_x = runner, saved, ctx.needs_input_grad[0]
        return out

    @staticmethod
    def _backward(ctx, g):
        r = ctx.runner
        if r.flat is not None:
            r.flat.attach(g.device)
        hook = r.reducer.param_ready if r.reducer is not None else None
        side = side_stream(g.device) if (r.wgrad_on_side_stream and r.flat is not None and not K.deterministic()) else None
        if r.reducer is not None:
            r.reducer.wait_streams = [side] if side is not None else []
        gin = run_backward(r.prog, ctx.saved, g.contiguous(), want_wgrad=r.flat is not None, want_input_grad=ctx.want_x,
                           on_param_grad=hook, wgrad_stream=side, det_ws=r.det_workspace(g.device) if side is None else None,
                           x3_ws=r.x3_workspace(g.device), input_sink=getattr(r, "input_sink", None))
        ctx.saved = None
        return gin, None, None, None, None


_RUNNERS = weakref.WeakSet()


def trainable_runners(model):
    out = []
    for m in model.modules():
        if not (hasattr(m, "_build") and hasattr(m, "__dict__") and "_runner" in m.__dict__):
            continue
        if getattr(m, "fix_mask", False):
            continue
        if m._runner is None:
            to_kernel_layout_(m)
            m._runner = m._build()
        if isinstance(m._runner, Runner) and m._runner.flat is not None:
            out.append(m._runner)
    return out


def set_stream_overlap(on, model=None):
    mods = None if model is None else {id(m) for m in model.modules()}
    for r in list(_RUNNERS):
        if mods is None or id(r.module) in mods:
            r.wgrad_on_side_stream = bool(on)
    if model is not None:
        for m in model.modules():
            if hasattr(m, "prefetch_features"):
                m.prefetch_features = bool(on)


def invalidate_caches(model=None):
    mods = None if model is None else {id(m) for m in model.modules()}
    for r in list(_RUNNERS):
        if mods is not None and id(r.module) not in mods:
            continue
        r._fold.clear()
        if r._packer is not None:
            r._packer.invalidate()
    K.invalidate_stem_tables()


class Runner:

    def __init__(self, module, prog, trainable, precision="f32", fold_cache=None):
        _RUNNERS.add(self)
        self.module, self.prog = module, prog
        self.precision = K.PRECISION[str(precision).lower()]
        self.det = K.deterministic()
        params = [p for p in module.parameters() if p.requires_grad]
        self.flat = FlatGrads(params) if (trainable and params) else None
        self.anchor = params[0] if (trainable and params) else None
        self._dummy = None
        self.reducer = None
        self._fold = fold_cache if fold_cache is not None else {}
        self.fold_bn = True
        self.wgrad_on_side_stream = os.environ.get("BIHOME_OVERLAP", "1") != "0"
        self.use_packer = True
        self._packer = None
        self._det_ws = None

    def det_workspace(self, device):
        if not K.deterministic() or self.flat is None:
            return None
        if self._det_ws is None or self._det_ws.device != device or self._det_ws.numel() * 4 < DET_WS_BYTES:
            self._det_ws = torch.empty(DET_WS_BYTES // 4, dtype=torch.float32, device=device)
        return self._det_ws

    def x3_workspace(self, device):
        if K.deterministic():
            return self.det_workspace(device)
        if self.precision not in K.SPLIT_PIECES or self.flat is None:
            return None
        if self._det_ws is None or self._det_ws.device != device:
            self._det_ws = torch.empty(X3_WS_BYTES // 4, dtype=torch.float32, device=device)
        return self._det_ws

    def packer_for(self, device):
# ... 21 lines not shown
```

### bihome_amd/plan.py

```python
import torch.nn as nn

from . import kernels as K


class ProgramIndex:
    __slots__ = ("nops", "producer", "consumers", "users", "consumer", "last_consumer")

    def __init__(self, ops):
        self.nops = len(ops)
        self.producer = {op.dst: j for j, op in enumerate(ops)}
        self.consumers = {}
        self.consumer = {}
        for j, op in enumerate(ops):
            self.consumers.setdefault(op.src, []).append(j)
            if op.res is not None:
                self.consumers.setdefault(op.res, []).append(j)
            self.consumer.setdefault(op.src, j)
        self.users = {s: len(v) for s, v in self.consumers.items()}
        self.last_consumer = {s: v[0] for s, v in self.consumers.items()}


def packs_weight(op, device=None):
    m = op.mod
    return (op.kind == "conv" and isinstance(m, nn.Conv2d) and op.extra["weight_fn"] is None and m.kernel_size == (3, 3)
            and m.stride == (1, 1) and m.padding == (1, 1) and m.in_channels % 32 == 0 and m.out_channels % 32 == 0
            and (device is None or m.weight.device == device))


def packed_weight_ids(prog):
    return {id(op.mod.weight) for op in prog.ops if packs_weight(op)}


class ForwardPlan:
    __slots__ = ("nops", "fused_stats", "bn_on_load", "bn_on_load_1x1", "joins", "join_lower", "consumer", "bn_pool", "folded", "deferred",
                 "bn_off", "total", "nrec")


def forward_key(prog, training, groups, precision, packer, fold):
    return (bool(training), int(groups), int(precision), packer.serial if packer is not None else 0,
            len(packer.entries) if packer is not None else 0, bool(packer.f16) if packer is not None else False,
            tuple(op.mod.weight.requires_grad for op in prog.ops if op.kind == "conv"), bool(fold))


def plan_fused_stats(prog, ix, training):
    fused_stats = {}
    if training:
        ops = prog.ops
        for i, op in enumerate(ops):
            j = ix.producer.get(op.src)
            if (op.kind == "bn" and j is not None and ops[j].kind == "conv" and ix.users.get(op.src, 0) == 1
                    and not ops[j].extra["out_nchw"] and ops[j].mod.weight.dim() == 4):
                fused_stats[j] = i
    return fused_stats


def plan_bn_on_load_1x1(prog, ix, training, groups, precision, fused_stats):
    out = set()
    if training and groups <= 2 and int(precision) != 1:
        ops = prog.ops
        fused_bn = set(fused_stats.values())
        for i, op in enumerate(ops):
            j = ix.consumer.get(op.dst)
            if (op.kind == "bn" and op.res is None and i in fused_bn and ix.users.get(op.dst, 0) == 1 and j is not None
                    and ops[j].kind == "conv" and ops[j].src == op.dst and ops[j].extra["weight_fn"] is None
                    and not ops[j].extra["in_nchw"] and not ops[j].extra["out_nchw"] and isinstance(ops[j].mod, nn.Conv2d)
                    and ops[j].mod.kernel_size == (1, 1) and ops[j].mod.stride == (1, 1) and ops[j].mod.padding == (0, 0)
                    and ops[j].mod.in_channels % 32 == 0 and ops[j].mod.out_channels % 4 == 0
                    and min(ops[j].mod.in_channels, ops[j].mod.out_channels) <= 32 and ops[j].mod.weight.requires_grad):
                out.add(i)
    return out


def plan_bn_on_load(prog, ix, training, groups, precision, packed_ids, fused_stats):
    out = set()
    if training and packed_ids is not None and int(precision) in K.SPLIT_PIECES:
        ops = prog.ops
        fused_bn = set(fused_stats.values())
        for i, op in enumerate(ops):
            j = ix.consumer.get(op.dst)
            if (op.kind == "bn" and op.res is None and i in fused_bn and ix.users.get(op.dst, 0) == 1 and j is not None
                    and ops[j].kind == "conv" and ops[j].src == op.dst and ops[j].extra["weight_fn"] is None
                    and not ops[j].extra["in_nchw"] and id(ops[j].mod.weight) in packed_ids
                    and groups * op.mod.num_features * 8 <= 4096):
                out.add(i)
    return out


def plan_joins(prog, ix, training, bn_on_load):
    joins = {}
    if training:
        ops = prog.ops
        for i, op in enumerate(ops):
            j = ix.producer.get(op.res) if (op.kind == "bn" and op.res is not None) else None
            if (j is not None and ops[j].kind == "bn" and ops[j].res is None and not ops[j].relu
                    and ix.users.get(op.res, 0) == 1 and j not in bn_on_load and i not in bn_on_load
                    and op.mod.num_features == ops[j].mod.num_features and op.mod.num_features % 4 == 0
                    and op.mod.weight is not None and ops[j].mod.weight is not None):
                joins[i] = j
    return joins


def plan_bn_pool(prog, ix):
    ops = prog.ops
    return {i for i, op in enumerate(ops[:-1])
            if op.kind == "bn" and op.res is None and ops[i + 1].kind == "maxpool" and ops[i + 1].src == op.dst
            and op.mod.num_features % 4 == 0 and op.mod.num_features > 1 and ix.users.get(op.dst, 0) == 1}


def plan_folded(prog, ix, fold):
    folded = {}
    if fold:
        ops = prog.ops
        for i, op in enumerate(ops):
            j = ix.producer.get(op.src)
            if (op.kind == "bn" and j is not None and ops[j].kind == "conv" and ix.users.get(op.src, 0) == 1
                    and not ops[j].extra["out_nchw"]):
                folded[i] = j
    return folded


def plan_forward_arenas(prog, groups, precision):
    bn_off, total = {}, 0
    for i, op in enumerate(prog.ops):
        if op.kind == "bn":
            bn_off[i] = total
            total += K.bn_stats_doubles(groups, op.mod.num_features)
    nrec = 0
    if int(precision) == K.F16X2:
        nrec = max(1, sum(1 for op in prog.ops if op.kind == "bn" or (op.kind == "conv" and isinstance(op.mod, nn.ConvTranspose2d))))
    return bn_off, total, nrec


def make_forward_plan(prog, training, groups, precision, packed_ids=None, fold=False):
    ix = prog.index()
    p = ForwardPlan()
    p.nops = ix.nops
    p.fused_stats = plan_fused_stats(prog, ix, training)
    p.bn_on_load_1x1 = plan_bn_on_load_1x1(prog, ix, training, groups, precision, p.fused_stats)
    p.bn_on_load = plan_bn_on_load(prog, ix, training, groups, precision, packed_ids, p.fused_stats)
    p.consumer = ix.consumer if (training and packed_ids is not None and int(precision) in K.SPLIT_PIECES) else None
    p.joins = plan_joins(prog, ix, training, p.bn_on_load)
    p.join_lower = set(p.joins.values())
    p.bn_pool = plan_bn_pool(prog, ix)
    p.folded = plan_folded(prog, ix, fold)
    p.deferred = set(p.folded.values())
    p.bn_off, p.total, p.nrec = plan_forward_arenas(prog, groups, precision)
    return p


def forward_plan(prog, training, groups, precision, packer, fold):
    key = forward_key(prog, training, groups, precision, packer, fold)
    p = prog.fw_plans.get(key)
    if p is None:
        if len(prog.fw_plans) > 16:
            prog.fw_plans.clear()
        p = prog.fw_plans[key] = make_forward_plan(prog, training, groups, precision,
                                                   set(packer.entries) if packer is not None else None, fold)
    assert p.nops == len(prog.ops), "Program grew after it first ran"
    prog.last_forward_plan = p
    return p


FROM_1X1_KC = (16,)


class BackwardPlan:
    __slots__ = ("nops", "consumed_by", "fuse_bn", "fuse_bias", "from_1x1", "red_off", "bias_off", "total", "nrec")


def backward_key(prog, ctx, gout_shape, want_wgrad):
    return (bool(ctx.training), bool(want_wgrad), int(ctx.groups), tuple(gout_shape), frozenset(ctx.joined.items()), frozenset(ctx.descs),
            ctx.precision,
            tuple((op.mod.weight.requires_grad, op.mod.bias is not None and op.mod.bias.requires_grad) for op in prog.ops if op.kind == "conv"))


def plan_fuse_bn(prog, ix, ctx):
    fuse_bn = {}
    if ctx.training:
        ops, descs = prog.ops, ctx.descs
        for j, op in enumerate(ops):
            b = ix.producer.get(op.src)
            if (op.kind == "conv" and b is not None and ops[b].kind == "bn" and ix.last_consumer.get(op.src) == j
                    and j in descs and descs[j].bh_reduce_ok and descs[j].N % ctx.groups == 0 and b not in ctx.joined):
                fuse_bn[j] = b
    return fuse_bn


def plan_fuse_bias(prog, ix, ctx, want_wgrad, fuse_bn):
    fuse_bias = {}
    if want_wgrad:
        ops, descs = prog.ops, ctx.descs
        for j, op in enumerate(ops):
            p = ix.producer.get(op.src)
            if (op.kind == "conv" and j not in fuse_bn and p is not None and ops[p].kind == "conv" and ix.users.get(op.src, 0) == 1
                    and j in descs and p in descs and descs[j].bh_reduce_ok):
                pm = ops[p].mod
                if pm.bias is not None and pm.bias.requires_grad and pm.weight.requires_grad and ops[p].extra["weight_fn"] is None:
                    fuse_bias[j] = p
    return fuse_bias


def plan_from_1x1(prog, ix, ctx, fuse_bn):
    from_1x1 = set()
    if ctx.training:
        ops = prog.ops
        for j, op in enumerate(ops):
            b = ix.producer.get(op.src)
            m = op.mod
            if (op.kind == "conv" and b is not None and ops[b].kind == "bn" and ops[b].res is None and b not in ctx.joined
                    and ix.users.get(op.src, 0) == 1 and j not in fuse_bn and isinstance(m, nn.Conv2d) and m.kernel_size == (1, 1)
                    and m.stride == (1, 1) and m.padding == (0, 0) and op.extra["weight_fn"] is None and m.out_channels in FROM_1X1_KC
                    and ops[b].mod.num_features % 4 == 0 and 256 % (ops[b].mod.num_features // 4) == 0
                    and not op.extra["in_nchw"] and not op.extra["out_nchw"]):
                from_1x1.add(j)
    return from_1x1


def plan_backward_arenas(prog, ctx, fuse_bn, fuse_bias):
    red_off, bias_off, total = {}, {}, 0
    for j, p in fuse_bias.items():
        bias_off[p] = total
        total += K.bn_stats_doubles(1, ctx.descs[j].Ci)
    for b in fuse_bn.values():
        red_off[b] = total
        total += K.bn_stats_doubles(ctx.groups, prog.ops[b].mod.num_features)
    nrec = max(1, sum(1 for op in prog.ops if op.kind == "bn")) if ctx.precision == K.F16X2 else 0
    return red_off, bias_off, total, nrec


def make_backward_plan(prog, ctx, want_wgrad):
    ix = prog.index()
    p = BackwardPlan()
    p.nops = ix.nops
    p.consumed_by = ix.users
    p.fuse_bn = plan_fuse_bn(prog, ix, ctx)
    p.fuse_bias = plan_fuse_bias(prog, ix, ctx, want_wgrad, p.fuse_bn)
    p.from_1x1 = plan_from_1x1(prog, ix, ctx, p.fuse_bn)
    p.red_off, p.bias_off, p.total, p.nrec = plan_backward_arenas(prog, ctx, p.fuse_bn, p.fuse_bias)
    return p


def backward_plan(prog, ctx, gout_shape, want_wgrad):
    key = backward_key(prog, ctx, gout_shape, want_wgrad)
    p = prog.bw_plans.get(key)
    if p is None:
        p = prog.bw_plans[key] = make_backward_plan(prog, ctx, want_wgrad)
    assert p.nops == len(prog.ops), "Program grew after it first ran"
    prog.last_backward_plan = p
    return p
```

### include/bihome.h

```cpp
#ifndef BIHOME_H
#define BIHOME_H

#include <stdint.h>

#ifdef __cplusplus
extern "C" {
#endif

#define BH_OK 0
#define BH_E_BADARG (-1)
#define BH_E_UNSUPPORTED (-2)

int bh_version(void);
int bh_device_arch(char* buf, int buflen);

#define BH_F_DETERMINISTIC 1
#define BH_BN_DETERMINISTIC 32
int bh_probe_mfma_bf16(int random_operands, float* sink_dev, double* tflops, void* stream);
int bh_probe_mfma_f32(int random_operands, float* sink_dev, double* tflops, void* stream);


int bh_h4pt_fwd(const float* delta, int B, float W, float H, double* H64, float* H32, void* stream);
int bh_h4pt_bwd(const float* delta, const double* H64, const double* gH, int B, float W, float H,
                float* gdelta, void* stream);

int bh_dlt_fwd(const float* pf, const int64_t* choice, int B, int n, int P, int h, int w,
               float* Hdlt, float* delta_hat, double* eig, void* stream);
int bh_dlt_bwd(const float* pf, const int64_t* choice, const double* eig, const float* g_delta, const double* g_Hdlt,
               int B, int n, int P, int h, int w, float* g_pf, int flags, void* stream);

enum { BH_DSAC_REPR_ERROR = 0, BH_DSAC_INLIERS = 1, BH_DSAC_SOFT_INLIERS = 2 };
int bh_dsac_score(const float* pf, const float* Hdlt, int B, int n, int h, int w, int method, float thr, float beta,
                  float* score, int64_t* best, void* stream);
int bh_dsac_scores_fwd(const float* err, int B, int n, float* scores, void* stream);
int bh_dsac_scores_bwd(const float* pf, const float* Hdlt, const float* scores, const float* g_scores, int B, int n, int h, int w,
                       int method, float thr, float beta, float* g_err, double* g_Hdlt, float* g_pf, int flags, void* stream);

int bh_ransac_homography(const float* pf, const int64_t* choice, int B, int K, int h, int w, float thr, float* hyp, int32_t* count,
                         int64_t* best, int32_t* n_inl, uint8_t* mask, double* work, float* H, float* delta_hat, void* stream);

int bh_homography_refine_lm(const float* pf, const uint8_t* mask, int B, int h, int w, int iters, float* H, float* delta_hat,
                            double* work, void* stream);

int bh_warp_fwd(const float* img, const double* H64, int B, int C, int h, int w, int pool,
                float* out, float* cov, int flags, void* stream);
int bh_warp_bwd(const float* img, const double* H64, const float* g_out, const float* g_cov,
                int B, int C, int h, int w, int pool, double* gH, int flags, void* stream);
int bh_photo_warp_fwd(const float* img, const double* Hp64, const float* origin, int B, int C, int Hi, int Wi, int P, float* out,
                      int flags, void* stream);
int bh_photo_warp_bwd(const float* img, const double* Hp64, const float* origin, const float* g_out, int B, int C, int Hi, int Wi,
                      int P, double* gH, int flags, void* stream);
size_t bh_warp_bwd_img_scratch_doubles(int B, int C, int h, int w, int flags);
int bh_warp_bwd_img(const double* H64, const float* g_out, int B, int C, int h, int w, float* g_img, double* scratch, int flags,
                    void* stream);

int bh_triplet_l1_fwd(const float* f1, const float* f2, const float* f1w, const float* f2w,
                      const float* m1w, const float* m2w, const float* m1, const float* m2,
                      int B, int hw, int C, float* M1, float* M2, double* numden, int flags, void* stream);
int bh_bihome_loss_fwd(const double* numden, const double* H1, const double* H2, int B, float mu,
                       float* loss4, void* stream);
int bh_bihome_loss_bwd(const float* g_loss, const float* f1, const float* f2, const float* f1w,
                       const float* f2w, const float* m1w, const float* m2w, const float* m1,
                       const float* m2, const float* M1, const float* M2, const double* numden,
                       const double* H1, const double* H2, int B, int hw, int C, float mu,
                       float* g_f1w, float* g_f2w, float* g_m1w, float* g_m2w,
                       double* gH1, double* gH2, void* stream);

int bh_oneline_loss_fwd(const float* f1, const float* f2, const float* f1w, const float* m1w, const float* m2, int B, int hw,
                        int C, float margin, int rep, const float* sample_w, float* T, double* numden, float* per_sample,
                        float* loss, int flags, void* stream);
int bh_oneline_loss_bwd(const float* g_loss, const float* f2, const float* f1w, const float* m1w, const float* m2,
                        const float* T, const double* numden, int B, int hw, int C, int rep, const float* sample_w,
                        float* g_f1w, float* g_m1w, void* stream);
int bh_zhang_triplet_fwd(const float* f1, const float* f2, const float* f1w, const float* f2w, const float* m1w, const float* m2w,
                         const float* m1, const float* m2, int B, int hw, float margin, int hinge, float* T1, float* T2, double* numden,
                         void* stream);
int bh_zhang_triplet_bwd(const float* g_loss, const float* f1, const float* f2, const float* f1w, const float* f2w, const float* m1w,
                         const float* m2w, const float* m1, const float* m2, const float* T1, const float* T2, const double* numden, int B,
                         int hw, int hinge, float* g_f1, float* g_f2, float* g_f1w, float* g_f2w, float* g_m1w, float* g_m2w,
                         float* g_m1, float* g_m2, void* stream);
int bh_mask_fwd(const float* y, const float* f, int N, int P, float strength, float* m, float* g, float* smax, int* imax, void* stream);
int bh_mask_bwd(const float* y, const float* f, const float* m, const float* smax, const int* imax, const float* g_m, const float* g_g,
                int N, int P, float strength, float* g_y, float* g_f, void* stream);
int bh_scale_samples_fwd(const float* x, const float* s, int Bn, long long L, int rep, float* y, void* stream);
int bh_scale_samples_bwd(const float* g_y, const float* x, const float* s, int Bn, long long L, int rep, float* g_x, float* g_s,
                         int flags, void* stream);

typedef struct {
    int N, Hi, Wi, Ci;
    int Ho, Wo, Co;
    int kh, kw, stride, pad;
    int transposed;
    int in_nchw;
    int out_nchw;
    int precision;
    int w_layout;
    int route;
    const float* a_bound;
    const float* b_bound;
} bh_conv_desc;
#define BH_AMAX_FLOATS 512
int bh_absmax(const float* x, long long n, float* record, void* stream);
#define BH_ROUTE_GENERIC_CONV 1
#define BH_ROUTE_HALO_SMALL 2
#define BH_ROUTE_NO_STEM7 4
#define BH_ROUTE_WGRAD_GENERIC 8
#define BH_ROUTE_WGRAD_3TAP 16
#define BH_ROUTE_C3_ONE_SUBTILE 32
#define BH_ROUTE_C3_ONE_POSITION 64
#define BH_ROUTE_DETERMINISTIC 128
#define BH_ROUTE_C3_PC 512
#define BH_ROUTE_C3_TILE_WG 256
#define BH_ROUTE_WX3_PC 1024
#define BH_ROUTE_WX3_SHARED 2048
#define BH_ROUTE_GEMM_X3 4096

typedef struct {
    const float* w;
    float* pf;
    float* pd;
    int Co, Ci;
    int split;
    int reserved;
} bh_pack3x3_job;
int bh_conv3x3_pack(const bh_pack3x3_job* jobs_dev, int njobs, void* stream);
int bh_conv3x3_pack_f16(const bh_pack3x3_job* jobs_dev, int njobs, void* stream);

int bh_conv_variant(const bh_conv_desc* d, int which, int accumulate, int bn_groups, char* buf, int n);

#ifdef BH_TUNING
int bh_debug_force_tile(int bm, int bn);
#endif
int bh_conv_fwd(const float* x, const float* w, const float* bias, float* y, const bh_conv_desc* d, void* stream);
int bh_conv_fwd_amax(const float* x, const float* w, const float* bias, float* y, const bh_conv_desc* d, float* amax_y, void* stream);

int bh_conv_fwd_act(const float* x, const float* w, const float* bias, const float* res, float* y, const bh_conv_desc* d,
                    int relu, void* stream);
typedef struct {
    const float* table;
    int groups;
    int relu;
} bh_bn_in;
int bh_bn_fwd_coeffs(const double* stats, const float* gamma, const float* beta, float* running_mean, float* running_var, int groups,
                     int rows, int C, float eps, float momentum, float* table, float* amax_y, void* stream);
int bh_conv_fwd_bnin(const float* x, const float* w, const float* bias, float* y, const bh_conv_desc* d, double* sums, int groups,
                     const bh_bn_in* bni, void* stream);
int bh_conv_wgrad_bnin(const float* x, const float* gy, float* gw, float* gbias, const bh_conv_desc* d, float* ws, long long ws_bytes,
                       const bh_bn_in* bni, void* stream);
int bh_conv_fwd_bnstats(const float* x, const float* w, const float* bias, float* y, const bh_conv_desc* d, double* sums,
                        int groups, void* stream);
int bh_conv_dgrad(const float* gy, const float* w, float* gx, const bh_conv_desc* d, int accumulate, void* stream);
int bh_conv_dgrad_s2(const float* gy, const float* w, float* gx, const bh_conv_desc* d, int accumulate, float* wpack,
                     void* stream);
typedef struct bh_bn_reduce {
    const float* z;
    const float* y;
    const double* stats;
    const float* gamma;
    const float* beta;
    float eps;
    int relu;
} bh_bn_reduce;
int bh_conv_dgrad_bnreduce(const float* gy, const float* w, float* gx, const bh_conv_desc* d, int accumulate,
                           const bh_bn_reduce* bnr, double* sums, int groups, void* stream);
int bh_conv_dgrad_colsum(const float* gy, const float* w, float* gx, const bh_conv_desc* d, double* sums, void* stream);
int bh_bias_grad_from_sums(const double* sums, float* gbias, int groups, int C, void* stream);
int bh_col2im_c1(const float* Tm, float* gx, const bh_conv_desc* d, int ldT, void* stream);
int bh_stem7_dgrad_c1(const float* gy, const float* w, float* gx, const bh_conv_desc* d, void* stream);
int bh_stem7_dgrad_c1_warp(const float* gy, const float* w, float* gx, const bh_conv_desc* d, const float* src, const double* H64,
                           const float* g_cov, int pool, double* gH, void* stream);
int bh_stem7_fwd_warp(const float* src, const double* H64, int pool, const float* w, const float* bias, float* y, const bh_conv_desc* d,
                      float* warped, float* cov, double* bn_sums, int groups, void* stream);
size_t bh_stem7_wgrad_ws_bytes(const bh_conv_desc* d);
int bh_stem7_wgrad(const float* x, const float* gy, float* gw, const bh_conv_desc* d, float* ws, size_t ws_bytes, void* stream);
int bh_conv_wgrad(const float* x, const float* gy, float* gw, float* gbias, const bh_conv_desc* d, void* stream);
long long bh_conv_wgrad_det_bytes(const bh_conv_desc* d);
int bh_conv_wgrad_det(const float* x, const float* gy, float* gw, float* gbias, const bh_conv_desc* d, float* ws, long long ws_bytes,
                      void* stream);
int bh_conv_bias_grad(const float* gy, float* gbias, const bh_conv_desc* d, void* stream);

int bh_bn_stats_doubles(int groups, int C);
int bh_bn_scratch_doubles(int groups, int C);
int bh_bn_fwd(const float* x, const float* gamma, const float* beta, float* running_mean, float* running_var,
              const float* res, float* y, double* stats, int groups, int rows, int C, float eps, float momentum,
              int flags, int use_running, float* amax_y, void* stream);
int bh_bn_bwd(const float* gy, const float* y, const float* x, const float* gamma, const float* beta, const double* stats,
              float* gx, float* gres, float* ggamma, float* gbeta, double* scratch,
              int groups, int rows, int C, float eps, int flags, int use_running,
              const float* running_mean, const float* running_var, float* amax_gx, void* stream);

int bh_bn_maxpool_fwd(const float* x, const float* gamma, const float* beta, float* running_mean, float* running_var, float* y,
                      unsigned char* idx, double* stats, int groups, int N, int Hi, int Wi, int C, float eps, float momentum, int flags,
                      int use_running, float* amax_y, void* stream);
int bh_bn_maxpool_bwd(const float* gy, const unsigned char* idx, const float* x, const float* gamma, const float* beta, const double* stats,
                      float* gx, float* ggamma, float* gbeta, double* scratch, int groups, int N, int Hi, int Wi, int C, float eps, int flags,
                      int use_running, const float* running_mean, const float* running_var, float* amax_gx, void* stream);
int bh_bn_bwd_from_1x1(const float* gs, const float* w, int KC, const float* x, const float* gamma, const float* beta, const double* stats,
                       float* gx, float* ggamma, float* gbeta, double* scratch, int groups, int rows, int C, float eps, int flags,
                       float* amax_gx, void* stream);
int bh_bn_stats(const float* x, double* stats, int groups, int rows, int C, int flags, void* stream);
int bh_bn_join_scratch_doubles(int groups, int C);
int bh_bn_join_fwd(const float* xa, const float* xb, const float* gamma_a, const float* beta_a, float* rmean_a, float* rvar_a,
                   const float* gamma_b, const float* beta_b, float* rmean_b, float* rvar_b, const double* stats_a, const double* stats_b,
                   float* y, int groups, int rows, int C, float eps_a, float eps_b, float momentum_a, float momentum_b, int flags,
                   float* amax_y, void* stream);
int bh_bn_join_bwd(const float* gy, const float* y, const float* xa, const float* xb, const float* gamma_a, const float* gamma_b,
                   const double* stats_a, const double* stats_b, float* gxa, float* gxb, float* ggamma_a, float* gbeta_a, float* ggamma_b,
                   float* gbeta_b, double* scratch, int groups, int rows, int C, float eps_a, float eps_b, int flags, float* amax_gxa,
                   float* amax_gxb, void* stream);
int bh_bn_join_bwd_remask(const float* gy, const float* xa, const float* xb, const float* gamma_a, const float* beta_a, const float* gamma_b,
                          const float* beta_b, const double* stats_a, const double* stats_b, float* gxa, float* gxb, float* ggamma_a,
                          float* gbeta_a, float* ggamma_b, float* gbeta_b, double* scratch, int groups, int rows, int C, float eps_a, float eps_b,
                          int flags, float* amax_gxa, float* amax_gxb, void* stream);

int bh_tail_ws_doubles(int groups, int Ci, int Cm);
int bh_tail_scratch_floats(int groups, int Ci, int Cm);
#define BH_TAIL_ROUTE_VALU_FWD 1
#define BH_TAIL_ROUTE_LDS_MOMENTS 2
int bh_tail_fwd(const float* x, const float* w1, const float* b1, const float* gamma, const float* beta,
                float* running_mean, float* running_var, const float* w2, const float* b2, float* out, double* ws,
                int groups, int rows, int hw, int Ci, int Cm, int Co, float eps, float momentum, int use_running,
                int route, void* stream);
int bh_tail_bwd(const float* gout, const float* x, const float* w1, const float* b1, const float* gamma,
                const float* beta, const float* w2, const double* ws, const float* running_mean,
                const float* running_var, float* gx, float* gw1, float* ggamma, float* gbeta, float* gw2, float* gb2,
                float* scratch, int groups, int rows, int hw, int Ci, int Cm, int Co, float eps, int use_running,
                int flags, void* stream);

int bh_synth_pairs(const float* images, const int* img_idx, const float* origin, const double* Hpatch, const float* photo,
                   int B, int n_images, int Hs, int Ws, int P, float mean, float std, float* patch1, float* patch2,
                   void* stream);

int bh_synth_image(const float* images, const int* img_idx, const float* photo, int B, int n_images, int Hs, int Ws, float mean,
                   float std, float* image1, void* stream);

int bh_maxpool3s2_fwd(const float* x, float* y, unsigned char* argmax, int N, int Hi, int Wi, int C, void* stream);
int bh_maxpool3s2_bwd(const unsigned char* argmax, const float* gy, float* gx, int N, int Hi, int Wi, int C, void* stream);
int bh_gap_fwd(const float* x, float* y, int N, int HW, int C, void* stream);
int bh_gap_bwd(const float* gy, float* gx, int N, int HW, int C, void* stream);
int bh_add(const float* a, const float* b, float* out, int64_t n, void* stream);

#ifdef __cplusplus
}
#endif
#endif
```

Baseline: 5122.

## Store ReLU-masked gradient from dgrad epilogue so BN backward skips reading y

When a dgrad conv already reduces BatchNorm sums for a BN+residual+ReLU block, its epilogue now applies the ReLU mask from the saved output before storing the gradient. The following BN backward can then drop its read of y and skip writing a separate residual gradient, reusing the masked gy tensor directly. This removes one full-activation read and one full-activation write per such block in exchange for extra kernel template instantiations. It also relies on the residual gradient aliasing the stored gradient buffer.

```diff
diff --git a/bihome_amd/_lib.py b/bihome_amd/_lib.py
--- a/bihome_amd/_lib.py
+++ b/bihome_amd/_lib.py
@@ -148,6 +148,7 @@
 
 lib = _load()
 ROUTE_DETERMINISTIC, BN_DETERMINISTIC, F_DETERMINISTIC = 128, 32, 1
+BN_GY_MASKED, BNR_STORE_MASKED = 64, 2
 DSAC_METHODS = {"repr_error": 0, "inliers_ratio": 1, "soft_inliers_ratio": 2}
 ROUTE_C3_PC = 512
 ROUTE_WX3_PC = 1024
diff --git a/bihome_amd/csrc/bn.hip b/bihome_amd/csrc/bn.hip
--- a/bihome_amd/csrc/bn.hip
+++ b/bihome_amd/csrc/bn.hip
@@ -758,14 +758,19 @@
               float* gres, float* ggamma, float* gbeta, double* scratch, int groups, int rows, int C, float eps, int flags,
               int use_running, const float* running_mean, const float* running_var, float* amax_gx, void* stream) {
     BnGeom g;
-    if (!gy || !x || !gx || !stats || !scratch || ((flags & 1) && !(flags & 4) && !y)) return BH_E_BADARG;
+    if (!gy || !x || !gx || !stats || !scratch || ((flags & 1) && !(flags & (4 | BH_BN_GY_MASKED)) && !y)) return BH_E_BADARG;
     if ((flags & 4) && (flags & 2)) return BH_E_BADARG;
+    if ((flags & BH_BN_GY_MASKED) && (!(flags & 16) || !(flags & 1) || (flags & 4) || gres || C == 1)) return BH_E_BADARG;
     if (C == 1) return amax_gx ? BH_E_UNSUPPORTED : bn1_bwd(gy, y, x, gamma, beta, stats, gx, gres, ggamma, gbeta, scratch, groups, rows, eps, flags, use_running,
                                running_mean, running_var, bh_stream(stream));
     if (!bn_geom(groups, rows, C, g, (flags & BH_BN_DETERMINISTIC) ? 1 : 0)) return BH_E_UNSUPPORTED;
     hipStream_t s = bh_stream(stream);
     if (flags & 16) {
         if (use_running) return BH_E_BADARG;
+        if (flags & BH_BN_GY_MASKED) {
+            flags &= ~1;
+            y = nullptr;
+        }
         hipLaunchKernelGGL(bn_bwd_apply_kernel, dim3(apply_blocks(g), groups), dim3(256), 0, s, gy, y, x, gamma, beta,
                            (const float4*)nullptr, gx, gres, g, flags, stats, (const double*)scratch, eps, ggamma, gbeta,
                            reinterpret_cast<unsigned*>(amax_gx));
diff --git a/bihome_amd/csrc/capi.hip b/bihome_amd/csrc/capi.hip
--- a/bihome_amd/csrc/capi.hip
+++ b/bihome_amd/csrc/capi.hip
@@ -37,7 +37,7 @@
 }
 
 int bh_conv_variant(const bh_conv_desc* d, int which, int accumulate, int with_bnstats , char* buf, int n) {
-    if (!d || !buf || n < 2 || which < 0 || which > 6) return BH_E_BADARG;
+    if (!d || !buf || n < 2 || which < 0 || which > 7) return BH_E_BADARG;
     BhQuery q;
     q.name[0] = 0; q.len = 0;
     float* p = reinterpret_cast<float*>(static_cast<uintptr_t>(256));
@@ -51,7 +51,7 @@
     else if (which == 6) rc = bh_conv_dgrad_colsum(p, p, p, d, pd, nullptr);
     else {
         bh_bn_reduce bnr = {};
-        bnr.z = p; bnr.y = which == 5 ? p : nullptr; bnr.stats = pd; bnr.gamma = p; bnr.beta = p; bnr.eps = 1e-5f; bnr.relu = 1;
+        bnr.z = p; bnr.y = which != 4 ? p : nullptr; bnr.stats = pd; bnr.gamma = p; bnr.beta = p; bnr.eps = 1e-5f; bnr.relu = which == 7 ? (1 | BH_BNR_STORE_MASKED) : 1;
         rc = bh_conv_dgrad_bnreduce(p, p, p, d, accumulate, &bnr, pd, with_bnstats > 0 ? with_bnstats : 1, nullptr);
     }
     bh_query_ctx = nullptr;
diff --git a/bihome_amd/csrc/conv3x3.hip b/bihome_amd/csrc/conv3x3.hip
--- a/bihome_amd/csrc/conv3x3.hip
+++ b/bihome_amd/csrc/conv3x3.hip
@@ -79,11 +79,12 @@
         } else {
             const bool rd_old = a.accumulate, rd_res = a.res != nullptr, rd_z = a.bnr_z != nullptr;
             const bool rd_y = rd_z && a.bnr_relu && a.bnr_y != nullptr;
+            const bool store_masked = rd_y && (a.bnr_relu & BH_BNR_STORE_MASKED);
             const float c_x0 = -r_mean * r_invstd;
             auto body = [&](auto EXTRA, auto ZMODE) {
                 constexpr bool HAS_EXTRA = decltype(EXTRA)::value;
                 constexpr int ZM = decltype(ZMODE)::value;
-                float ext[HAS_EXTRA ? TM : 1][16], zin[ZM > 0 ? TM : 1][16], yin[ZM == 2 ? TM : 1][16];
+                float ext[HAS_EXTRA ? TM : 1][16], zin[ZM > 0 ? TM : 1][16], yin[ZM >= 2 ? TM : 1][16];
                 if constexpr (HAS_EXTRA) {
                     const __amdgpu_buffer_rsrc_t rsR = __builtin_amdgcn_make_buffer_rsrc(const_cast<float*>(rd_res ? a.res : a.Out), 0, a.out_bytes, 0x00020000);
 #pragma unroll
@@ -104,7 +105,7 @@
                         for (int r = 0; r < 16; ++r)
                             zin[i][r] = __builtin_bit_cast(float, __builtin_amdgcn_raw_buffer_load_b32(rsZ, rowoff[r >> 2], C3_SOFF(i, r), 0));
                 }
-                if constexpr (ZM == 2) {
+                if constexpr (ZM >= 2) {
                     const __amdgpu_buffer_rsrc_t rsY = __builtin_amdgcn_make_buffer_rsrc(const_cast<float*>(a.bnr_y), 0, a.out_bytes, 0x00020000);
 #pragma unroll
                     for (int i = 0; i < TM; ++i)
@@ -123,6 +124,12 @@
                             float v = acc[i][r] + bv;
                             if constexpr (HAS_EXTRA) v += ext[i][r];
                             if (a.relu) v = fmaxf(v, 0.0f);
+                            if constexpr (ZM == 3) {
+                                if (!(yin[i][r] > 0.f)) v = 0.f;
+                                __builtin_amdgcn_raw_buffer_store_b32(__builtin_bit_cast(unsigned, v), rsO, rowoff[rq], C3_SOFF(i, r), 0);
+                                q1 += v; q2 = __builtin_fmaf(v, __builtin_fmaf(zin[i][r], r_invstd, c_x0), q2);
+                                continue;
+                            }
                             __builtin_amdgcn_raw_buffer_store_b32(__builtin_bit_cast(unsigned, v), rsO, rowoff[rq], C3_SOFF(i, r), 0);
                             if constexpr (ZM > 0) {
                                 const float zv = zin[i][r];
@@ -140,10 +147,11 @@
             };
             using T_ = std::true_type; using F_ = std::false_type;
             using Z0 = std::integral_constant<int, 0>; using Z1 = std::integral_constant<int, 1>; using Z2 = std::integral_constant<int, 2>;
+            using Z3 = std::integral_constant<int, 3>;
             if (rd_old || rd_res) {
-                if (!rd_z) body(T_{}, Z0{}); else if (!rd_y) body(T_{}, Z1{}); else body(T_{}, Z2{});
+                if (!rd_z) body(T_{}, Z0{}); else if (!rd_y) body(T_{}, Z1{}); else if (!store_masked) body(T_{}, Z2{}); else body(T_{}, Z3{});
             } else {
-                if (!rd_z) body(F_{}, Z0{}); else if (!rd_y) body(F_{}, Z1{}); else body(F_{}, Z2{});
+                if (!rd_z) body(F_{}, Z0{}); else if (!rd_y) body(F_{}, Z1{}); else if (!store_masked) body(F_{}, Z2{}); else body(F_{}, Z3{});
             }
         }
 #undef C3_SOFF
@@ -728,6 +736,7 @@
     if (bn_sums && (groups < 1 || d->N % groups || (!dgrad && bnr) || (dgrad && !bnr && accumulate))) return BH_E_BADARG;
     if (bnr) {
         if (!bnr->z || !bnr->stats) return BH_E_BADARG;
+        if ((bnr->relu & BH_BNR_STORE_MASKED) && (!(bnr->relu & 1) || !bnr->y)) return BH_E_BADARG;
         a.bnr_z = bnr->z; a.bnr_y = bnr->y; a.bnr_stats = bnr->stats; a.bnr_gamma = bnr->gamma; a.bnr_beta = bnr->beta;
         a.bnr_eps = bnr->eps; a.bnr_relu = bnr->relu; a.bnr_rows = (d->N / groups) * d->Hi * d->Wi;
     }
diff --git a/bihome_amd/csrc/conv3x3_pc.hip b/bihome_amd/csrc/conv3x3_pc.hip
--- a/bihome_amd/csrc/conv3x3_pc.hip
+++ b/bihome_amd/csrc/conv3x3_pc.hip
@@ -382,7 +382,8 @@
         const __amdgpu_buffer_rsrc_t rsR = __builtin_amdgcn_make_buffer_rsrc(const_cast<float*>(a.res ? a.res : a.Out), 0, a.out_bytes, 0x00020000);
         const __amdgpu_buffer_rsrc_t rsZ = __builtin_amdgcn_make_buffer_rsrc(const_cast<float*>(a.bnr_z ? a.bnr_z : a.Out), 0, a.out_bytes, 0x00020000);
         const __amdgpu_buffer_rsrc_t rsY = __builtin_amdgcn_make_buffer_rsrc(const_cast<float*>(a.bnr_y ? a.bnr_y : a.Out), 0, a.out_bytes, 0x00020000);
-        constexpr bool stats = EM & 1, use_ext = EM & 2, rd_z = EM & 4, rd_y = EM & 8;
+        constexpr bool stats = EM & 1, use_ext = EM & 2, rd_z = EM & 4, rd_y = EM & 8, st_masked = EM & 16;
+        static_assert(!st_masked || (stats && rd_z && rd_y), "the masked store rides on the BatchNorm sums with a saved output");
         const bool rd_res = a.res != nullptr;
         const unsigned nn4 = (unsigned)a.Nn * 4u;
 #ifdef BH_TUNING
@@ -500,6 +501,13 @@
                 float v = __builtin_ldexpf(accv[e], kout) + bb[e];
                 if constexpr (use_ext) v += oo[e];
                 v = do_relu ? fmaxf(v, 0.0f) : v;
+                if constexpr (st_masked) {
+                    v = (y4[e] > 0.f) ? v : 0.f;
+                    out[e] = v;
+                    S1[e] += (double)v;
+                    S2[e] = __builtin_fma((double)v, (double)__builtin_fmaf(z4[e], isd[e], cx[e]), S2[e]);
+                    continue;
+                }
                 out[e] = v;
                 if constexpr (stats) {
                     float vm = v, t = v;
@@ -596,12 +604,14 @@
         if (dgrad || bni_groups < 1 || a.N % bni_groups || ((long long)(a.N / bni_groups) * a.tiles_per_img) % 2) return BH_E_UNSUPPORTED;
         a.bni = bni_table; a.bni_groups = bni_groups; a.bni_relu = bni_relu; a.bni_ipg = a.N / bni_groups;
     }
-    const int em = (a.bn_sums ? 1 : 0) | ((a.accumulate || a.res) ? 2 : 0) | (a.bnr_z ? 4 : 0) | ((a.bnr_z && a.bnr_relu && a.bnr_y) ? 8 : 0);
+    const int em = (a.bn_sums ? 1 : 0) | ((a.accumulate || a.res) ? 2 : 0) | (a.bnr_z ? 4 : 0) | ((a.bnr_z && a.bnr_relu && a.bnr_y) ? 8 : 0) |
+                   ((a.bnr_z && a.bnr_y && (a.bnr_relu & 1) && (a.bnr_relu & BH_BNR_STORE_MASKED)) ? 16 : 0);
     typedef void (*kern_t)(C3Args);
     struct Row { int dgrad, bni, em; kern_t fn; };
 #define PC_ROW(D, B, E) {D, B, E, conv3x3_pc_kernel<(D) != 0, (B) != 0, E>}
     static const Row rows[] = {PC_ROW(0, 0, 0), PC_ROW(0, 0, 1), PC_ROW(0, 0, 2), PC_ROW(0, 1, 0), PC_ROW(0, 1, 1),
-                               PC_ROW(1, 0, 0), PC_ROW(1, 0, 1), PC_ROW(1, 0, 2), PC_ROW(1, 0, 5), PC_ROW(1, 0, 7), PC_ROW(1, 0, 13), PC_ROW(1, 0, 15)};
+                               PC_ROW(1, 0, 0), PC_ROW(1, 0, 1), PC_ROW(1, 0, 2), PC_ROW(1, 0, 5), PC_ROW(1, 0, 7), PC_ROW(1, 0, 13), PC_ROW(1, 0, 15),
+                               PC_ROW(1, 0, 29), PC_ROW(1, 0, 31)};
 #undef PC_ROW
     constexpr int NROWS = sizeof(rows) / sizeof(rows[0]);
     kern_t fn = nullptr;
diff --git a/bihome_amd/kernels.py b/bihome_amd/kernels.py
--- a/bihome_amd/kernels.py
+++ b/bihome_amd/kernels.py
@@ -3,7 +3,7 @@
 
 import torch
 
-from ._lib import (AMAX_FLOATS, BN_DETERMINISTIC, DSAC_METHODS, F_DETERMINISTIC, GEOMETRY_FIELDS, ROUTE_DETERMINISTIC, ROUTE_WX3_PC, ROUTE_WX3_SHARED, BhBnIn, BhBnReduce, BhConvDesc,
+from ._lib import (AMAX_FLOATS, BN_DETERMINISTIC, BN_GY_MASKED, BNR_STORE_MASKED, DSAC_METHODS, F_DETERMINISTIC, GEOMETRY_FIELDS, ROUTE_DETERMINISTIC, ROUTE_WX3_PC, ROUTE_WX3_SHARED, BhBnIn, BhBnReduce, BhConvDesc,
                    BhPack3x3Job, check, lib)
 
 
@@ -136,7 +136,7 @@
         if d.precision == 4 and not d.a_bound:
             d = _with_layout(d, d.w_layout)
             d.a_bound = d.b_bound = 256
-        check(lib.bh_conv_variant(ctypes.byref(d), {"fwd": 0, "dgrad": 1, "wgrad": 2, "wgrad_det": 3, "dgrad_bnr_z": 4, "dgrad_bnr_y": 5, "dgrad_colsum": 6}[which], int(bool(accumulate)), int(bn_groups),
+        check(lib.bh_conv_variant(ctypes.byref(d), {"fwd": 0, "dgrad": 1, "wgrad": 2, "wgrad_det": 3, "dgrad_bnr_z": 4, "dgrad_bnr_y": 5, "dgrad_colsum": 6, "dgrad_bnr_ym": 7}[which], int(bool(accumulate)), int(bn_groups),
                                   buf, 256), "bh_conv_variant")
         v = _VARIANT_CACHE[key] = buf.value.decode()
     return v
@@ -792,8 +792,12 @@
             out = torch.empty((d.N, d.Hi, d.Wi, d.Ci), dtype=torch.float32, device=gy.device)
         b = bn_reduce
         _chk(b["z"]); _chk(b["y"]); _chk(b["stats"], torch.float64); _chk(b["sums"], torch.float64)
-        st = BhBnReduce(_p(b["z"]), _p(b["y"]), _p(b["stats"]), _p(b["gamma"]), _p(b["beta"]), float(b["eps"]), int(bool(b["relu"])))
-        with _Timed(_conv_variant(d, "dgrad_bnr_y" if b["y"] is not None else "dgrad_bnr_z", acc, int(b["groups"])), conv_flops(d),
+        masked = bool(b.get("store_masked"))
+        if masked and not (b["relu"] and b["y"] is not None):
+            raise RuntimeError("conv_dgrad: store_masked needs the ReLU and the saved output of the BatchNorm")
+        st = BhBnReduce(_p(b["z"]), _p(b["y"]), _p(b["stats"]), _p(b["gamma"]), _p(b["beta"]), float(b["eps"]),
+                        int(bool(b["relu"])) | (BNR_STORE_MASKED if masked else 0))
+        with _Timed(_conv_variant(d, ("dgrad_bnr_ym" if masked else "dgrad_bnr_y") if b["y"] is not None else "dgrad_bnr_z", acc, int(b["groups"])), conv_flops(d),
                     4.0 * (gy.numel() + out.numel() * ((3 if acc else 2) + (1 if b["y"] is not None else 0)) + w.numel())):
             check(lib.bh_conv_dgrad_bnreduce(_p(gy), _p(w), _p(out), ctypes.byref(d), int(acc), ctypes.byref(st), _p(b["sums"]),
                                              int(b["groups"]), _stream()), "bh_conv_dgrad_bnreduce")
@@ -943,10 +947,23 @@
 
 
 def bn_bwd(gy, y, x, gamma, stats, rmean, rvar, groups, eps, relu, training, want_gres, ggamma=None, gbeta=None, beta=None,
-           had_res=None, scratch=None, sums_ready=None, amax=None):
+           had_res=None, scratch=None, sums_ready=None, amax=None, gy_masked=False):
     _chk(gy); _chk(x)
     C = gamma.numel() if gamma is not None else x.shape[-1]
     rows = x.numel() // C // groups
+    if gy_masked:
+        had_res = want_gres if had_res is None else had_res
+        if sums_ready is None or not relu or not had_res or C == 1:
+            raise RuntimeError("bn_bwd: gy_masked is the one-launch form of a BatchNorm + residual + ReLU behind conv_dgrad(bn_reduce=...)")
+        gx = torch.empty_like(x)
+        flags = 1 | 16 | BN_GY_MASKED | (BN_DETERMINISTIC if deterministic() else 0)
+        with _Timed("bn_bwd(1 kernels)" + (" g%d rows%d C%d" % (groups, rows, C) if TIMING_DETAIL else ""), 0.0, 4.0 * x.numel() * 3):
+            check(lib.bh_bn_bwd(_p(gy), None, _p(x), _p(gamma), _p(beta), _p(stats), _p(gx), None, _p(ggamma), _p(gbeta),
+                                _p(sums_ready), groups, rows, C, float(eps), flags, 0 if training else 1, _p(rmean), _p(rvar),
+                                _p(amax), _stream()), "bh_bn_bwd")
+        if amax is not None:
+            gx._bh_amax = amax
+        return gx, (gy if want_gres else None)
     gx = torch.empty_like(x)
     gres = torch.empty_like(x) if want_gres else None
     if sums_ready is not None:
diff --git a/bihome_amd/net.py b/bihome_amd/net.py
--- a/bihome_amd/net.py
+++ b/bihome_amd/net.py
@@ -451,7 +451,7 @@
 
 
 class _BwPass:
-    __slots__ = ("prog", "plan", "ctx", "slots", "grads", "bn_reduced", "red_arena", "amax_next", "want_wgrad", "want_input_grad",
+    __slots__ = ("prog", "plan", "ctx", "slots", "grads", "bn_reduced", "bn_masked", "red_arena", "amax_next", "want_wgrad", "want_input_grad",
                  "on_param_grad", "wgrad_stream", "main", "det_ws", "x3_ws", "input_sink")
 
 
@@ -514,8 +514,10 @@
         sums = s.red_arena[plan.red_off[b]:plan.red_off[b] + K.bn_stats_doubles(ctx.groups, bm.num_features)]
         red = dict(z=s.slots[bop.src], y=s.slots[bop.dst] if (bop.relu and bop.res is not None) else None,
                    stats=ctx.stats[b], gamma=bm.weight, beta=bm.bias, eps=bm.eps, relu=bop.relu, sums=sums,
-                   groups=ctx.groups)
+                   groups=ctx.groups, store_masked=i in plan.store_masked)
         s.bn_reduced[b] = sums
+        if red["store_masked"]:
+            s.bn_masked.add(b)
     if i in plan.fuse_bias and op.src not in grads and red is None:
         p = plan.fuse_bias[i]
         grads[op.src] = K.conv_dgrad(g, wk, d, wpacked=ctx.wpacked.get(i),
@@ -565,7 +567,8 @@
             yb = None
         gx, gres = K.bn_bwd(g, yb, x, m.weight, ctx.stats[i], m.running_mean, m.running_var, ctx.groups,
                             m.eps, op.relu, ctx.training, op.res is not None and ((op.res != 0) or s.want_input_grad),
-                            ggamma, gbeta, beta=m.bias, had_res=op.res is not None, sums_ready=s.bn_reduced.get(i), amax=amax)
+                            ggamma, gbeta, beta=m.bias, had_res=op.res is not None, sums_ready=s.bn_reduced.get(i), amax=amax,
+                            gy_masked=i in s.bn_masked)
     if train_w and s.on_param_grad is not None:
         s.on_param_grad(m.weight)
         s.on_param_grad(m.bias)
@@ -622,7 +625,7 @@
     s.want_wgrad, s.want_input_grad, s.on_param_grad = want_wgrad, want_input_grad, on_param_grad
     s.det_ws, s.x3_ws, s.input_sink = det_ws, x3_ws, input_sink
     s.grads = grads = {prog.ops[-1].dst: gout}
-    s.bn_reduced = {}
+    s.bn_reduced, s.bn_masked = {}, set()
     s.red_arena, amax_arena = _zero_arenas(plan.total, plan.nrec * K.AMAX_FLOATS, gout.device)
     s.amax_next = iter(amax_arena.split(K.AMAX_FLOATS)).__next__ if plan.nrec else None
     ops, slots, joined, arms = prog.ops, ctx.slots, ctx.joined, _BW_ARMS
diff --git a/bihome_amd/plan.py b/bihome_amd/plan.py
--- a/bihome_amd/plan.py
+++ b/bihome_amd/plan.py
@@ -165,7 +165,7 @@
 
 
 class BackwardPlan:
-    __slots__ = ("nops", "consumed_by", "fuse_bn", "fuse_bias", "from_1x1", "red_off", "bias_off", "total", "nrec")
+    __slots__ = ("nops", "consumed_by", "fuse_bn", "store_masked", "fuse_bias", "from_1x1", "red_off", "bias_off", "total", "nrec")
 
 
 def backward_key(prog, ctx, gout_shape, want_wgrad):
@@ -184,6 +184,11 @@
                     and j in descs and descs[j].bh_reduce_ok and descs[j].N % ctx.groups == 0 and b not in ctx.joined):
                 fuse_bn[j] = b
     return fuse_bn
+
+
+def plan_store_masked(prog, ix, ctx, fuse_bn):
+    ops = prog.ops
+    return {j for j, b in fuse_bn.items() if ops[b].relu and ops[b].res is not None}
 
 
 def plan_fuse_bias(prog, ix, ctx, want_wgrad, fuse_bn):
@@ -234,6 +239,7 @@
     p.nops = ix.nops
     p.consumed_by = ix.users
     p.fuse_bn = plan_fuse_bn(prog, ix, ctx)
+    p.store_masked = plan_store_masked(prog, ix, ctx, p.fuse_bn)
     p.fuse_bias = plan_fuse_bias(prog, ix, ctx, want_wgrad, p.fuse_bn)
     p.from_1x1 = plan_from_1x1(prog, ix, ctx, p.fuse_bn)
     p.red_off, p.bias_off, p.total, p.nrec = plan_backward_arenas(prog, ctx, p.fuse_bn, p.fuse_bias)
diff --git a/include/bihome.h b/include/bihome.h
--- a/include/bihome.h
+++ b/include/bihome.h
@@ -16,6 +16,7 @@
 
 #define BH_F_DETERMINISTIC 1
 #define BH_BN_DETERMINISTIC 32
+#define BH_BN_GY_MASKED 64
 int bh_probe_mfma_bf16(int random_operands, float* sink_dev, double* tflops, void* stream);
 int bh_probe_mfma_f32(int random_operands, float* sink_dev, double* tflops, void* stream);
 
@@ -152,6 +153,7 @@
 int bh_conv_dgrad(const float* gy, const float* w, float* gx, const bh_conv_desc* d, int accumulate, void* stream);
 int bh_conv_dgrad_s2(const float* gy, const float* w, float* gx, const bh_conv_desc* d, int accumulate, float* wpack,
                      void* stream);
+#define BH_BNR_STORE_MASKED 2
 typedef struct bh_bn_reduce {
     const float* z;
     const float* y;
```

Result: no change. 5149, median of 6 (+0.5%).
